# AllenNeuralDynamics/aind-exaspim-neuron-segmentation

Hardware: AMD Instinct MI355X
Metric: affinity voxels/sec on 96^3 patches over a 1024x1024x1024 volume, 1 MI355X (higher is better)
Workload: dtype fp16; 1 GPU; 1024x1024x1024 uint16 volume, 96^3 patches, overlap 32, trim 8, batch 16, fp16 (IEEE half) storage of activations and weights / fp32 accumulate (BASELINE.json configs[2]); streams=1

## Files before the change

### aind_exaspim_neuron_segmentation_amd/_native.py

```python

import ctypes
import os

_HERE = os.path.dirname(os.path.abspath(__file__))
LIB_PATH = os.path.join(_HERE, "csrc", "libexaspim_affinity.so")

DT_F32, DT_BF16, DT_F16 = 0, 1, 2
DT_BF16X3 = 3
VOX_U8, VOX_U16, VOX_I16, VOX_F32, VOX_F64 = 0, 1, 2, 3, 4
IN_F32, IN_PADDED_F32, IN_PADDED_SPLIT_F16, IN_PADDED_SPLIT_BF16 = 0, 1, 2, 3
UP_CONVT = 0x100
OPT_SEPARATE_POOL, OPT_SEPARATE_DEEP_POOLS, OPT_PLAIN_UPSAMPLE, OPT_FIRST_PER_GROUP = 1, 2, 4, 8
OPT_UPSAMPLE_PER_THREAD = 16
OPT_PER_PATCH_ENCODER = 32
OPT_SEPARATE_HEAD = 64
OPT_ROW_SEPARATE_BORDERS = 256
AFF_F32, AFF_F16 = 0, 1

DTYPE_CODES = {
    "fp32": DT_F32, "float32": DT_F32, "f32": DT_F32,
    "bf16": DT_BF16, "bfloat16": DT_BF16,
    "fp16": DT_F16, "float16": DT_F16, "f16": DT_F16,
    "bf16x3": DT_BF16X3,
}


class Block(ctypes.Structure):

    _fields_ = [
        ("dims", ctypes.c_int32 * 3),
        ("origin", ctypes.c_int32 * 3),
        ("global_", ctypes.c_int32 * 3),
    ]

    @classmethod
    def make(cls, dims, origin=None, global_shape=None):
        origin = (0, 0, 0) if origin is None else origin
        global_shape = dims if global_shape is None else global_shape
        b = cls()
        b.dims[:] = [int(v) for v in dims]
        b.origin[:] = [int(v) for v in origin]
        b.global_[:] = [int(v) for v in global_shape]
        return b


class Window(ctypes.Structure):

    _fields_ = [
        ("patch", ctypes.c_int32 * 3),
        ("overlap", ctypes.c_int32 * 3),
        ("trim", ctypes.c_int32),
    ]

    @classmethod
    def make(cls, patch, overlap, trim):
        w = cls()
        w.patch[:] = [int(v) for v in patch]
        w.overlap[:] = [int(v) for v in overlap]
        w.trim = int(trim)
        return w


class ComponentsStreamDesc(ctypes.Structure):

    _fields_ = [
        ("dims", ctypes.c_int32 * 3),
        ("channels", ctypes.c_int32),
        ("threshold", ctypes.c_float),
        ("capacity", ctypes.c_int32),
        ("min_size", ctypes.c_int64),
        ("next_z", ctypes.c_int32),
        ("reserved", ctypes.c_int32),
        ("id_parent_dev", ctypes.c_void_p),
        ("id_count_dev", ctypes.c_void_p),
        ("table_dev", ctypes.c_void_p),
        ("state_dev", ctypes.c_void_p),
        ("seam_ids_dev", ctypes.c_void_p),
        ("seam_bits_dev", ctypes.c_void_p),
    ]


_lib = None

_I32x5 = ctypes.c_int32 * 5
_I32x3 = ctypes.c_int32 * 3
_vp = ctypes.c_void_p
_sz = ctypes.c_size_t
_i32 = ctypes.c_int32

SIGNATURES = {
    "exaspim_abi_version": (_i32, []),
    "exaspim_last_error": (ctypes.c_char_p, []),
    "exaspim_unet_param_count": (_sz, [_I32x5, _i32, _i32]),
    "exaspim_unet_packed_bytes": (_sz, [_I32x5, _i32, _i32]),
    "exaspim_unet_pack_weights": (_i32, [_I32x5, _i32, _i32, _vp, _sz, _vp, _sz]),
    "exaspim_unet_create": (_i32, [_I32x5, _i32, _i32, _i32, _vp, _sz, ctypes.POINTER(_vp)]),
    "exaspim_unet_destroy": (None, [_vp]),
    "exaspim_unet_workspace_bytes": (_sz, [_vp, _i32, _i32, _i32, _i32]),
    "exaspim_unet_forward": (_i32, [_vp, _vp, _vp, _i32, _i32, _i32, _i32, _i32, _vp, _sz, _vp]),
    "exaspim_unet_forward_trimmed": (
        _i32, [_vp, _vp, _vp, _i32, _i32, _i32, _i32, _i32, _i32, _vp, _sz, _vp]
    ),
    "exaspim_unet_input_layout": (_i32, [_vp]),
    "exaspim_unet_forward_prepared": (
        _i32, [_vp, _vp, _vp, _i32, _i32, _i32, _i32, _i32, _i32, _vp, _sz, _vp]),
    "exaspim_unet_forward_prepared_row": (
        _i32, [_vp, _vp, _vp, _i32, _i32, _i32, _i32, _i32, _i32, _i32, _vp, _sz, _vp]),
    "exaspim_unet_forward_prepared_clipped": (
        _i32, [_vp, _vp, _vp, _i32, _i32, _i32, _i32, _i32, _i32, _i32, _I32x3, _vp, _sz, _vp]),
    "exaspim_unet_forward_absmax": (
        _i32, [_vp, _vp, _vp, _i32, _i32, _i32, _i32, _i32, _vp, _vp, _sz, _vp]),
    "exaspim_unet_set_options": (_i32, [_vp, ctypes.c_uint32]),
    "exaspim_unet_timing_begin": (_i32, [_vp, ctypes.c_uint32]),
    "exaspim_unet_timing_read": (_i32, [_vp, ctypes.POINTER(ctypes.c_double * 17),
                                        ctypes.POINTER(ctypes.c_int32 * 17)]),
    "exaspim_histogram": (_i32, [_vp, _i32, _sz, ctypes.c_double, _i32, _i32, ctypes.c_uint32, _vp, _vp]),
    "exaspim_histogram_wide": (_i32, [_vp, _i32, _sz, ctypes.c_double, _i32, _i32, ctypes.c_uint64, _vp, _vp]),
    "exaspim_gather_patches": (_i32, [_vp, _i32, ctypes.POINTER(Block), _vp, _i32, _I32x3,
                                      ctypes.c_double, _i32, ctypes.c_double, ctypes.c_double, _vp, _vp]),
    "exaspim_gather_patches_as": (_i32, [_vp, _i32, ctypes.POINTER(Block), _vp, _i32, _I32x3,
                                         ctypes.c_double, _i32, ctypes.c_double, ctypes.c_double, _i32,
                                         _vp, _vp]),
    "exaspim_stitch_accumulate": (_i32, [_vp, _vp, _i32, _i32, ctypes.POINTER(Window), _vp,
                                         ctypes.POINTER(Block), _vp]),
    "exaspim_stitch_finalize": (_i32, [_vp, _i32, ctypes.POINTER(Window), ctypes.POINTER(Block), _vp]),
    "exaspim_export_f16": (_i32, [_vp, _vp, ctypes.c_size_t, _vp]),
    "exaspim_components_workspace_bytes": (_sz, [_I32x3]),
    "exaspim_components": (_i32, [_vp, _i32, _i32, _I32x3, ctypes.c_float, ctypes.c_int64, _vp, _vp, _vp,
                                  _sz, _vp]),
    "exaspim_components_stream_slab_workspace_bytes": (_sz, [_I32x3]),
    "exaspim_components_stream_finish_workspace_bytes": (_sz, [_i32]),
    "exaspim_components_stream_slab": (_i32, [ctypes.POINTER(ComponentsStreamDesc), _vp, _i32, _I32x3, _i32, _vp,
                                              _vp, _sz, _vp]),
    "exaspim_components_stream_finish": (_i32, [ctypes.POINTER(ComponentsStreamDesc), _vp, _sz, _vp]),
    "exaspim_components_stream_apply": (_i32, [ctypes.POINTER(ComponentsStreamDesc), _vp, _sz, _vp]),
    "exaspim_region_graph_workspace_bytes": (_sz, [_I32x3, _i32, ctypes.c_int64]),
    "exaspim_region_graph": (_i32, [_vp, _vp, _i32, _I32x3, _i32, ctypes.c_int64, _vp, _vp, _vp, _vp, _vp, _vp,
                                    _sz, _vp]),
    "exaspim_agglomerate": (_i32, [_vp, _vp, _vp, ctypes.c_int64, _vp, _i32, ctypes.c_float, ctypes.c_int64,
                                   _vp, _vp]),
    "exaspim_apply_label_table": (_i32, [_vp, _sz, _vp, _i32, _vp]),
    "exaspim_synth_volume_u16": (_i32, [_vp, ctypes.POINTER(Block), ctypes.c_uint64, _vp]),
    "exaspim_synth_volume_neurite_u16": (_i32, [_vp, ctypes.POINTER(Block), ctypes.c_uint64, _vp]),
}


def lib():
    global _lib
    if _lib is None:
        path = LIB_PATH
        override = os.environ.get("EXASPIM_LIB")
        if override:
            import sys

            path = os.path.abspath(override)
            print(f"exaspim: EXASPIM_LIB is set, loading {path} instead of the in-tree library",
                  file=sys.stderr)
        if not os.path.exists(path):
            raise RuntimeError(
                f"HIP extension not built: {path} is missing. Build it with "
                "`make -C aind_exaspim_neuron_segmentation_amd/csrc` (or "
                "`python -c 'import __graft_entry__ as g; g.build()'`). "
                "There is no CPU fallback."
            )
        handle = ctypes.CDLL(path)
        for name, (restype, argtypes) in SIGNATURES.items():
            fn = getattr(handle, name)
            fn.restype = restype
            fn.argtypes = argtypes
        _lib = handle
    return _lib


def last_error():
    msg = lib().exaspim_last_error()
    return msg.decode("utf-8", "replace") if msg else ""


def check(rc, what):
    if rc == 0:
        return
    msg = f"{what}: {last_error()} (code {rc})"
    if rc == -1:
        raise ValueError(msg)
    raise RuntimeError(msg)


def channels_array(channels):
    if len(channels) != 5:
        raise ValueError("expected five channel widths")
    return _I32x5(*[int(c) for c in channels])


def int3(values):
    return _I32x3(*[int(v) for v in values])
```

### aind_exaspim_neuron_segmentation_amd/csrc/common.h

```cpp
#pragma once

#include <hip/hip_runtime.h>

#include <cstdarg>
#include <cstddef>
#include <cstdint>
#include <cstdio>

#include "../../include/exaspim_affinity.h"

namespace exaspim {

void set_error(const char* fmt, ...);
const char* get_error();

#define EXA_CHECK_ARG(cond, ...)                 \
    do {                                         \
        if (!(cond)) {                           \
            ::exaspim::set_error(__VA_ARGS__);   \
            return EXASPIM_E_INVALID;            \
        }                                        \
    } while (0)

#define EXA_CHECK_HIP(expr)                                                  \
    do {                                                                     \
        hipError_t _e = (expr);                                              \
        if (_e != hipSuccess) {                                              \
            ::exaspim::set_error("%s failed: %s (%s:%d)", #expr,             \
                                 hipGetErrorString(_e), __FILE__, __LINE__); \
            return EXASPIM_E_HIP;                                            \
        }                                                                    \
    } while (0)

__device__ __forceinline__ uint4 record_half(uint2 lo_group, uint2 hi_group) {
    const auto r0 = __builtin_amdgcn_permlane32_swap(lo_group.x, hi_group.x, false, false);
    const auto r1 = __builtin_amdgcn_permlane32_swap(lo_group.y, hi_group.y, false, false);
    return make_uint4(r0[0], r1[0], r0[1], r1[1]);
}


typedef unsigned int exa_u32x4 __attribute__((ext_vector_type(4)));
__device__ __forceinline__ void buf_store16(const uint4& v, __amdgpu_buffer_rsrc_t rsrc, unsigned voff,
                                            unsigned soff) {
    const exa_u32x4 d = {v.x, v.y, v.z, v.w};
    const unsigned ssoff = __builtin_amdgcn_readfirstlane(soff);
    asm volatile("s_nop 4\n\tbuffer_store_dwordx4 %0, %1, %2, %3 offen\n\ts_nop 1"
                 :: "v"(d), "v"(voff), "s"(rsrc), "s"(ssoff) : "memory");
}

__device__ __forceinline__ void buf_store16_counted(const uint4& v, __amdgpu_buffer_rsrc_t rsrc, unsigned voff,
                                                    unsigned soff) {
    const exa_u32x4 d = {v.x, v.y, v.z, v.w};
    __builtin_amdgcn_sched_barrier(0);
    __builtin_amdgcn_raw_buffer_store_b128(d, rsrc, (int)voff, (int)__builtin_amdgcn_readfirstlane(soff), 0);
    asm volatile("s_nop 1");
    __builtin_amdgcn_sched_barrier(0);
}

__device__ __forceinline__ float sat_f16(float v) {
    return v != v ? v : __builtin_amdgcn_fmed3f(v, -65504.f, 65504.f);
}

__device__ __forceinline__ float max_nan(float a, float b) {
    return (a != a || b != b) ? __uint_as_float(0x7fc00000u) : fmaxf(a, b);
}
__device__ __forceinline__ uint4 max_nan4(const uint4& a, const uint4& b) {
    return make_uint4(__float_as_uint(max_nan(__uint_as_float(a.x), __uint_as_float(b.x))),
                      __float_as_uint(max_nan(__uint_as_float(a.y), __uint_as_float(b.y))),
                      __float_as_uint(max_nan(__uint_as_float(a.z), __uint_as_float(b.z))),
                      __float_as_uint(max_nan(__uint_as_float(a.w), __uint_as_float(b.w))));
}
typedef short s16x2 __attribute__((ext_vector_type(2)));
typedef unsigned short u16x2 __attribute__((ext_vector_type(2)));
__device__ __forceinline__ unsigned key16x2(unsigned x) {
    const s16x2 m = __builtin_bit_cast(s16x2, x) >> (short)15;
    return x ^ (__builtin_bit_cast(unsigned, m) & 0x7fff7fffu);
}
template <unsigned INF16>
__device__ __forceinline__ unsigned okey16x2(unsigned x) {
    const u16x2 mag = __builtin_bit_cast(u16x2, x & 0x7fff7fffu);
    const auto nan = mag > (u16x2){(unsigned short)INF16, (unsigned short)INF16};
    return key16x2(x & ~(__builtin_bit_cast(unsigned, nan) & 0x80008000u));
}
__device__ __forceinline__ unsigned maxkey16x2(unsigned ka, unsigned kb) {
    return __builtin_bit_cast(
        unsigned, __builtin_elementwise_max(__builtin_bit_cast(s16x2, ka), __builtin_bit_cast(s16x2, kb)));
}
__device__ __forceinline__ uint4 key16(const uint4& v) {
    return make_uint4(key16x2(v.x), key16x2(v.y), key16x2(v.z), key16x2(v.w));
}
template <unsigned INF16>
__device__ __forceinline__ uint4 okey16(const uint4& v) {
    return make_uint4(okey16x2<INF16>(v.x), okey16x2<INF16>(v.y), okey16x2<INF16>(v.z), okey16x2<INF16>(v.w));
}
__device__ __forceinline__ uint4 maxkey16(const uint4& a, const uint4& b) {
    return make_uint4(maxkey16x2(a.x, b.x), maxkey16x2(a.y, b.y), maxkey16x2(a.z, b.z), maxkey16x2(a.w, b.w));
}

template <int N>
__device__ __forceinline__ float head_dot(float acc, const float (&f)[N], const float* w) {
#pragma clang fp contract(off)
#pragma unroll
    for (int j = 0; j < N; ++j) acc = fmaf(f[j], w[j], acc);
    return acc;
}
__device__ __forceinline__ float head_activation(float r, int apply_sigmoid) {
#pragma clang fp contract(off)
    if (apply_sigmoid) r = 1.f / (1.f + expf(-r));
    return r;
}

constexpr int kChannelPad = 32;
constexpr int kNumMfmaConvs = 17;

inline int pad_channels(int c) { return (c + kChannelPad - 1) / kChannelPad * kChannelPad; }
inline size_t align_up(size_t v, size_t a) { return (v + a - 1) / a * a; }
inline int storage_dtype(int dtype) { return dtype == EXASPIM_DT_BF16X3 ? EXASPIM_DT_F32 : dtype; }
inline int dtype_size(int dtype) { return storage_dtype(dtype) == EXASPIM_DT_F32 ? 4 : 2; }

struct ConvLayer {
    int ca_real = 0, cb_real = 0;
    int ca = 0, cb = 0;
    int cout_real = 0, cout = 0;
    size_t w_off = 0;
    size_t b_off = 0;
    size_t p_off = 0;
};

struct ConvTLayer {
    int cin_real = 0, cin = 0;
    int cout_real = 0, cout = 0;
    size_t w_off = 0;
    size_t b_off = 0;
    size_t p_off = 0;
};

struct UNetPlan {
    int channels[5] = {0, 0, 0, 0, 0};
    int out_channels = 0;
    int dtype = 0;
    bool convt = false;
    ConvTLayer up[4];
    int c0 = 0, c0p = 0;
    size_t first_p_off = 0;
    size_t first_w_off = 0;
    size_t first_b_off = 0;
    ConvLayer conv[kNumMfmaConvs];
    size_t head_p_off = 0;
    size_t head_w_off = 0;
    size_t head_b_off = 0;
    size_t packed_bytes = 0;
    size_t n_params = 0;
};

bool make_plan(const int32_t channels[5], int32_t out_channels, int32_t dtype,
               UNetPlan* plan);

int pack_weights(const UNetPlan& plan, const float* params, void* packed_host);

struct ConvArgs {
    const void* src_a;
    const void* src_b;
    int ca, cb;
    const void* weights;
    const void* weights_paired = nullptr;
    const void* weights_k32 = nullptr;
    const float* bias;
    void* dst;
    int cout;
    int n, d, h, w;
    float slope;
    const float* head_w = nullptr;
    const float* head_b = nullptr;
    float* head_out = nullptr;
    int head_oc = 0;
    int head_sigmoid = 0;
    int org[3] = {0, 0, 0};
    int ext[3] = {0, 0, 0};
    void* pool_dst = nullptr;
    int row_stride = 0;
    float* partial = nullptr;
    size_t partial_patch_bytes = 0;
    int ksplit = 1;
#ifdef EXASPIM_TRACE
    unsigned long long* trace = nullptr;
#endif
};

struct ConvLaunchRecord {
    const char* config = "";
    int ksplit = 0;
    bool row = false;
};
ConvLaunchRecord& last_conv_launch();
const char*& last_layer_kernel();

int launch_conv3x3x3(int dtype, const ConvArgs& a, hipStream_t stream);
int launch_conv3x3x3_thin(int dtype, const ConvArgs& a, hipStream_t stream);
int conv_zcol_main_extent(int ext, int axis);
bool conv_can_fuse_head(int cout, int w, int head_oc, int dtype = EXASPIM_DT_F32);
int launch_conv3x3x3_x3_head(const ConvArgs& a, hipStream_t stream);
bool conv_x3_can_fuse_head(int cout, int w, int head_oc);
bool conv_can_fuse_pool(int dtype, int cout, int d, int h, int w);
bool conv_row_mode_ok(int dtype, int cout, int n, int w, int row_stride, bool fused_pool_whole_patch);
constexpr int kRowStageMain = 1, kRowStageThin = 2, kRowStagePool = 4;
constexpr int kRowStagesAll = kRowStageMain | kRowStageThin | kRowStagePool;
constexpr int kRowStageBorders = 8;
constexpr int kRowStagesFused = kRowStageMain | kRowStageBorders;
int launch_conv3x3x3_row(int dtype, const ConvArgs& a, int stages, hipStream_t stream);

int launch_conv_first(int dtype, const float* x, float* xpad, const float* w, const float* bias,
                      void* dst, int n, int d, int h, int wd, int c0p, float slope,
                      hipStream_t stream, bool first_no_strips = false);
int launch_convt2(int dtype, const void* src, const void* weights, const float* bias, void* dst,
                  int n, int d, int h, int w, int cin, int cout, hipStream_t stream);
int launch_maxpool2(int dtype, const void* src, void* dst, int n, int d, int h, int w,
                    int c, hipStream_t stream);
int launch_maxpool2_xcols(int dtype, const void* src, void* dst, int n, int d, int h, int w,
                          int c, int ox0, int ox1, hipStream_t stream);
int launch_upsample2(int dtype, const void* src, void* dst, int n, int d, int h, int w,
                     int c, int margin, hipStream_t stream, bool plain_kernel = false, bool per_thread = false,
                     const int* margin_hi = nullptr);
int launch_absmax(int dtype, const void* src, size_t bytes, float* out, hipStream_t stream);
int launch_head(int dtype, const void* src, const float* w, const float* bias,
                float* out, int n, int d, int h, int wd, int c0p, int out_channels,
                int apply_sigmoid, hipStream_t stream);

}
```

### aind_exaspim_neuron_segmentation_amd/csrc/conv3d.hip

```cpp

#include <cstdlib>

#include "common.h"
#include "conv_device.h"
#include "conv_t14.h"
#include "conv_x3.h"
#include "conv_zcol.h"

namespace exaspim {

#ifdef EXASPIM_TRACE
int g_variant = 0;
#endif

ConvLaunchRecord& last_conv_launch() {
    static thread_local ConvLaunchRecord rec;
    return rec;
}

static int resident_workgroups(int per_cu) {
    static int cus = 0;
    if (cus == 0) {
        int dev = 0, n = 0;
        if (hipGetDevice(&dev) != hipSuccess ||
            hipDeviceGetAttribute(&n, hipDeviceAttributeMultiprocessorCount, dev) != hipSuccess || n <= 0)
            n = 256;
        cus = n;
    }
    return cus * per_cu;
}

static inline int cdiv(int a, int b) { return (a + b - 1) / b; }

struct TileGrid {
    int tz, ty, tx;
    long long blocks;
};
static int tile_grid(const ConvArgs& a, int TZ, int TY, int TX, int ex, int n, TileGrid& g) {
    g.tz = cdiv(a.ext[0], TZ), g.ty = cdiv(a.ext[1], TY), g.tx = cdiv(ex, TX);
    g.blocks = (long long)g.tz * g.ty * g.tx * n;
    if (g.blocks <= 0 || g.blocks > 0x7fffffffLL) {
        set_error("conv: grid of %lld blocks out of range", g.blocks);
        return EXASPIM_E_INVALID;
    }
    return EXASPIM_OK;
}

static int choose_ksplit(const ConvArgs& a, const TileGrid& g, int slices, int units) {
    const bool whole = a.ext[0] == a.d && a.ext[1] == a.h && a.ext[2] == a.w;
    constexpr int kNominalBatch = 16;
    const long long wgs = (long long)g.tz * g.ty * g.tx * kNominalBatch * slices;
    if (!a.partial || !whole || wgs * 2 > resident_workgroups(2)) return 1;
    int ks = (int)(resident_workgroups(2) / wgs);
    if (ks > 4) ks = 4;
    if (ks > units) ks = units;
    const size_t patch_vox = (size_t)a.d * a.h * a.w;
    while (ks > 1 && (size_t)ks * patch_vox * a.cout * sizeof(float) > a.partial_patch_bytes) --ks;
    return ks;
}

template <typename Tag, int TZ, int TY, int TX, int MINW, int D, int HEAD = 0, bool POOL = false>
static int launch_zpipe(const ConvArgs& a, hipStream_t stream) {
    const bool row = POOL && HEAD == 0 && Tag::kG == 8 && a.row_stride > 0;
    TileGrid g;
    if (int rc = row ? tile_grid(a, TZ, TY, TX, a.n * a.row_stride + a.w - a.row_stride, 1, g)
                     : tile_grid(a, TZ, TY, TX, a.ext[2], a.n, g))
        return rc;
    const int tz = g.tz, ty = g.ty, tx = g.tx;
    const long long blocks = g.blocks;
    const int slices = a.cout / 32;
    long long wgs = resident_workgroups(MINW) / slices / 8 * 8;
    if (wgs < 8) wgs = 8;
    if (wgs > blocks) wgs = blocks;
#ifdef EXASPIM_TRACE
    if (g_variant >= 10 && g_variant < 20) wgs = blocks;
    if (const char* e = getenv("EXASPIM_TRACE_WGS_PER_CU")) wgs = resident_workgroups(1) * (long long)atoi(e) / slices / 8 * 8;
#endif
    dim3 grid((unsigned)wgs, slices);
    last_conv_launch() = {__PRETTY_FUNCTION__, 1};
    if constexpr (POOL && HEAD == 0 && Tag::kG == 8) {
        if (row) {
            last_conv_launch().row = true;
            conv3x3x3_zpipe_row<Tag, TZ, TY, TX, MINW, D><<<grid, TY * TX * 2, 0, stream>>>(a, tz, ty, tx);
            EXA_CHECK_HIP(hipGetLastError());
            return EXASPIM_OK;
        }
    }
    conv3x3x3_zpipe<Tag, TZ, TY, TX, MINW, D, HEAD, POOL><<<grid, TY * TX * 2, 0, stream>>>(a, tz, ty, tx);
    EXA_CHECK_HIP(hipGetLastError());
    return EXASPIM_OK;
}


template <typename Tag, int TZ, int TY, int TX, int WAVES_M, int WAVES_N, int MT, int NT, int MINW, int PD = 3,
          bool ZORD = false, bool POOL = false>
static int launch_cfg(const ConvArgs& a, hipStream_t stream) {
    constexpr int NWG = WAVES_N * NT * 32;
    if (a.cout % NWG != 0) {
        set_error("conv: cout %d not a multiple of the %d-channel tile", a.cout, NWG);
        return EXASPIM_E_INVALID;
    }
    TileGrid g;
    if (int rc = tile_grid(a, TZ, TY, TX, a.ext[2], a.n, g)) return rc;
    const int tz = g.tz, ty = g.ty, tx = g.tx;
    ConvArgs b = a;
    b.ksplit = a.head_out ? 1 : choose_ksplit(a, g, a.cout / NWG, (a.ca + a.cb) / (2 * Tag::kG));
    const size_t nvox_all = (size_t)a.n * a.d * a.h * a.w;
    dim3 grid((unsigned)g.blocks, a.cout / NWG, b.ksplit);
    last_conv_launch() = {__PRETTY_FUNCTION__, b.ksplit};
    if (POOL && b.ksplit > 1) {
        b.pool_dst = nullptr;
        conv3x3x3_t14<Tag, TZ, TY, TX, WAVES_M, WAVES_N, MT, NT, MINW, PD, ZORD, false>
            <<<grid, WAVES_M * WAVES_N * 64, 0, stream>>>(b, tz, ty, tx);
    } else {
        conv3x3x3_t14<Tag, TZ, TY, TX, WAVES_M, WAVES_N, MT, NT, MINW, PD, ZORD, POOL>
            <<<grid, WAVES_M * WAVES_N * 64, 0, stream>>>(b, tz, ty, tx);
    }
    EXA_CHECK_HIP(hipGetLastError());
    if (b.ksplit > 1) {
        const size_t items = nvox_all * (a.cout / 4);
        splitk_reduce_kernel<Tag><<<(unsigned)((items + 255) / 256), 256, 0, stream>>>(
            a.partial, a.bias, a.dst, nvox_all, (size_t)a.d * a.h * a.w, a.cout, b.ksplit, a.slope);
        EXA_CHECK_HIP(hipGetLastError());
        if (POOL)
            return launch_maxpool2(Tag::kCode, a.dst, a.pool_dst, a.n, a.d, a.h, a.w, a.cout, stream);
    }
    return EXASPIM_OK;
}

template <typename Tag> struct ES_of { static constexpr int value = 16 / Tag::kG; };

template <typename Tag, int TZ, int TY, int TX, int WAVES_M, int WAVES_N, int MT, int NT, int MINW>
static int launch_cfg_pool(const ConvArgs& a, hipStream_t stream) {
    if constexpr (ES_of<Tag>::value == 2) {
        if (a.pool_dst)
            return launch_cfg<Tag, TZ, TY, TX, WAVES_M, WAVES_N, MT, NT, MINW, 3, false, true>(a, stream);
    }
    return launch_cfg<Tag, TZ, TY, TX, WAVES_M, WAVES_N, MT, NT, MINW>(a, stream);
}

template <typename Tag, int TZ, int D>
static int launch_zpipe_head(const ConvArgs& a, hipStream_t stream) {
    if (a.head_out && a.cout == 32) {
        switch (a.head_oc) {
            case 1: return launch_zpipe<Tag, TZ, 8, 16, 2, D, 1>(a, stream);
            case 2: return launch_zpipe<Tag, TZ, 8, 16, 2, D, 2>(a, stream);
            case 3: return launch_zpipe<Tag, TZ, 8, 16, 2, D, 3>(a, stream);
            case 4: return launch_zpipe<Tag, TZ, 8, 16, 2, D, 4>(a, stream);
        }
    }
    if (a.pool_dst) return launch_zpipe<Tag, TZ, 8, 16, 2, D, 0, true>(a, stream);
    return launch_zpipe<Tag, TZ, 8, 16, 2, D>(a, stream);
}

template <typename Tag, int TZ>
static int launch_zpipe_d(const ConvArgs& a, hipStream_t stream) {
#ifdef EXASPIM_TRACE
    if (g_variant % 10 == 3) return launch_zpipe_head<Tag, TZ, 3>(a, stream);
    if (g_variant % 10 == 5) return launch_zpipe_head<Tag, TZ, 5>(a, stream);
#endif
    return launch_zpipe_head<Tag, TZ, 4>(a, stream);
}

template <typename Tag>
static int launch_typed(const ConvArgs& a, hipStream_t stream) {
    if (a.w >= 16 && a.w % 16 == 0) {
#ifdef EXASPIM_TRACE
        if (g_variant >= 20) return launch_zpipe_d<Tag, 6>(a, stream);
#endif
        if (a.cout % 64 != 0) {
            if (a.head_out && a.cout == 32 && a.ext[0] % 6 != 0 && a.ext[0] % kHeadTZ == 0) {
                switch (a.head_oc) {
                    case 1: return launch_zpipe<Tag, kHeadTZ, 8, 16, 2, 4, 1>(a, stream);
                    case 2: return launch_zpipe<Tag, kHeadTZ, 8, 16, 2, 4, 2>(a, stream);
                    case 3: return launch_zpipe<Tag, kHeadTZ, 8, 16, 2, 4, 3>(a, stream);
                    case 4: return launch_zpipe<Tag, kHeadTZ, 8, 16, 2, 4, 4>(a, stream);
                }
            }
            if (a.d % 6 == 0) return launch_zpipe_d<Tag, 6>(a, stream);
            return launch_zpipe_d<Tag, 4>(a, stream);
        }
        if (a.pool_dst) return launch_cfg_pool<Tag, 4, 8, 16, 4, 1, 4, 2, 2>(a, stream);
        return launch_cfg<Tag, 4, 8, 16, 4, 1, 4, 2, 2>(a, stream);
    }
    if (a.w > 12) {
        if (a.cout % 64 == 0) return launch_cfg_pool<Tag, 4, 4, 24, 4, 1, 3, 2, 2>(a, stream);
        return launch_cfg_pool<Tag, 4, 4, 24, 4, 1, 3, 1, 2>(a, stream);
    }
    if (a.w > 6) {
        if (a.cout % 256 == 0) return launch_cfg_pool<Tag, 4, 4, 12, 2, 1, 3, 1, 2>(a, stream);
        if (a.cout % 128 == 0) return launch_cfg_pool<Tag, 4, 4, 12, 2, 2, 3, 2, 2>(a, stream);
        if (a.cout % 64 == 0) return launch_cfg_pool<Tag, 4, 4, 12, 2, 2, 3, 1, 2>(a, stream);
        return launch_cfg_pool<Tag, 4, 4, 12, 2, 1, 3, 1, 2>(a, stream);
    }
    return launch_cfg<Tag, 6, 6, 6, 4, 1, 2, 1, 2>(a, stream);
}

template <int TZ, int TY, int TX, int WAVES_M, int WAVES_N, int MT, int NT, int MINW, int PD>
static int launch_x3(const ConvArgs& a, hipStream_t stream) {
    constexpr int NWG = WAVES_N * NT * 32;
    if (a.cout % NWG != 0) {
        set_error("conv: cout %d not a multiple of the %d-channel tile", a.cout, NWG);
        return EXASPIM_E_INVALID;
    }
    TileGrid g;
    if (int rc = tile_grid(a, TZ, TY, TX, a.ext[2], a.n, g)) return rc;
    const int tz = g.tz, ty = g.ty, tx = g.tx;
    ConvArgs b = a;
    b.ksplit = choose_ksplit(a, g, a.cout / NWG, (a.ca + a.cb) / 16);
    const size_t patch_vox_all = (size_t)a.d * a.h * a.w;
    const size_t nvox_all = (size_t)a.n * patch_vox_all;
    dim3 grid((unsigned)g.blocks, a.cout / NWG, b.ksplit);
    last_conv_launch() = {__PRETTY_FUNCTION__, b.ksplit};
    conv3x3x3_x3<TZ, TY, TX, WAVES_M, WAVES_N, MT, NT, MINW, PD>
        <<<grid, WAVES_M * WAVES_N * 64, 0, stream>>>(b, tz, ty, tx);
    EXA_CHECK_HIP(hipGetLastError());
    if (b.ksplit > 1) {
        const size_t items = nvox_all * (a.cout / 4);
        splitk_reduce_kernel<F32Tag><<<(unsigned)((items + 255) / 256), 256, 0, stream>>>(
            a.partial, a.bias, a.dst, nvox_all, patch_vox_all, a.cout, b.ksplit, a.slope);
        EXA_CHECK_HIP(hipGetLastError());
    }
    return EXASPIM_OK;
}

static int launch_typed_x3(const ConvArgs& a, hipStream_t stream) {
    if (a.w >= 16 && a.w % 16 == 0) {
        if (a.cout % 64 == 0) return launch_x3<2, 8, 16, 4, 1, 2, 2, 2, 3>(a, stream);
        return launch_x3<4, 8, 16, 4, 1, 4, 1, 2, 3>(a, stream);
    }
    if (a.w > 12) {
        if (a.cout % 64 == 0) return launch_x3<4, 4, 24, 4, 1, 3, 2, 2, 1>(a, stream);
        return launch_x3<4, 4, 24, 4, 1, 3, 1, 2, 3>(a, stream);
    }
    if (a.w > 6) {
        if (a.cout % 256 == 0) return launch_x3<4, 4, 12, 2, 1, 3, 1, 2, 3>(a, stream);
        if (a.cout % 128 == 0) return launch_x3<4, 4, 12, 2, 2, 3, 2, 2, 2>(a, stream);
        if (a.cout % 64 == 0) return launch_x3<4, 4, 12, 2, 2, 3, 1, 2, 3>(a, stream);
        return launch_x3<4, 4, 12, 2, 1, 3, 1, 2, 3>(a, stream);
    }
    return launch_x3<6, 6, 6, 4, 1, 2, 1, 2, 3>(a, stream);
}

static int launch_thin_typed_x3(const ConvArgs& a, hipStream_t stream) {
    if (a.ext[1] <= a.ext[2]) return launch_x3<8, 2, 16, 4, 1, 2, 1, 2, 3>(a, stream);
    return launch_x3<8, 16, 2, 4, 1, 2, 1, 2, 3>(a, stream);
}

template <int HEAD>
static int launch_x3_head(const ConvArgs& a, hipStream_t stream) {
    TileGrid g;
    if (int rc = tile_grid(a, kX3HeadTZ, kX3HeadTY, kX3HeadTX, a.ext[2], a.n, g)) return rc;
    last_conv_launch() = {__PRETTY_FUNCTION__, 1};
    conv3x3x3_x3_head<HEAD><<<dim3((unsigned)g.blocks, 1, 1), 256, 0, stream>>>(a, g.tz, g.ty, g.tx);
    EXA_CHECK_HIP(hipGetLastError());
    return EXASPIM_OK;
}

bool conv_can_fuse_pool(int dtype, int cout, int d, int h, int w) {
    if (d % 2 != 0 || h % 2 != 0 || w % 2 != 0) return false;
    if (dtype == EXASPIM_DT_BF16X3) return false;
    if (cout % 64 != 0 && w >= 16 && w % 16 == 0) return true;
    return dtype != EXASPIM_DT_F32 && w > 6;
}

static bool head_shape_ok(int cout, int w, int head_oc) {
    return cout == 32 && w >= 16 && w % 16 == 0 && head_oc >= 1 && head_oc <= 4;
}
bool conv_can_fuse_head(int cout, int w, int head_oc, int dtype) {
    return dtype != EXASPIM_DT_BF16X3 && head_shape_ok(cout, w, head_oc);
}
bool conv_x3_can_fuse_head(int cout, int w, int head_oc) { return head_shape_ok(cout, w, head_oc); }

static int resolve_region(ConvArgs& a) {
    const int dims[3] = {a.d, a.h, a.w};
    for (int i = 0; i < 3; ++i) {
        if (a.ext[i] == 0 && a.org[i] == 0) a.ext[i] = dims[i];
        EXA_CHECK_ARG(a.org[i] >= 0 && a.ext[i] > 0 && a.org[i] + a.ext[i] <= dims[i],
                      "conv: region [%d, %d) outside axis %d of a %dx%dx%d patch", a.org[i],
                      a.org[i] + a.ext[i], i, a.d, a.h, a.w);
    }
    return EXASPIM_OK;
}

int conv_zcol_main_extent(int ext, int axis) {
    const int tile = axis == 1 ? 8 : 16;
    const int rem = ext % tile;
    return (axis != 0 && ext > tile && rem >= 1 && rem <= 4) ? ext - rem : ext;
}

bool conv_row_mode_ok(int dtype, int cout, int n, int w, int row_stride, bool fused_pool_whole_patch) {
    const int o = w - row_stride;
    return dtype_size(dtype) == 2 && fused_pool_whole_patch && cout % 64 != 0 &&
           w % 16 == 0 && n >= 2 && row_stride > 0 && o > 0 && o % 32 == 0 && row_stride >= o;
}

static int check_row_args(int dtype, const ConvArgs& a) {
    const bool whole = a.ext[0] == a.d && a.ext[1] == a.h && a.ext[2] == a.w;
    EXA_CHECK_ARG(conv_row_mode_ok(dtype, a.cout, a.n, a.w, a.row_stride,
                                   a.pool_dst && !a.head_out && whole &&
                                       conv_can_fuse_pool(dtype, a.cout, a.d, a.h, a.w)),
                  "conv: row mode needs a 16-bit fused-pool z-column layer, whole patches, n >= 2 and "
                  "an overlap that is a multiple of 32 and at most the stride (w %d, stride %d, n %d)",
                  a.w, a.row_stride, a.n);
    return EXASPIM_OK;
}

enum : unsigned { kCheckPadded = 1, kCheckEmpty = 2, kCheckSlope = 4, kCheckPatchBytes = 8, kCheckAll = 15 };
static int check_conv_args(int dtype, const ConvArgs& a, unsigned checks) {
    const int kc = dtype == EXASPIM_DT_F32 ? 8 : 16;
    EXA_CHECK_ARG(!(checks & kCheckPadded) || (a.ca % kc == 0 && a.cb % kc == 0 && a.cout % 32 == 0 && a.ca > 0),
                  "conv: channels (%d,%d)->%d not padded", a.ca, a.cb, a.cout);
    EXA_CHECK_ARG(!(checks & kCheckEmpty) || (a.n > 0 && a.d > 0 && a.h > 0 && a.w > 0), "conv: empty input");
    EXA_CHECK_ARG(!(checks & kCheckSlope) || (a.slope >= 0.f && a.slope <= 1.f),
                  "conv: LeakyReLU slope %g outside [0, 1]", a.slope);
    const unsigned long long rec = (unsigned long long)a.d * a.h * a.w * (a.ca > a.cb ? a.ca : a.cb) * dtype_size(dtype);
    EXA_CHECK_ARG(!(checks & kCheckPatchBytes) || rec < 0x80000000ULL,
                  "conv: one patch of one source is %llu bytes (>= 2 GiB)", rec);
    return EXASPIM_OK;
}

int launch_conv3x3x3(int dtype, const ConvArgs& a_in, hipStream_t stream) {
    ConvArgs a = a_in;
    if (int rc = check_conv_args(dtype, a, kCheckAll)) return rc;
    if (int rc = resolve_region(a)) return rc;
    const bool whole = a.ext[0] == a.d && a.ext[1] == a.h && a.ext[2] == a.w;
    EXA_CHECK_ARG(!a.pool_dst || (conv_can_fuse_pool(dtype, a.cout, a.d, a.h, a.w) && !a.head_out && whole),
                  "conv: fused max-pool needs an even, untrimmed patch (16-bit modes: wider than 6 voxels; "
                  "float32: a 32-cout-slice layer)");
    EXA_CHECK_ARG(!a.head_out || conv_can_fuse_head(a.cout, a.w, a.head_oc, dtype),
                  "conv: fused head needs cout 32, w %% 16 == 0, 1..4 outputs (and not bf16x3)");
    if (a.row_stride > 0)
        if (int rc = check_row_args(dtype, a)) return rc;
    switch (dtype) {
        case EXASPIM_DT_F32: return launch_typed<F32Tag>(a, stream);
        case EXASPIM_DT_BF16: return launch_typed<BF16Tag>(a, stream);
        case EXASPIM_DT_F16: return launch_typed<F16Tag>(a, stream);
        case EXASPIM_DT_BF16X3: return launch_typed_x3(a, stream);
    }
    set_error("conv: unknown dtype %d", dtype);
    return EXASPIM_E_INVALID;
}

int launch_conv3x3x3_x3_head(const ConvArgs& a_in, hipStream_t stream) {
    ConvArgs a = a_in;
    if (int rc = check_conv_args(EXASPIM_DT_BF16X3, a, kCheckAll)) return rc;
    EXA_CHECK_ARG(conv_x3_can_fuse_head(a.cout, a.w, a.head_oc),
                  "conv: bf16x3 fused head needs cout 32, w %% 16 == 0 and 1..4 outputs (cout %d, w %d, %d outputs)",
                  a.cout, a.w, a.head_oc);
    EXA_CHECK_ARG(a.head_out && a.head_w && a.head_b, "conv: bf16x3 fused head: NULL head pointer");
    EXA_CHECK_ARG(!a.pool_dst && a.row_stride == 0, "conv: bf16x3 fused head has no fused max-pool or row mode");
    if (int rc = resolve_region(a)) return rc;
    a.partial = nullptr;
    a.ksplit = 1;
    switch (a.head_oc) {
        case 1: return launch_x3_head<1>(a, stream);
        case 2: return launch_x3_head<2>(a, stream);
        case 3: return launch_x3_head<3>(a, stream);
        default: return launch_x3_head<4>(a, stream);
    }
}

template <typename Tag>
static int launch_thin_typed(const ConvArgs& a, hipStream_t stream) {
    const int ez = a.ext[0];
    auto planes = [&](int tz) { return (ez + tz - 1) / tz * tz; };
    if (a.ext[1] <= a.ext[2]) {
        const float c4 = planes(4) * 1.00f, c8 = planes(8) * 0.76f, c12 = planes(12) * 0.66f;
        if (c12 <= c8 && c12 <= c4) return launch_cfg<Tag, 12, 2, 16, 4, 1, 3, 1, 3, 3, true>(a, stream);
        if (c8 <= c4) return launch_cfg<Tag, 8, 2, 16, 4, 1, 2, 1, 4, 3, true>(a, stream);
        return launch_cfg<Tag, 4, 2, 16, 4, 1, 1, 1, 4, 3, true>(a, stream);
    }
    if (planes(8) * 0.78f <= planes(4) * 1.00f) return launch_cfg<Tag, 8, 16, 2, 4, 1, 2, 1, 4, 3, true>(a, stream);
    return launch_cfg<Tag, 4, 16, 2, 4, 1, 1, 1, 4, 3, true>(a, stream);
}

int launch_conv3x3x3_thin(int dtype, const ConvArgs& a_in, hipStream_t stream) {
    ConvArgs a = a_in;
    if (int rc = check_conv_args(dtype, a, kCheckPadded | kCheckEmpty)) return rc;
    EXA_CHECK_ARG(!a.pool_dst && !a.head_out && a.row_stride == 0, "conv: thin tiles have no fused pool, head or row mode");
    if (int rc = resolve_region(a)) return rc;
    a.partial = nullptr;
    switch (dtype) {
        case EXASPIM_DT_F32: return launch_thin_typed<F32Tag>(a, stream);
        case EXASPIM_DT_BF16: return launch_thin_typed<BF16Tag>(a, stream);
        case EXASPIM_DT_F16: return launch_thin_typed<F16Tag>(a, stream);
        case EXASPIM_DT_BF16X3: return launch_thin_typed_x3(a, stream);
    }
    set_error("conv: unknown dtype %d", dtype);
    return EXASPIM_E_INVALID;
}

template <typename Tag, int TZ, int MT>
static int launch_row_borders_cfg(const ConvArgs& a, hipStream_t stream) {
    const int tz = cdiv(a.d, TZ), ty = cdiv(a.h, 16);
    const long long blocks = (long long)tz * ty * 2 * (a.n - 1);
    if (blocks <= 0 || blocks > 0x7fffffffLL) {
        set_error("conv: grid of %lld blocks out of range", blocks);
        return EXASPIM_E_INVALID;
    }
    last_conv_launch() = {__PRETTY_FUNCTION__, 1};
    conv3x3x3_t14<Tag, TZ, 16, 2, 4, 1, MT, 1, 4, 3, true, true>
        <<<dim3((unsigned)blocks, a.cout / 32, 1), 256, 0, stream>>>(a, tz, ty, 2);
    EXA_CHECK_HIP(hipGetLastError());
    return EXASPIM_OK;
}

template <typename Tag>
static int launch_row_borders(const ConvArgs& a_in, hipStream_t stream) {
    ConvArgs a = a_in;
    a.partial = nullptr;
    a.ksplit = 1;
    a.row_stride = 0;
    auto planes = [&](int tz) { return (a.d + tz - 1) / tz * tz; };
    if (planes(8) * 0.78f <= planes(4) * 1.00f) return launch_row_borders_cfg<Tag, 8, 2>(a, stream);
    return launch_row_borders_cfg<Tag, 4, 1>(a, stream);
}

int launch_conv3x3x3_row(int dtype, const ConvArgs& a, int stages, hipStream_t stream) {
    ConvArgs b = a;
    if (int rc = check_conv_args(dtype, a, kCheckEmpty)) return rc;
    if (int rc = resolve_region(b)) return rc;
    if (int rc = check_row_args(dtype, b)) return rc;
    int r = EXASPIM_OK;
    if (stages & kRowStageMain) r = launch_conv3x3x3(dtype, a, stream);
    b.pool_dst = nullptr;
    b.row_stride = 0;
    b.n = a.n - 1;
    b.ext[2] = 2;
    if (r == EXASPIM_OK && (stages & kRowStageThin)) {
        const size_t vox = (size_t)a.d * a.h * a.w;
        b.src_a = static_cast<const char*>(a.src_a) + vox * a.ca * dtype_size(dtype);
        b.dst = static_cast<char*>(a.dst) + vox * a.cout * dtype_size(dtype);
        r = launch_conv3x3x3_thin(dtype, b, stream);
        if (r == EXASPIM_OK) {
            b.org[2] = a.w - 2;
            b.src_a = a.src_a;
            b.dst = a.dst;
            r = launch_conv3x3x3_thin(dtype, b, stream);
        }
    }
    if (r == EXASPIM_OK && (stages & kRowStagePool))
        r = launch_maxpool2_xcols(dtype, a.dst, a.pool_dst, a.n, a.d, a.h, a.w, a.cout, 0, a.w / 2 - 1, stream);
    if (r == EXASPIM_OK && (stages & kRowStageBorders)) {
        r = check_conv_args(dtype, a, kCheckPadded);
        ConvArgs c = a;
        for (int i = 0; i < 3; ++i) { c.org[i] = b.org[i]; c.ext[i] = b.ext[i]; }
        c.org[2] = 0;
        if (r == EXASPIM_OK)
            r = dtype == EXASPIM_DT_F16 ? launch_row_borders<F16Tag>(c, stream) : launch_row_borders<BF16Tag>(c, stream);
    }
    return r;
}

}
```

### aind_exaspim_neuron_segmentation_amd/csrc/conv_zcol.h

```cpp
#pragma once

#include "conv_device.h"

namespace exaspim {

template <typename Tag, int TZ, int TY, int TX, int MINW, int D, int HEAD, bool POOL, bool ROW>
__device__ __forceinline__ void zpipe_body(const ConvArgs& a, int tiles_z, int tiles_y, int tiles_x) {
    constexpr int G = Tag::kG;
    constexpr int KC = 2 * G;
    constexpr int ES = 16 / G;
    constexpr int HZ = TZ + 2, HY = TY + 2, HX = TX + 2;
    constexpr int HXP = HX;
    constexpr int PLANE = HY * HXP;
    constexpr int HVP = HZ * PLANE;
    constexpr int GS = HVP + (24 - HVP % 16) % 16;
    constexpr int NWAVES = TY * TX / 32;
    constexpr int NTHREADS = NWAVES * 64;
    constexpr int NPAIR = 2 * HY * HX;
    constexpr int REM = NPAIR > NTHREADS ? NPAIR - NTHREADS : 0;
    constexpr int SEC = (REM * HZ + NTHREADS - 1) / NTHREADS;
    constexpr int NITEMS = HZ + SEC;
    constexpr int RECB = 32 * ES;
    constexpr int RECP = RECB + 16;
    constexpr int EPI_UNITS = NWAVES * 32 * RECP / 16;
    constexpr int WUNITS = 27 * 64;
    constexpr int WITEMS = (WUNITS + NTHREADS - 1) / NTHREADS;
    constexpr int XUNITS = 2 * GS > EPI_UNITS ? 2 * GS : EPI_UNITS;
    constexpr int LDS_UNITS = XUNITS + WUNITS;
    constexpr int NS = 9 * HZ;
    constexpr int R = D + 1;
    constexpr int kLoadStride = 2;
    constexpr int LOAD_STRIDE = kLoadStride * (NITEMS + WITEMS) <= NS ? kLoadStride : 1;
    static_assert(TY * TX % 32 == 0 && NPAIR <= 2 * NTHREADS, "tile shape");
    static_assert(LOAD_STRIDE * (NITEMS + WITEMS) <= NS, "the staged pieces fit into the steps");

    __shared__ __attribute__((aligned(16))) uint4 lds[LDS_UNITS];

    const int tid = threadIdx.x;
    const int lane = tid & 63;
    const int wave = __builtin_amdgcn_readfirstlane(tid >> 6);
    const int half = lane >> 5;
    const int r = (TX == 16 && (lane & 16)) ? 16 + (((lane & 15) - HXP) & 15) : (lane & 31);

    constexpr bool row = ROW;
    static_assert(!ROW || (POOL && ES == 2 && HEAD == 0), "row mode: 16-bit fused-pool epilogue");
    const int total = tiles_z * tiles_y * tiles_x * (row ? 1 : a.n);
    int t_first, t_count, t_step;
    {
        const int q = total >> 3, rem = total & 7;
        const int xcd = blockIdx.x & 7, slot = blockIdx.x >> 3;
        t_first = (xcd < rem ? xcd * (q + 1) : rem * (q + 1) + (xcd - rem) * q) + slot;
        t_count = q + (xcd < rem ? 1 : 0) - slot;
        t_step = (gridDim.x + 7 - xcd) >> 3;
    }
    if (t_count <= 0) return;
    const int ntiles = a.cout >> 5;
    const int ntile0 = blockIdx.y;

    struct Tile {
        int z0, y0, x0, nb;
    };
    auto row_tile_at = [&](int id) {
        Tile t;
        const int s = a.row_stride, ho = (a.w - s) >> 1;
        const int rx = (id % tiles_x) * TX; id /= tiles_x;
        const int nb = min(max(rx - ho, 0) / s, a.n - 1);
        t.x0 = __builtin_amdgcn_readfirstlane(rx - nb * s);
        t.y0 = __builtin_amdgcn_readfirstlane((id % tiles_y) * TY); id /= tiles_y;
        t.z0 = __builtin_amdgcn_readfirstlane((id % tiles_z) * TZ);
        t.nb = __builtin_amdgcn_readfirstlane(nb);
        return t;
    };
    auto tile_at = [&](int id) {
        if (row) return row_tile_at(id);
        Tile t;
        t.x0 = __builtin_amdgcn_readfirstlane(a.org[2] + (id % tiles_x) * TX); id /= tiles_x;
        t.y0 = __builtin_amdgcn_readfirstlane(a.org[1] + (id % tiles_y) * TY); id /= tiles_y;
        t.z0 = __builtin_amdgcn_readfirstlane(a.org[0] + (id % tiles_z) * TZ); id /= tiles_z;
        id = __builtin_amdgcn_readfirstlane(id);
        t.nb = id;
        return t;
    };

    const int pos = wave * 32 + r;
    const int col = (pos / TX) * HXP + (pos % TX) + half * GS;

    const int plane_vox = a.h * a.w;
    const size_t patch_vox = (size_t)a.d * plane_vox;
    const bool p_ok = tid < NPAIR;
    const int p_hy = (tid >> 1) / HX, p_hx = (tid >> 1) % HX, p_kg = tid & 1;
    const int p_slot = p_kg * GS + p_hy * HXP + p_hx;
    unsigned p_voff;
    unsigned s_voff[SEC > 0 ? SEC : 1];
    int s_slot[SEC > 0 ? SEC : 1];
#pragma unroll
    for (int k = 0; k < SEC; ++k) {
        const int q = tid + k * NTHREADS;
        const int pr = NTHREADS + q % REM, hz = q / REM;
        const int c = pr >> 1, kg = pr & 1;
        s_slot[k] = q < REM * HZ ? kg * GS + hz * PLANE + (c / HX) * HXP + c % HX : -1;
    }
    auto set_offsets = [&](const Tile& t) {
        {
            const int gy = t.y0 + p_hy - 1, gx = t.x0 + p_hx - 1;
            const bool in = p_ok && (unsigned)gy < (unsigned)a.h && (unsigned)gx < (unsigned)a.w;
            p_voff = in ? (unsigned)(gy * a.w + gx) * 32u + p_kg * 16u : kOutOfRange;
        }
#pragma unroll
        for (int k = 0; k < SEC; ++k) {
            const int q = tid + k * NTHREADS;
            const int pr = NTHREADS + q % REM, hz = q / REM;
            const int c = pr >> 1, kg = pr & 1;
            const int gz = t.z0 + hz - 1, gy = t.y0 + c / HX - 1, gx = t.x0 + c % HX - 1;
            const bool in = q < REM * HZ && (unsigned)gz < (unsigned)a.d &&
                            (unsigned)gy < (unsigned)a.h && (unsigned)gx < (unsigned)a.w;
            s_voff[k] = in ? (unsigned)((gz * a.h + gy) * a.w + gx) * 32u + kg * 16u : kOutOfRange;
        }
    };
    const unsigned wvoff = (((tid >> 6) * ntiles) * 64 + (tid & 63)) * 16u;

    __shared__ __attribute__((aligned(16))) float bias_s[32];
    if (tid < 32) bias_s[tid] = a.bias[ntile0 * 32 + tid];
    __shared__ __attribute__((aligned(16))) float head_s[HEAD > 0 ? HEAD * 32 + 4 : 4];
    if (HEAD > 0) {
        if (tid < HEAD * 32) head_s[tid] = a.head_w[tid];
        if (tid < HEAD) head_s[HEAD * 32 + tid] = a.head_b[tid];
    }

    const int nchunks = (a.ca + a.cb) / KC;
    uint4 stg[NITEMS + WITEMS];
    uint4* const wlds = lds + XUNITS;
    const __amdgpu_buffer_rsrc_t wrsrc = make_rsrc(a.weights, (size_t)nchunks * 27 * ntiles * 1024);

    struct ChunkSrc {
        __amdgpu_buffer_rsrc_t rsrc;
        __amdgpu_buffer_rsrc_t none;
        unsigned cbase;
    };
    auto chunk_src = [&](int c, int nb) {
        const char* src;
        int cs, ch0;
        if (c * KC < a.ca) {
            src = static_cast<const char*>(a.src_a); cs = a.ca; ch0 = c * KC;
        } else {
            src = static_cast<const char*>(a.src_b); cs = a.cb; ch0 = c * KC - a.ca;
        }
        const size_t patchb = patch_vox * cs * ES;
        return ChunkSrc{make_rsrc(src + (size_t)nb * patchb, patchb), make_rsrc(src + (size_t)nb * patchb, 0),
                        (unsigned)(ch0 / KC) * (unsigned)patch_vox * 32u};
    };
    auto load_piece = [&](const ChunkSrc& cs, int c, int z0, int i) {
        if (i < NITEMS) {
            if (i < HZ) {
                const int gz = z0 + i - 1;
                stg[i] = (unsigned)gz < (unsigned)a.d
                             ? buf_load16(cs.rsrc, p_voff, cs.cbase + (unsigned)gz * plane_vox * 32u)
                             : buf_load16(cs.none, p_voff, 0);
            } else {
                stg[i] = buf_load16(cs.rsrc, s_voff[i - HZ], cs.cbase);
            }
        } else {
            const int it = i - NITEMS;
            stg[i] = it * NWAVES + wave < 27
                         ? buf_load16(wrsrc, wvoff, ((c * 27 + it * NWAVES) * ntiles + ntile0) * 1024)
                         : make_uint4(0, 0, 0, 0);
        }
    };
    auto stage_store = [&]() {
        if ((EXASPIM_ABLATE & 4) && stg[0].x != 0x12345u) return;
        if (p_ok) {
#pragma unroll
            for (int hz = 0; hz < HZ; ++hz) lds[p_slot + hz * PLANE] = stg[hz];
        }
#pragma unroll
        for (int k = 0; k < SEC; ++k)
            if (s_slot[k] >= 0) lds[s_slot[k]] = stg[HZ + k];
#pragma unroll
        for (int it = 0; it < WITEMS; ++it) {
            const int i = tid + it * NTHREADS;
            if (i < WUNITS) wlds[i] = stg[NITEMS + it];
        }
    };

    int tile_id = t_first;
    Tile cur = tile_at(tile_id);
    set_offsets(cur);
    {
        const ChunkSrc cs0 = chunk_src(0, cur.nb);
#pragma unroll
        for (int i = 0; i < NITEMS + WITEMS; ++i) load_piece(cs0, 0, cur.z0, i);
    }
    stage_store();

    for (;;) {
#ifdef EXASPIM_TRACE
        const size_t trace_rec = ((size_t)tile_id * NWAVES + wave) * 16;
        if (a.trace && lane == 0)
            a.trace[trace_rec + 15] =
                ((unsigned long long)__builtin_amdgcn_s_getreg((31 << 11) | 20) << 32) |
                (unsigned)__builtin_amdgcn_s_getreg((31 << 11) | 4);
#endif
        EXA_TRACE(0);
        EXA_TRACE(1);
        __syncthreads();
        f32x16 acc[TZ];
        const int half_t = fresh_lane() >> 5;
#pragma unroll
        for (int q = 0; q < 4; ++q) {
            const float4 b = *reinterpret_cast<const float4*>(bias_s + 8 * q + 4 * half_t);
#pragma unroll
            for (int mt = 0; mt < TZ; ++mt) {
                acc[mt][4 * q + 0] = b.x; acc[mt][4 * q + 1] = b.y;
                acc[mt][4 * q + 2] = b.z; acc[mt][4 * q + 3] = b.w;
            }
        }
        EXA_TRACE(2);

        t_count -= t_step;
        const bool has_next = t_count > 0;
        Tile nxt = cur;
        for (int c = 0; c < nchunks; ++c) {
            const bool more = c + 1 < nchunks;
            const bool pre = more || has_next;
            if (!more && has_next) {
                nxt = tile_at(tile_id + t_step);
                set_offsets(nxt);
            }
            const ChunkSrc csn = chunk_src(more ? c + 1 : 0, more ? cur.nb : nxt.nb);
            const int cn = more ? c + 1 : 0, zn = more ? cur.z0 : nxt.z0;
            uint4 xr[R];
            uint4 wb[3];
#pragma unroll
            for (int dz = 0; dz < 3; ++dz) wb[dz] = wlds[(dz * 9) * 64 + lane];
#pragma unroll
            for (int s = 0; s < D; ++s)
                xr[s % R] = lds[col + (s % HZ) * PLANE + ((s / HZ) / 3) * HXP + (s / HZ) % 3];
            __builtin_amdgcn_sched_barrier(0);
            if (ES == 2) __builtin_amdgcn_s_setprio(kSetprio);
#pragma unroll
            for (int s = 0; s < NS; ++s) {
                const int g = s / HZ, zin = s % HZ;
                if (s + D < NS) {
                    const int g2 = (s + D) / HZ, z2 = (s + D) % HZ;
                    xr[(s + D) % R] = lds[col + z2 * PLANE + (g2 / 3) * HXP + g2 % 3];
                }
#ifdef EXASPIM_TRACE
                if (nchunks == 2 && c == 0 && s > 0 && s % (NS / 4) == 0 && s / (NS / 4) <= 3) EXA_TRACE(8 + s / (NS / 4));
#endif
                if (g + 1 < 9 && zin >= TZ) wb[zin - TZ] = wlds[((zin - TZ) * 9 + g + 1) * 64 + lane];
                if (g > 0 && zin == 0) wb[2] = wlds[(2 * 9 + g) * 64 + lane];
                if (!(EXASPIM_ABLATE & 1) && pre && s % LOAD_STRIDE == 0 && s / LOAD_STRIDE < NITEMS + WITEMS)
                    load_piece(csn, cn, zn, s / LOAD_STRIDE);
#pragma unroll
                for (int dz = 0; dz < 3; ++dz) {
                    const int z = zin - dz;
                    if (z >= 0 && z < TZ) mma_inplace<Tag>(acc[z], wb[dz], xr[s % R]);
                }
                __builtin_amdgcn_sched_barrier(0);
            }
            if (ES == 2) __builtin_amdgcn_s_setprio(0);
            if (ES == 2) asm volatile("s_nop 7\n\ts_nop 7\n\ts_nop 1");
            if (c < 4) EXA_TRACE(3 + 3 * c);
            __syncthreads();
            if (c < 4) EXA_TRACE(4 + 3 * c);
            if (more) {
                stage_store();
                __syncthreads();
                if (c < 3) EXA_TRACE(5 + 3 * c);
            }
        }
        if (has_next) {
#pragma unroll
            for (int i = 0; i < NITEMS + WITEMS; ++i)
                asm volatile("" : "+v"(stg[i].x), "+v"(stg[i].y), "+v"(stg[i].z), "+v"(stg[i].w));
        }

        const int lane_e = fresh_lane();
        const int half_e = lane_e >> 5;
        const int r_e = (TX == 16 && (lane_e & 16)) ? 16 + (((lane_e & 15) - HXP) & 15) : (lane_e & 31);
        const int pos_e = wave * 32 + r_e;
        if (HEAD > 0) {
            float part[TZ][HEAD > 0 ? HEAD : 1];
#pragma unroll
            for (int z = 0; z < TZ; ++z)
#pragma unroll
                for (int o = 0; o < HEAD; ++o) part[z][o] = 0.f;
#pragma unroll
            for (int q = 0; q < 4; ++q) {
                float4 hw[HEAD > 0 ? HEAD : 1];
#pragma unroll
                for (int o = 0; o < HEAD; ++o)
                    hw[o] = *reinterpret_cast<const float4*>(head_s + o * 32 + 8 * q + 4 * half_e);
#pragma unroll
                for (int z = 0; z < TZ; ++z) {
                    float v0 = acc[z][4 * q + 0], v1 = acc[z][4 * q + 1];
                    float v2 = acc[z][4 * q + 2], v3 = acc[z][4 * q + 3];
                    v0 = leaky(v0, a.slope);
                    v1 = leaky(v1, a.slope);
                    v2 = leaky(v2, a.slope);
                    v3 = leaky(v3, a.slope);
#pragma unroll
                    for (int o = 0; o < HEAD; ++o)
                        part[z][o] = fmaf(v3, hw[o].w, fmaf(v2, hw[o].z, fmaf(v1, hw[o].y, fmaf(v0, hw[o].x, part[z][o]))));
                }
            }
            const size_t plane = (size_t)a.h * a.w;
            const int gy = cur.y0 + pos_e / TX, gx = cur.x0 + pos_e % TX;
            const bool okyx = gy < a.org[1] + a.ext[1] && gx < a.org[2] + a.ext[2];
            float* const hpatch = a.head_out + (size_t)cur.nb * HEAD * a.d * plane;
            const size_t hbytes = (size_t)HEAD * a.d * plane * sizeof(float);
            const unsigned hvoff[2] = {okyx && half_e == 0 ? (unsigned)(gy * a.w + gx) * 4u : kOutOfRange,
                                       okyx && half_e == 1 ? (unsigned)(gy * a.w + gx) * 4u : kOutOfRange};
#pragma unroll
            for (int z = 0; z < TZ; ++z) {
                const int gz = cur.z0 + z;
                const __amdgpu_buffer_rsrc_t hrsrc = make_rsrc(hpatch, gz < a.org[0] + a.ext[0] ? hbytes : (size_t)0);
#pragma unroll
                for (int o = 0; o < HEAD; ++o) {
                    float t = part[z][o] + __shfl_xor(part[z][o], 32) + head_s[HEAD * 32 + o];
                    if (a.head_sigmoid) t = 1.f / (1.f + expf(-t));
                    __builtin_amdgcn_raw_buffer_store_b32(__float_as_uint(t), hrsrc, (int)hvoff[o & 1],
                                                          (int)((unsigned)(o * a.d + gz) * (unsigned)plane * 4u), 0);
                }
            }
        } else if (ES == 2 && !POOL) {
            char* const dplane = static_cast<char*>(a.dst) +
                                 ((size_t)cur.nb * (a.cout / KC) + ntile0 * 2) * patch_vox * 32;
            const int gy = cur.y0 + pos_e / TX, gx = cur.x0 + pos_e % TX;
            const bool okyx = gy < a.org[1] + a.ext[1] && gx < a.org[2] + a.ext[2];
            const unsigned ovoff = okyx ? (unsigned)(gy * a.w + gx) * 32u + half_e * 16u : kOutOfRange;
#pragma unroll
            for (int z = 0; z < TZ; ++z) {
                uint2 grp[4];
#pragma unroll
                for (int q = 0; q < 4; ++q)
                    grp[q] = pack4<Tag>(leaky(acc[z][4 * q + 0], a.slope), leaky(acc[z][4 * q + 1], a.slope),
                                        leaky(acc[z][4 * q + 2], a.slope), leaky(acc[z][4 * q + 3], a.slope));
                const int gz = cur.z0 + z;
#pragma unroll
                for (int ck = 0; ck < 2; ++ck) {
                    const uint4 rec = record_half(grp[2 * ck], grp[2 * ck + 1]);
                    const unsigned soff = ((unsigned)ck * (unsigned)patch_vox + (unsigned)gz * (unsigned)plane_vox) * 32u;
                    const __amdgpu_buffer_rsrc_t orsrc =
                        make_rsrc(dplane, gz < a.org[0] + a.ext[0] ? (size_t)2 * patch_vox * 32 : (size_t)0);
                    buf_store16(rec, orsrc, ovoff, soff);
                }
            }
        } else if (ES == 2 && POOL) {
            static_assert(!(ES == 2 && POOL) || (TZ % 2 == 0 && TY % 2 == 0 && TX == 16), "pooled tile shape");
            constexpr int CPT = 2;
            char* wl = reinterpret_cast<char*>(lds) + wave * ((TZ / 2) * 32 * RECP);
            char* const dplane = static_cast<char*>(a.dst) +
                                 ((size_t)cur.nb * (a.cout / KC) + ntile0 * 2) * patch_vox * 32;
            const int gy = cur.y0 + pos_e / TX, gx = cur.x0 + pos_e % TX;
            const bool okyx = gy < a.org[1] + a.ext[1] && gx < a.org[2] + a.ext[2];
            const unsigned ovoff = okyx ? (unsigned)(gy * a.w + gx) * 32u + half_e * 16u : kOutOfRange;
            const int rs = a.row_stride, rho = (a.w - rs) >> 1;
            const bool nnext = row && cur.x0 >= rs && cur.x0 < rs + rho && cur.nb + 1 < a.n;
            const bool nprev = row && cur.x0 >= rho && cur.x0 < 2 * rho && cur.nb >= 1;
            const bool shared = nnext || nprev;
            const int nshift = nnext ? -rs : nprev ? rs : 0;
            const int nnb = cur.nb + (nnext ? 1 : nprev ? -1 : 0);
            const int ngx = gx + nshift;
            const bool nlane = ngx >= 2 && ngx < a.w - 2;
            const int nbase = nshift * 32;
            char* const nplane = static_cast<char*>(a.dst) + nbase +
                                 ((size_t)nnb * (a.cout / KC) + ntile0 * 2) * patch_vox * 32;
            const size_t nbytes = (size_t)((long long)2 * patch_vox * 32 - nbase);
#pragma unroll
            for (int zp = 0; zp < TZ / 2; ++zp) {
                uint2 grp[2][4];
#pragma unroll
                for (int zz = 0; zz < 2; ++zz)
#pragma unroll
                    for (int q = 0; q < 4; ++q)
                        grp[zz][q] = pack4<Tag>(leaky(acc[2 * zp + zz][4 * q + 0], a.slope), leaky(acc[2 * zp + zz][4 * q + 1], a.slope),
                                                leaky(acc[2 * zp + zz][4 * q + 2], a.slope), leaky(acc[2 * zp + zz][4 * q + 3], a.slope));
#pragma unroll
                for (int q = 0; q < 4; ++q) {
                    const uint2 km = make_uint2(maxkey16x2(okey16x2<Tag::kInf16>(grp[0][q].x), okey16x2<Tag::kInf16>(grp[1][q].x)),
                                                maxkey16x2(okey16x2<Tag::kInf16>(grp[0][q].y), okey16x2<Tag::kInf16>(grp[1][q].y)));
                    *reinterpret_cast<uint2*>(wl + zp * (32 * RECP) + r_e * RECP + (8 * q + 4 * half_e) * ES) = km;
                }
#pragma unroll
                for (int zz = 0; zz < 2; ++zz) {
                    const int gz = cur.z0 + 2 * zp + zz;
                    const __amdgpu_buffer_rsrc_t orsrc =
                        make_rsrc(dplane, gz < a.org[0] + a.ext[0] ? (size_t)2 * patch_vox * 32 : (size_t)0);
                    const __amdgpu_buffer_rsrc_t nrsrc = make_rsrc(nplane, gz < a.org[0] + a.ext[0] ? nbytes : (size_t)0);
#pragma unroll
                    for (int ck = 0; ck < 2; ++ck) {
                        const uint4 rec = record_half(grp[zz][2 * ck], grp[zz][2 * ck + 1]);
                        buf_store16(rec, orsrc, ovoff, ((unsigned)ck * (unsigned)patch_vox + (unsigned)gz * (unsigned)plane_vox) * 32u);
                        if (shared)
                            buf_store16(rec, nrsrc, nlane ? ovoff : kOutOfRange, ((unsigned)ck * (unsigned)patch_vox + (unsigned)gz * (unsigned)plane_vox) * 32u);
                    }
                }
            }
            __builtin_amdgcn_fence(__ATOMIC_RELEASE, "wavefront");
            __builtin_amdgcn_wave_barrier();
            {
                constexpr int NP = (TZ / 2) * 8 * CPT * 2;
                const int pd = a.d >> 1, ph = a.h >> 1, pw2 = a.w >> 1;
                const size_t pvox = (size_t)pd * ph * pw2;
                char* const pplane = static_cast<char*>(a.pool_dst) +
                                     ((size_t)cur.nb * (a.cout / KC) + ntile0 * CPT) * pvox * 32;
                const __amdgpu_buffer_rsrc_t prsrc = make_rsrc(pplane, (size_t)CPT * pvox * 32);
                char* const npplane = static_cast<char*>(a.pool_dst) + nbase / 2 +
                                      ((size_t)nnb * (a.cout / KC) + ntile0 * CPT) * pvox * 32;
                const __amdgpu_buffer_rsrc_t nprsrc = make_rsrc(npplane, (size_t)((long long)CPT * pvox * 32 - nbase / 2));
#pragma unroll
                for (int p0 = 0; p0 < NP; p0 += 64) {
                    const int p = p0 + lane_e;
                    const bool live = p < NP;
                    const int pc = live ? p : 0;
                    const int zp = pc / (8 * CPT * 2), rem = pc % (8 * CPT * 2);
                    const int ck = rem / 16, xp = (rem % 16) >> 1, sb = rem & 1;
                    const char* rec = wl + zp * (32 * RECP) + (2 * xp) * RECP + (ck * 2 + sb) * 16;
                    uint4 m = *reinterpret_cast<const uint4*>(rec);
#pragma unroll
                    for (int k = 1; k < 4; ++k)
                        m = maxkey16(m, *reinterpret_cast<const uint4*>(rec + (k >> 1) * 16 * RECP + (k & 1) * RECP));
                    m = key16(m);
                    const int qz = cur.z0 / 2 + zp, qy = cur.y0 / 2 + wave, qx = cur.x0 / 2 + xp;
                    const unsigned pvoff = live && qz < pd && qy < ph && qx < pw2
                                               ? (unsigned)((ck * (int)pvox + (qz * ph + qy) * pw2 + qx) * 32 + sb * 16)
                                               : kOutOfRange;
                    buf_store16(m, prsrc, pvoff, 0u);
                    if (shared) {
                        const int nqx = qx + nshift / 2;
                        buf_store16(m, nprsrc, nqx >= 1 && nqx < pw2 - 1 ? pvoff : kOutOfRange, 0u);
                    }
                }
            }
            __builtin_amdgcn_fence(__ATOMIC_ACQUIRE, "wavefront");
            __builtin_amdgcn_wave_barrier();
        } else {
            constexpr int CPT = RECB / 32;
            constexpr int TB_MAX = LDS_UNITS * 16 / (NWAVES * 32 * RECP);
            constexpr int TB = POOL ? ((TB_MAX >= TZ ? TZ : TB_MAX) & ~1)
                                    : (TB_MAX >= TZ ? TZ : (TB_MAX >= (TZ + 1) / 2 ? (TZ + 1) / 2 : 1));
            static_assert(!POOL || (TB >= 2 && TZ % 2 == 0 && TY % 2 == 0 && TX == 16), "pooled tile shape");
            char* wl = reinterpret_cast<char*>(lds) + wave * (TB * 32 * RECP);
            char* const dplane = static_cast<char*>(a.dst) +
                                 ((size_t)cur.nb * (a.cout / KC) + ntile0 * CPT) * patch_vox * 32;
            const int vv = lane_e >> 1, sub = lane_e & 1;
            const int po = wave * 32 + vv;
            const int ogy = cur.y0 + po / TX, ogx = cur.x0 + po % TX;
#pragma unroll
            for (int zb = 0; zb < TZ; zb += TB) {
#pragma unroll
                for (int z = zb; z < zb + TB && z < TZ; ++z) {
#pragma unroll
                    for (int q = 0; q < 4; ++q) {
                        const int cl = 8 * q + 4 * half_e;
                        float v0 = acc[z][4 * q + 0], v1 = acc[z][4 * q + 1];
                        float v2 = acc[z][4 * q + 2], v3 = acc[z][4 * q + 3];
                        v0 = leaky(v0, a.slope);
                        v1 = leaky(v1, a.slope);
                        v2 = leaky(v2, a.slope);
                        v3 = leaky(v3, a.slope);
                        store4<Tag>(wl + (z - zb) * (32 * RECP), (size_t)(r_e * RECP) / ES + cl, v0, v1, v2, v3);
                    }
                }
                __builtin_amdgcn_fence(__ATOMIC_RELEASE, "wavefront");
                __builtin_amdgcn_wave_barrier();
#pragma unroll
                for (int z = zb; z < zb + TB && z < TZ; ++z) {
                    const int gz = cur.z0 + z;
                    const bool tokyx = ogy < a.org[1] + a.ext[1] && ogx < a.org[2] + a.ext[2];
                    const unsigned tvoff = tokyx ? (unsigned)(ogy * a.w + ogx) * 32u + sub * 16u : kOutOfRange;
                    const __amdgpu_buffer_rsrc_t trsrc =
                        make_rsrc(dplane, gz < a.org[0] + a.ext[0] ? (size_t)CPT * patch_vox * 32 : (size_t)0);
#pragma unroll
                    for (int ck = 0; ck < CPT; ++ck) {
                        const uint4 val = *reinterpret_cast<const uint4*>(
                            wl + (z - zb) * (32 * RECP) + vv * RECP + (ck * 2 + sub) * 16);
                        buf_store16(val, trsrc, tvoff,
                                    ((unsigned)ck * (unsigned)patch_vox + (unsigned)gz * (unsigned)plane_vox) * 32u);
                    }
                }
                if (POOL) {
                    constexpr int NP = (TB / 2) * 8 * CPT * 2;
                    const int pd = a.d >> 1, ph = a.h >> 1, pw2 = a.w >> 1;
                    const size_t pvox = (size_t)pd * ph * pw2;
                    char* const pplane = static_cast<char*>(a.pool_dst) +
                                         ((size_t)cur.nb * (a.cout / KC) + ntile0 * CPT) * pvox * 32;
                    const __amdgpu_buffer_rsrc_t prsrc = make_rsrc(pplane, (size_t)CPT * pvox * 32);
#pragma unroll
                    for (int p0 = 0; p0 < NP; p0 += 64) {
                        const int p = p0 + lane_e;
                        const bool live0 = p < NP;
                        const int pc = live0 ? p : 0;
                        const int zp = pc / (8 * CPT * 2), rem = pc % (8 * CPT * 2);
                        const int ck = rem / 16, xp = (rem % 16) >> 1, sb = rem & 1;
                        const bool live = live0 && zb + 2 * zp + 1 < TZ;
                        const int zr = zb + 2 * zp + 1 < TZ ? zp : 0;
                        const char* rec = wl + (2 * zr) * (32 * RECP) + (2 * xp) * RECP + (ck * 2 + sb) * 16;
                        uint4 m = *reinterpret_cast<const uint4*>(rec);
                        if (ES == 2) m = okey16<Tag::kInf16>(m);
#pragma unroll
                        for (int k = 1; k < 8; ++k) {
                            const uint4 v = *reinterpret_cast<const uint4*>(
                                rec + (k >> 2) * (32 * RECP) + ((k >> 1) & 1) * 16 * RECP + (k & 1) * RECP);
                            m = ES == 2 ? maxkey16(m, okey16<Tag::kInf16>(v)) : max16<Tag>(m, v);
                        }
                        if (ES == 2) m = key16(m);
                        const int qz = (cur.z0 + zb) / 2 + zp, qy = cur.y0 / 2 + wave, qx = cur.x0 / 2 + xp;
                        const unsigned pvoff =
                            live && qz < pd && qy < ph && qx < pw2
                                ? (unsigned)((ck * (int)pvox + (qz * ph + qy) * pw2 + qx) * 32 + sb * 16)
                                : kOutOfRange;
                        buf_store16(m, prsrc, pvoff, 0u);
                    }
                }
                __builtin_amdgcn_fence(__ATOMIC_ACQUIRE, "wavefront");
                __builtin_amdgcn_wave_barrier();
            }
        }
        EXA_TRACE(14);
        if (!has_next) break;
        if (!(HEAD > 0 || (ES == 2 && !POOL))) __syncthreads();
        stage_store();
        tile_id += t_step;
        cur = nxt;
    }
}

template <typename Tag, int TZ, int TY, int TX, int MINW, int D, int HEAD = 0, bool POOL = false>
__global__ __launch_bounds__(TY* TX * 2, MINW) void conv3x3x3_zpipe(
    ConvArgs a, int tiles_z, int tiles_y, int tiles_x) {
    zpipe_body<Tag, TZ, TY, TX, MINW, D, HEAD, POOL, false>(a, tiles_z, tiles_y, tiles_x);
}

template <typename Tag, int TZ, int TY, int TX, int MINW, int D>
__global__ __launch_bounds__(TY* TX * 2, MINW) void conv3x3x3_zpipe_row(
    ConvArgs a, int tiles_z, int tiles_y, int tiles_x) {
    zpipe_body<Tag, TZ, TY, TX, MINW, D, 0, true, true>(a, tiles_z, tiles_y, tiles_x);
}

}
```

### aind_exaspim_neuron_segmentation_amd/csrc/engine.hip

```cpp

#include <algorithm>
#include <cstdlib>
#include <new>
#include <string_view>

#include "common.h"

namespace exaspim {

constexpr float kLeakySlope = 0.01f;

struct Workspace {
    size_t skip[5], a[5], b[5];
    size_t xpad;
    size_t bytes;
};

}

struct LayerTimer {
    static constexpr int kRing = 16384;
    uint32_t mask = 0;
    int next = 0, used = 0;
    hipEvent_t start[kRing], stop[kRing];
    int layer[kRing];
    bool created = false;
};

struct exaspim_unet {
    exaspim::UNetPlan plan;
    int device;
    const char* packed;
    LayerTimer* timer = nullptr;
    uint32_t options = 0;
};

namespace exaspim {

static bool level_dims_ok(int d, int h, int w) {
    return d > 0 && h > 0 && w > 0 && d % 16 == 0 && h % 16 == 0 && w % 16 == 0;
}

static int conv_level(int i) {
    if (i == 0) return 0;
    if (i <= 8) return (i + 1) / 2;
    return 3 - (i - 9) / 2;
}

static Workspace make_workspace(const UNetPlan& p, int n, int d, int h, int w) {
    int maxc[5] = {p.c0p, 0, 0, 0, 0};
    for (int i = 0; i < kNumMfmaConvs; ++i) {
        const ConvLayer& L = p.conv[i];
        int& m = maxc[conv_level(i)];
        m = std::max(m, std::max(std::max(L.ca, L.cb), L.cout));
    }
    const size_t es = dtype_size(p.dtype);
    Workspace ws;
    size_t off = 0;
    for (int l = 0; l < 5; ++l) {
        const size_t vox = (size_t)n * (d >> l) * (h >> l) * (w >> l);
        const size_t sz = align_up(vox * maxc[l] * es, 256);
        ws.skip[l] = off; off += (l < 4 ? sz : 0);
        ws.a[l] = off; off += sz;
        ws.b[l] = off; off += sz;
    }
    ws.xpad = off;
    off += align_up((size_t)n * (d + 2) * (h + 2) * (w + 2) * sizeof(float), 256);
    ws.bytes = off;
    return ws;
}

static int forward(exaspim_unet* e, const float* x, float* out, int n, int d, int h, int w,
                   int apply_sigmoid, int trim, void* workspace, size_t workspace_bytes,
                   hipStream_t stream, const void* x_prepared = nullptr, float* absmax = nullptr,
                   int row_stride = 0, const int32_t* keep_hi = nullptr) {
    const UNetPlan& p = e->plan;
    const Workspace ws = make_workspace(p, n, d, h, w);
    if (workspace_bytes < ws.bytes) {
        set_error("forward: workspace %zu bytes < required %zu", workspace_bytes, ws.bytes);
        return EXASPIM_E_WORKSPACE;
    }
    char* base = static_cast<char*>(workspace);
    auto skip = [&](int l) { return (void*)(base + ws.skip[l]); };
    auto A = [&](int l) { return (void*)(base + ws.a[l]); };
    auto B = [&](int l) { return (void*)(base + ws.b[l]); };
    const int dt = p.dtype;
    int rc;

    const bool x3 = dt == EXASPIM_DT_BF16X3;
    const int last_cout = p.conv[kNumMfmaConvs - 1].cout;
    const bool fuse_head = !absmax && !(e->options & EXASPIM_OPT_SEPARATE_HEAD) &&
                           (x3 ? conv_x3_can_fuse_head(last_cout, w, p.out_channels)
                               : conv_can_fuse_head(last_cout, w, p.out_channels, dt));
    const bool trimmed = fuse_head && trim > 0 && 2 * trim < d && 2 * trim < h && 2 * trim < w;
    int khi[3] = {d - trim, h - trim, w - trim};
    if (trimmed && keep_hi)
        for (int i = 0; i < 3; ++i) khi[i] = keep_hi[i];
    const bool separate_pool = (e->options & EXASPIM_OPT_SEPARATE_POOL) != 0;
    const bool separate_deep = (e->options & EXASPIM_OPT_SEPARATE_DEEP_POOLS) != 0;
    bool fuse_pool[4];
    for (int l = 0; l < 4; ++l)
        fuse_pool[l] = !separate_pool && !(separate_deep && l > 0) && conv_can_fuse_pool(p.dtype, p.conv[2 * l].cout, d >> l, h >> l, w >> l);
    const bool row = !absmax && !(e->options & EXASPIM_OPT_PER_PATCH_ENCODER) &&
                     conv_row_mode_ok(dt, p.conv[0].cout, n, w, row_stride, fuse_pool[0]);
    auto conv = [&](int idx, const void* sa, const void* sb, void* dst, int l) -> int {
        const ConvLayer& L = p.conv[idx];
        ConvArgs a;
        a.partial = reinterpret_cast<float*>(base + ws.xpad);
        a.partial_patch_bytes = (size_t)(d + 2) * (h + 2) * (w + 2) * sizeof(float);
        if (idx <= 6 && idx % 2 == 0 && fuse_pool[idx / 2]) a.pool_dst = A(idx / 2 + 1);
        const bool last = idx == kNumMfmaConvs - 1, last_but_one = idx == kNumMfmaConvs - 2;
        const int margin = !trimmed ? 0 : last ? trim : last_but_one ? trim - 1 : 0;
        const int full[3] = {d >> l, h >> l, w >> l};
        for (int i = 0; i < 3; ++i) {
            a.org[i] = margin;
            a.ext[i] = trimmed && (last || last_but_one) ? khi[i] + (last ? 0 : 1) - margin : full[i];
        }
        int rem_y = 0, rem_x = 0;
        const bool has_head = idx == kNumMfmaConvs - 1 && fuse_head;
        if (margin > 0 && !has_head && L.cout % 64 != 0 && full[2] % 16 == 0) {
            rem_y = a.ext[1] - conv_zcol_main_extent(a.ext[1], 1);
            rem_x = a.ext[2] - conv_zcol_main_extent(a.ext[2], 2);
            a.ext[1] -= rem_y;
            a.ext[2] -= rem_x;
        }
        if (idx == kNumMfmaConvs - 1 && fuse_head) {
            a.head_w = reinterpret_cast<const float*>(e->packed + p.head_w_off);
            a.head_b = reinterpret_cast<const float*>(e->packed + p.head_b_off);
            a.head_out = out;
            a.head_oc = p.out_channels;
            a.head_sigmoid = apply_sigmoid;
        }
        a.src_a = sa; a.src_b = sb; a.ca = L.ca; a.cb = L.cb;
        a.weights = e->packed + L.w_off;
        a.bias = reinterpret_cast<const float*>(e->packed + L.b_off);
        a.dst = dst; a.cout = L.cout;
        a.n = n; a.d = d >> l; a.h = h >> l; a.w = w >> l;
        a.slope = kLeakySlope;
        if (idx == 0 && row) a.row_stride = row_stride;
        LayerTimer* t = e->timer;
        const bool timed = t && (t->mask >> idx & 1u) && t->used < LayerTimer::kRing;
        int slot = 0;
        if (timed) {
            slot = t->next;
            EXA_CHECK_HIP(hipEventRecord(t->start[slot], stream));
        }
        int r = x3 && has_head      ? launch_conv3x3x3_x3_head(a, stream)
                : a.row_stride > 0 ? launch_conv3x3x3_row(dt, a, (e->options & EXASPIM_OPT_ROW_SEPARATE_BORDERS) ? kRowStagesAll : kRowStagesFused, stream)
                                   : launch_conv3x3x3(dt, a, stream);
        if (timed && r == EXASPIM_OK) {
            EXA_CHECK_HIP(hipEventRecord(t->stop[slot], stream));
            t->layer[slot] = idx;
            t->next = (slot + 1) % LayerTimer::kRing;
            t->used++;
        }
        if (r == EXASPIM_OK && rem_y > 0) {
            ConvArgs b = a;
            b.org[1] = a.org[1] + a.ext[1]; b.ext[1] = rem_y;
            b.ext[2] = a.ext[2] + rem_x;
            r = launch_conv3x3x3_thin(dt, b, stream);
        }
        if (r == EXASPIM_OK && rem_x > 0) {
            ConvArgs b = a;
            b.org[2] = a.org[2] + a.ext[2]; b.ext[2] = rem_x;
            r = launch_conv3x3x3_thin(dt, b, stream);
        }
        if (r == EXASPIM_OK && absmax)
            r = launch_absmax(dt, dst, (size_t)n * (d >> l) * (h >> l) * (w >> l) * L.cout * dtype_size(dt),
                              absmax + 1 + idx, stream);
        return r;
    };
#define RUN(expr) do { rc = (expr); if (rc) return rc; } while (0)

    RUN(launch_conv_first(dt, x, x ? reinterpret_cast<float*>(base + ws.xpad)
                                   : const_cast<float*>(static_cast<const float*>(x_prepared)),
                          reinterpret_cast<const float*>(e->packed + p.first_w_off),
                          reinterpret_cast<const float*>(e->packed + p.first_b_off), A(0), n, d,
                          h, w, p.c0p, kLeakySlope, stream, (e->options & EXASPIM_OPT_FIRST_PER_GROUP) != 0));
    if (absmax) RUN(launch_absmax(dt, A(0), (size_t)n * d * h * w * p.c0p * dtype_size(dt), absmax, stream));
    RUN(conv(0, A(0), nullptr, skip(0), 0));
    for (int l = 1; l <= 4; ++l) {
        const ConvLayer& L0 = p.conv[2 * l - 1];
        const void* prev = skip(l - 1);
        if (!fuse_pool[l - 1])
            RUN(launch_maxpool2(dt, prev, A(l), n, d >> (l - 1), h >> (l - 1), w >> (l - 1), L0.ca,
                                stream));
        RUN(conv(2 * l - 1, A(l), nullptr, B(l), l));
        RUN(conv(2 * l, B(l), nullptr, l < 4 ? skip(l) : A(l), l));
    }
    const void* prev = A(4);
    for (int l = 3; l >= 0; --l) {
        const int i0 = 9 + 2 * (3 - l);
        const ConvLayer& L0 = p.conv[i0];
        if (p.convt) {
            const ConvTLayer& U = p.up[3 - l];
            RUN(launch_convt2(dt, prev, e->packed + U.w_off,
                              reinterpret_cast<const float*>(e->packed + U.b_off), A(l), n,
                              d >> (l + 1), h >> (l + 1), w >> (l + 1), U.cin, U.cout, stream));
            if (absmax)
                RUN(launch_absmax(dt, A(l), (size_t)n * (d >> l) * (h >> l) * (w >> l) * U.cout * dtype_size(dt),
                                  absmax + 1 + kNumMfmaConvs + (3 - l), stream));
        } else {
            const bool ups_trimmed = trimmed && l == 0 && trim > 2;
            const int ups_hi[3] = {std::max(d - khi[0] - 2, 0), std::max(h - khi[1] - 2, 0), std::max(w - khi[2] - 2, 0)};
            RUN(launch_upsample2(dt, prev, A(l), n, d >> (l + 1), h >> (l + 1), w >> (l + 1), L0.cb,
                                 ups_trimmed ? trim - 2 : 0, stream,
                                 (e->options & EXASPIM_OPT_PLAIN_UPSAMPLE) != 0,
                                 (e->options & EXASPIM_OPT_UPSAMPLE_PER_THREAD) != 0, ups_trimmed ? ups_hi : nullptr));
        }
        RUN(conv(i0, skip(l), A(l), B(l), l));
        RUN(conv(i0 + 1, B(l), nullptr, A(l), l));
        prev = A(l);
    }
    if (!fuse_head)
    RUN(launch_head(dt, prev, reinterpret_cast<const float*>(e->packed + p.head_w_off),
                    reinterpret_cast<const float*>(e->packed + p.head_b_off), out, n, d, h, w,
                    p.c0p, p.out_channels, apply_sigmoid, stream));
#undef RUN
    return EXASPIM_OK;
}

}

using namespace exaspim;

extern "C" int exaspim_abi_version(void) { return EXASPIM_ABI_VERSION; }
extern "C" const char* exaspim_last_error(void) { return get_error(); }

extern "C" size_t exaspim_unet_param_count(const int32_t channels[5], int32_t out_channels,
                                           int32_t dtype) {
    UNetPlan p;
    if (!make_plan(channels, out_channels, dtype, &p)) return 0;
    return p.n_params;
}

extern "C" size_t exaspim_unet_packed_bytes(const int32_t channels[5], int32_t out_channels,
                                            int32_t dtype) {
    UNetPlan p;
    if (!make_plan(channels, out_channels, dtype, &p)) return 0;
    return p.packed_bytes;
}

extern "C" int exaspim_unet_pack_weights(const int32_t channels[5], int32_t out_channels,
                                         int32_t dtype, const float* params, size_t n_params,
                                         void* packed_host, size_t packed_bytes) {
    UNetPlan p;
    if (!make_plan(channels, out_channels, dtype, &p)) return EXASPIM_E_INVALID;
    EXA_CHECK_ARG(params && packed_host, "pack_weights: NULL pointer");
    EXA_CHECK_ARG(n_params == p.n_params, "pack_weights: got %zu parameters, expected %zu",
                  n_params, p.n_params);
    EXA_CHECK_ARG(packed_bytes == p.packed_bytes, "pack_weights: buffer %zu bytes, expected %zu",
                  packed_bytes, p.packed_bytes);
    return pack_weights(p, params, packed_host);
}

extern "C" int exaspim_unet_create(const int32_t channels[5], int32_t out_channels,
                                   int32_t dtype, int32_t device, const void* packed_dev,
                                   size_t packed_bytes, exaspim_unet** out) {
    EXA_CHECK_ARG(out != nullptr && packed_dev != nullptr, "create: NULL pointer");
    UNetPlan p;
    if (!make_plan(channels, out_channels, dtype, &p)) return EXASPIM_E_INVALID;
    EXA_CHECK_ARG(packed_bytes == p.packed_bytes, "create: packed image %zu bytes, expected %zu",
                  packed_bytes, p.packed_bytes);
    int ndev = 0;
    if (hipGetDeviceCount(&ndev) != hipSuccess || ndev <= 0 || device < 0 || device >= ndev) {
        set_error("create: device %d not available (%d HIP devices visible)", device, ndev);
        return EXASPIM_E_NODEVICE;
    }
    hipDeviceProp_t prop;
    EXA_CHECK_HIP(hipGetDeviceProperties(&prop, device));
    if (std::string_view(prop.gcnArchName).substr(0, 6) != "gfx950") {
        set_error("create: device %d is %s; this library is built for gfx950 only", device,
                  prop.gcnArchName);
        return EXASPIM_E_NODEVICE;
    }
    exaspim_unet* e = new (std::nothrow) exaspim_unet;
    EXA_CHECK_ARG(e != nullptr, "create: out of host memory");
    e->plan = p;
    e->device = device;
    e->packed = static_cast<const char*>(packed_dev);
    *out = e;
    return EXASPIM_OK;
}

extern "C" void exaspim_unet_destroy(exaspim_unet* h) {
    if (!h) return;
    if (h->timer) {
        if (h->timer->created)
            for (int i = 0; i < LayerTimer::kRing; ++i) {
                (void)hipEventDestroy(h->timer->start[i]);
                (void)hipEventDestroy(h->timer->stop[i]);
            }
        delete h->timer;
    }
    delete h;
}

extern "C" int exaspim_unet_timing_begin(exaspim_unet* h, uint32_t conv_mask) {
    EXA_CHECK_ARG(h != nullptr, "timing_begin: NULL handle");
    if (!h->timer) h->timer = new (std::nothrow) LayerTimer;
    EXA_CHECK_ARG(h->timer != nullptr, "timing_begin: out of host memory");
    LayerTimer* t = h->timer;
    if (!t->created) {
        for (int i = 0; i < LayerTimer::kRing; ++i) {
            EXA_CHECK_HIP(hipEventCreate(&t->start[i]));
            EXA_CHECK_HIP(hipEventCreate(&t->stop[i]));
        }
        t->created = true;
    }
    t->mask = conv_mask;
    t->next = 0;
    t->used = 0;
    return EXASPIM_OK;
}

extern "C" int exaspim_unet_timing_read(exaspim_unet* h, double ms_sum[17], int32_t count[17]) {
    EXA_CHECK_ARG(h && h->timer && ms_sum && count, "timing_read: timing was not started");
    LayerTimer* t = h->timer;
    for (int i = 0; i < kNumMfmaConvs; ++i) { ms_sum[i] = 0.0; count[i] = 0; }
    for (int s = 0; s < t->used; ++s) {
        EXA_CHECK_HIP(hipEventSynchronize(t->stop[s]));
        float ms = 0.f;
        EXA_CHECK_HIP(hipEventElapsedTime(&ms, t->start[s], t->stop[s]));
        ms_sum[t->layer[s]] += ms;
        count[t->layer[s]]++;
    }
    t->mask = 0;
    t->used = 0;
    t->next = 0;
    return EXASPIM_OK;
}

extern "C" size_t exaspim_unet_workspace_bytes(const exaspim_unet* h, int32_t n, int32_t d,
                                               int32_t hgt, int32_t w) {
    if (!h || n <= 0 || !level_dims_ok(d, hgt, w)) {
        set_error("workspace_bytes: bad arguments (n %d, patch %dx%dx%d must be multiples of 16)",
                  n, d, hgt, w);
        return 0;
    }
    return make_workspace(h->plan, n, d, hgt, w).bytes;
}

extern "C" int exaspim_unet_forward(exaspim_unet* h, const float* x_dev, float* out_dev,
                                    int32_t n, int32_t d, int32_t hgt, int32_t w,
                                    int32_t apply_sigmoid, void* workspace_dev,
                                    size_t workspace_bytes, void* stream) {
    EXA_CHECK_ARG(h && x_dev && out_dev && workspace_dev, "forward: NULL pointer");
    EXA_CHECK_ARG(n > 0, "forward: empty batch");
    EXA_CHECK_ARG(level_dims_ok(d, hgt, w),
                  "forward: patch %dx%dx%d: every dimension must be a positive multiple of 16",
                  d, hgt, w);
    return forward(h, x_dev, out_dev, n, d, hgt, w, apply_sigmoid, 0, workspace_dev, workspace_bytes,
                   (hipStream_t)stream);
}

extern "C" int exaspim_unet_input_layout(const exaspim_unet* h) {
    if (!h) return EXASPIM_E_INVALID;
    switch (h->plan.dtype) {
        case EXASPIM_DT_F32:
        case EXASPIM_DT_BF16X3: return EXASPIM_IN_PADDED_F32;
        case EXASPIM_DT_F16: return EXASPIM_IN_PADDED_SPLIT_F16;
        case EXASPIM_DT_BF16: return EXASPIM_IN_PADDED_SPLIT_BF16;
    }
    return EXASPIM_E_INVALID;
}

extern "C" int exaspim_unet_forward_prepared(exaspim_unet* h, const void* x_prepared_dev, float* out_dev,
                                             int32_t n, int32_t d, int32_t hgt, int32_t w,
                                             int32_t apply_sigmoid, int32_t trim,
                                             void* workspace_dev, size_t workspace_bytes,
                                             void* stream) {
    EXA_CHECK_ARG(h && x_prepared_dev && out_dev && workspace_dev, "forward: NULL pointer");
    EXA_CHECK_ARG(n > 0, "forward: empty batch");
    EXA_CHECK_ARG(trim >= 0, "forward: negative trim %d", trim);
    EXA_CHECK_ARG(level_dims_ok(d, hgt, w),
                  "forward: patch %dx%dx%d: every dimension must be a positive multiple of 16",
                  d, hgt, w);
    return forward(h, nullptr, out_dev, n, d, hgt, w, apply_sigmoid, trim, workspace_dev,
                   workspace_bytes, (hipStream_t)stream, x_prepared_dev);
}

extern "C" int exaspim_unet_forward_prepared_row(exaspim_unet* h, const void* x_prepared_dev, float* out_dev,
                                                 int32_t n, int32_t d, int32_t hgt, int32_t w,
                                                 int32_t apply_sigmoid, int32_t trim, int32_t row_stride,
                                                 void* workspace_dev, size_t workspace_bytes,
                                                 void* stream) {
    EXA_CHECK_ARG(h && x_prepared_dev && out_dev && workspace_dev, "forward: NULL pointer");
    EXA_CHECK_ARG(n > 0, "forward: empty batch");
    EXA_CHECK_ARG(trim >= 0, "forward: negative trim %d", trim);
    EXA_CHECK_ARG(row_stride >= 0, "forward: negative row stride %d", row_stride);
    EXA_CHECK_ARG(level_dims_ok(d, hgt, w),
                  "forward: patch %dx%dx%d: every dimension must be a positive multiple of 16",
                  d, hgt, w);
    return forward(h, nullptr, out_dev, n, d, hgt, w, apply_sigmoid, trim, workspace_dev,
                   workspace_bytes, (hipStream_t)stream, x_prepared_dev, nullptr, row_stride);
}

extern "C" int exaspim_unet_forward_prepared_clipped(exaspim_unet* h, const void* x_prepared_dev, float* out_dev,
                                                     int32_t n, int32_t d, int32_t hgt, int32_t w,
                                                     int32_t apply_sigmoid, int32_t trim, int32_t row_stride,
                                                     const int32_t keep_hi[3], void* workspace_dev,
                                                     size_t workspace_bytes, void* stream) {
    EXA_CHECK_ARG(h && x_prepared_dev && out_dev && workspace_dev && keep_hi, "forward: NULL pointer");
    EXA_CHECK_ARG(n > 0, "forward: empty batch");
    EXA_CHECK_ARG(trim >= 0, "forward: negative trim %d", trim);
    EXA_CHECK_ARG(row_stride >= 0, "forward: negative row stride %d", row_stride);
    EXA_CHECK_ARG(level_dims_ok(d, hgt, w),
                  "forward: patch %dx%dx%d: every dimension must be a positive multiple of 16",
                  d, hgt, w);
    const int size[3] = {d, hgt, w};
    for (int i = 0; i < 3; ++i)
        EXA_CHECK_ARG(keep_hi[i] > trim && keep_hi[i] <= size[i] - trim,
                      "forward: keep_hi[%d] = %d outside (%d, %d] (trim %d of %d voxels)", i, keep_hi[i], trim,
                      size[i] - trim, trim, size[i]);
    return forward(h, nullptr, out_dev, n, d, hgt, w, apply_sigmoid, trim, workspace_dev,
                   workspace_bytes, (hipStream_t)stream, x_prepared_dev, nullptr, row_stride, keep_hi);
}

extern "C" int exaspim_unet_forward_trimmed(exaspim_unet* h, const float* x_dev, float* out_dev,
                                            int32_t n, int32_t d, int32_t hgt, int32_t w,
                                            int32_t apply_sigmoid, int32_t trim,
                                            void* workspace_dev, size_t workspace_bytes,
                                            void* stream) {
    EXA_CHECK_ARG(h && x_dev && out_dev && workspace_dev, "forward: NULL pointer");
    EXA_CHECK_ARG(n > 0, "forward: empty batch");
    EXA_CHECK_ARG(trim >= 0, "forward: negative trim %d", trim);
    EXA_CHECK_ARG(level_dims_ok(d, hgt, w),
                  "forward: patch %dx%dx%d: every dimension must be a positive multiple of 16",
                  d, hgt, w);
    return forward(h, x_dev, out_dev, n, d, hgt, w, apply_sigmoid, trim, workspace_dev,
                   workspace_bytes, (hipStream_t)stream);
}

extern "C" int exaspim_unet_forward_absmax(exaspim_unet* h, const float* x_dev, float* out_dev,
                                           int32_t n, int32_t d, int32_t hgt, int32_t w,
                                           int32_t apply_sigmoid, float* absmax_dev,
                                           void* workspace_dev, size_t workspace_bytes, void* stream) {
    EXA_CHECK_ARG(h && x_dev && out_dev && workspace_dev && absmax_dev, "forward_absmax: NULL pointer");
    EXA_CHECK_ARG(n > 0, "forward: empty batch");
    EXA_CHECK_ARG(level_dims_ok(d, hgt, w),
                  "forward: patch %dx%dx%d: every dimension must be a positive multiple of 16",
                  d, hgt, w);
    return forward(h, x_dev, out_dev, n, d, hgt, w, apply_sigmoid, 0, workspace_dev, workspace_bytes,
                   (hipStream_t)stream, nullptr, absmax_dev);
}

extern "C" int exaspim_unet_set_options(exaspim_unet* h, uint32_t options) {
    EXA_CHECK_ARG(h != nullptr, "set_options: NULL handle");
    EXA_CHECK_ARG((options & ~(uint32_t)(EXASPIM_OPT_SEPARATE_POOL | EXASPIM_OPT_SEPARATE_DEEP_POOLS | EXASPIM_OPT_PLAIN_UPSAMPLE | EXASPIM_OPT_FIRST_PER_GROUP |
                                          EXASPIM_OPT_UPSAMPLE_PER_THREAD | EXASPIM_OPT_PER_PATCH_ENCODER |
                                          EXASPIM_OPT_SEPARATE_HEAD | EXASPIM_OPT_ROW_SEPARATE_BORDERS)) == 0,
                  "set_options: unknown option bits 0x%x", options);
    h->options = options;
    return EXASPIM_OK;
}
```

### aind_exaspim_neuron_segmentation_amd/csrc/layer_probe.hip

```cpp

#include "common.h"

using namespace exaspim;

extern "C" {

const char* probe_last_error(void) { return get_error(); }

const char* probe_last_config(void) { return last_conv_launch().config; }
int probe_last_ksplit(void) { return last_conv_launch().ksplit; }
void probe_reset_config(void) {
    last_conv_launch() = ConvLaunchRecord{};
    last_layer_kernel() = "";
}
int probe_last_row(void) { return last_conv_launch().row ? 1 : 0; }
const char* probe_last_layer_kernel(void) { return last_layer_kernel(); }

int probe_conv3x3x3(int thin, int dtype, const void* src_a, const void* src_b, int ca, int cb,
                    const void* weights, const float* bias, void* dst, int cout, int n, int d, int h,
                    int w, float slope, const int32_t* region, void* pool_dst, float* partial,
                    size_t partial_patch_bytes, const float* head_w, const float* head_b,
                    float* head_out, int head_oc, int head_sigmoid, hipStream_t stream) {
    ConvArgs a{};
    a.src_a = src_a;
    a.src_b = src_b;
    a.ca = ca;
    a.cb = cb;
    a.weights = weights;
    a.bias = bias;
    a.dst = dst;
    a.cout = cout;
    a.n = n;
    a.d = d;
    a.h = h;
    a.w = w;
    a.slope = slope;
    for (int i = 0; i < 3; ++i) {
        a.org[i] = region ? region[i] : 0;
        a.ext[i] = region ? region[3 + i] : 0;
    }
    a.pool_dst = pool_dst;
    a.partial = partial;
    a.partial_patch_bytes = partial_patch_bytes;
    a.head_w = head_w;
    a.head_b = head_b;
    a.head_out = head_out;
    a.head_oc = head_oc;
    a.head_sigmoid = head_sigmoid;
    return thin ? launch_conv3x3x3_thin(dtype, a, stream) : launch_conv3x3x3(dtype, a, stream);
}

int probe_conv3x3x3_x3_head(int thin, int dtype, const void* src_a, const void* src_b, int ca, int cb,
                            const void* weights, const float* bias, void* dst, int cout, int n, int d, int h,
                            int w, float slope, const int32_t* region, void* pool_dst, float* partial,
                            size_t partial_patch_bytes, const float* head_w, const float* head_b,
                            float* head_out, int head_oc, int head_sigmoid, hipStream_t stream) {
    EXA_CHECK_ARG(!thin && dtype == EXASPIM_DT_BF16X3 && !partial,
                  "probe: the bf16x3 head launcher has no thin tiles, no other dtype and no split-K");
    ConvArgs a{};
    a.src_a = src_a;
    a.src_b = src_b;
    a.ca = ca;
    a.cb = cb;
    a.weights = weights;
    a.bias = bias;
    a.dst = dst;
    a.cout = cout;
    a.n = n;
    a.d = d;
    a.h = h;
    a.w = w;
    a.slope = slope;
    for (int i = 0; i < 3; ++i) {
        a.org[i] = region ? region[i] : 0;
        a.ext[i] = region ? region[3 + i] : 0;
    }
    a.pool_dst = pool_dst;
    a.head_w = head_w;
    a.head_b = head_b;
    a.head_out = head_out;
    a.head_oc = head_oc;
    a.head_sigmoid = head_sigmoid;
    return launch_conv3x3x3_x3_head(a, stream);
}

int probe_conv3x3x3_row(int dtype, const void* src, int ca, const void* weights, const float* bias, void* dst,
                        int cout, int n, int d, int h, int w, float slope, int row_stride, void* pool_dst,
                        int stages, hipStream_t stream) {
    ConvArgs a{};
    a.src_a = src;
    a.ca = ca;
    a.weights = weights;
    a.bias = bias;
    a.dst = dst;
    a.cout = cout;
    a.n = n;
    a.d = d;
    a.h = h;
    a.w = w;
    a.slope = slope;
    a.row_stride = row_stride;
    a.pool_dst = pool_dst;
    return launch_conv3x3x3_row(dtype, a, stages, stream);
}

int probe_conv_row_mode_ok(int dtype, int cout, int n, int w, int row_stride, int fused_pool_whole_patch) {
    return conv_row_mode_ok(dtype, cout, n, w, row_stride, fused_pool_whole_patch != 0) ? 1 : 0;
}

int probe_conv_first(int dtype, const float* x, float* xpad, const float* w, const float* bias,
                     void* dst, int n, int d, int h, int wd, int c0p, float slope, int per_group,
                     hipStream_t stream) {
    return launch_conv_first(dtype, x, xpad, w, bias, dst, n, d, h, wd, c0p, slope, stream, per_group != 0);
}

int probe_maxpool2(int dtype, const void* src, void* dst, int n, int d, int h, int w, int c,
                   hipStream_t stream) {
    return launch_maxpool2(dtype, src, dst, n, d, h, w, c, stream);
}

int probe_maxpool2_xcols(int dtype, const void* src, void* dst, int n, int d, int h, int w, int c, int ox0,
                         int ox1, hipStream_t stream) {
    return launch_maxpool2_xcols(dtype, src, dst, n, d, h, w, c, ox0, ox1, stream);
}

int probe_upsample2(int dtype, const void* src, void* dst, int n, int d, int h, int w, int c,
                    int margin, int plain_kernel, int per_thread, hipStream_t stream) {
    return launch_upsample2(dtype, src, dst, n, d, h, w, c, margin, stream, plain_kernel != 0,
                            per_thread != 0);
}

int probe_convt2(int dtype, const void* src, const void* weights, const float* bias, void* dst, int n,
                 int d, int h, int w, int cin, int cout, hipStream_t stream) {
    return launch_convt2(dtype, src, weights, bias, dst, n, d, h, w, cin, cout, stream);
}

int probe_head(int dtype, const void* src, const float* w, const float* bias, float* out, int n,
               int d, int h, int wd, int c0p, int out_channels, int apply_sigmoid, hipStream_t stream) {
    return launch_head(dtype, src, w, bias, out, n, d, h, wd, c0p, out_channels, apply_sigmoid, stream);
}

int probe_plan_conv(const int32_t channels[5], int32_t out_channels, int32_t dtype, int layer,
                    int64_t out[8]) {
    UNetPlan p;
    if (!make_plan(channels, out_channels, dtype, &p)) return EXASPIM_E_INVALID;
    EXA_CHECK_ARG(layer >= 0 && layer < kNumMfmaConvs, "probe: layer %d out of range", layer);
    const ConvLayer& L = p.conv[layer];
    const int64_t v[8] = {L.ca_real, L.cb_real, L.ca, L.cb, L.cout_real, L.cout, (int64_t)L.w_off,
                          (int64_t)L.b_off};
    for (int i = 0; i < 8; ++i) out[i] = v[i];
    return EXASPIM_OK;
}

}
```

### aind_exaspim_neuron_segmentation_amd/inference.py

```python

import ctypes
import itertools
import threading
import time
from concurrent.futures import ThreadPoolExecutor

import numpy as np
import torch

from aind_exaspim_neuron_segmentation_amd import _native
from aind_exaspim_neuron_segmentation_amd.machine_learning.unet3d import UNet3D
from aind_exaspim_neuron_segmentation_amd.utils import img_util

try:
    from tqdm import tqdm
except ImportError:
    tqdm = None

DEFAULT_STREAMS = 3
PLAIN_GATHER = False
FULL_PATCHES = False
CLIP_TO_VOLUME = True

_VOX_CODES = {
    np.dtype(np.uint8): _native.VOX_U8,
    np.dtype(np.uint16): _native.VOX_U16,
    np.dtype(np.int16): _native.VOX_I16,
    np.dtype(np.float32): _native.VOX_F32,
    np.dtype(np.float64): _native.VOX_F64,
}
_TORCH_VOXELS = {np.dtype(np.uint8): torch.uint8, np.dtype(np.uint16): torch.int16,
                 np.dtype(np.int16): torch.int16, np.dtype(np.float32): torch.float32,
                 np.dtype(np.float64): torch.float64}


def predict(
    img,
    model,
    affinity_mode=True,
    batch_size=16,
    brightness_clip=1000,
    normalization_percentiles=(1, 99.9),
    patch_shape=(96, 96, 96),
    overlap=(32, 32, 32),
    trim=8,
    verbose=True,
    *,
    return_device_tensor=False,
    n_streams=DEFAULT_STREAMS,
    out_dtype=np.float32,
):
    out_dtype = _checked_out_dtype(out_dtype)
    device = _hip_device(model)
    if not return_device_tensor and not isinstance(img, (DeviceVolume, torch.Tensor)):
        return predict_streaming(
            img, model, affinity_mode=affinity_mode, batch_size=batch_size,
            brightness_clip=brightness_clip, normalization_percentiles=normalization_percentiles,
            patch_shape=patch_shape, overlap=overlap, trim=trim, verbose=verbose,
            n_streams=n_streams, out_dtype=out_dtype,
        )
    volume = DeviceVolume.from_array(img, device, clip=brightness_clip)
    plan = SlidingWindow(volume.shape, patch_shape, overlap, trim)
    n_channels = 3 if affinity_mode else 1
    with torch.cuda.device(device):
        mn, mx = volume_percentiles(volume, brightness_clip, normalization_percentiles)
        accum = run_sliding_window(
            volume, model, plan, n_channels, batch_size, brightness_clip, mn, mx,
            verbose=verbose, n_streams=n_streams,
        )
        stitch_finalize(accum, plan, volume.block)
        if out_dtype == np.float16:
            accum = export_half(accum)
    pred = accum if affinity_mode else accum[0]
    if return_device_tensor:
        return pred
    return pred.cpu().numpy()


def _checked_out_dtype(out_dtype):
    out_dtype = np.dtype(out_dtype)
    if out_dtype not in (np.dtype(np.float32), np.dtype(np.float16)):
        raise TypeError(f"out_dtype must be numpy.float32 or numpy.float16, got {out_dtype}")
    return out_dtype


def export_half(tensor, out=None):
    if tensor.dtype != torch.float32 or not tensor.is_contiguous():
        raise ValueError("export_half needs a contiguous float32 tensor")
    if out is None:
        out = torch.empty(tensor.shape, dtype=torch.float16, device=tensor.device)
    elif out.dtype != torch.float16 or not out.is_contiguous() or out.numel() != tensor.numel():
        raise ValueError("export_half: out must be a contiguous float16 tensor of the same size")
    _native.check(
        _native.lib().exaspim_export_f16(tensor.data_ptr(), out.data_ptr(), tensor.numel(),
                                         _stream(tensor.device)),
        "exaspim_export_f16",
    )
    return out.view(tensor.shape)


_AFF_CODES = {torch.float32: _native.AFF_F32, torch.float16: _native.AFF_F16}


def _components_on_device(affinities, threshold=0.5, min_segment_size=100):
    if not isinstance(affinities, torch.Tensor):
        raise TypeError(f"_components_on_device needs a torch tensor, got {type(affinities).__name__}")
    if affinities.dtype not in _AFF_CODES:
        raise TypeError(f"affinities must be float32 or float16, got {affinities.dtype}")
    if affinities.dim() == 4:
        if affinities.shape[0] != 3:
            raise ValueError(f"4-D affinities must be (3, D, H, W), got {tuple(affinities.shape)}")
        channels = 3
    elif affinities.dim() == 3:
        channels = 1
    else:
        raise ValueError("affinities must be (3, D, H, W) or a (D, H, W) foreground map, "
                         f"got {affinities.dim()} dimensions")
    if affinities.device.type != "cuda":
        raise RuntimeError(
            "affinities_to_components (MI355X) has no CPU path: the tensor must be on a HIP device, "
            f"got {affinities.device}"
        )
    dims = tuple(int(v) for v in affinities.shape[-3:])
    if min(dims) < 1:
        raise ValueError(f"empty volume {dims}")
    affinities = affinities.contiguous()
    device = affinities.device
    lib = _native.lib()
    need = lib.exaspim_components_workspace_bytes(_native.int3(dims))
    if need == 0:
        raise ValueError(_native.last_error())
    with torch.cuda.device(device):
        labels = torch.empty(dims, dtype=torch.int32, device=device)
        count = torch.empty(1, dtype=torch.int32, device=device)
        workspace = torch.empty(need, dtype=torch.uint8, device=device)
        _native.check(
            lib.exaspim_components(affinities.data_ptr(), _AFF_CODES[affinities.dtype], channels,
                                   _native.int3(dims), float(np.float32(threshold)), int(min_segment_size),
                                   labels.data_ptr(), count.data_ptr(), workspace.data_ptr(), need,
                                   _stream(device)),
            "exaspim_components",
        )
    return labels, count


def affinities_to_components(affinities, threshold=0.5, min_segment_size=100, *,
                             return_device_tensor=False):
    if isinstance(affinities, np.ndarray):
        if affinities.dtype not in (np.dtype(np.float32), np.dtype(np.float16)):
            raise TypeError(f"affinities must be float32 or float16, got {affinities.dtype}")
        if affinities.ndim not in (3, 4):
            raise ValueError("affinities must be (3, D, H, W) or a (D, H, W) foreground map, "
                             f"got {affinities.ndim} dimensions")
        if not torch.cuda.is_available():
            raise RuntimeError("affinities_to_components (MI355X) has no CPU path and no HIP device is present")
        affinities = torch.from_numpy(np.ascontiguousarray(affinities)).to("cuda:0")
    labels, _ = _components_on_device(affinities, threshold, min_segment_size)
    if return_device_tensor:
        return labels
    return labels.cpu().numpy()


DEFAULT_EDGE_CAPACITY = 1 << 22


def _default_edge_capacity(voxels):
    want = 6 * int(voxels)
    return min(DEFAULT_EDGE_CAPACITY, 1 << max(want - 1, 0).bit_length())


def _region_graph_on_device(labels, affinities, n_labels, edge_capacity=None):
    if labels.dtype != torch.int32 or labels.dim() != 3:
        raise TypeError(f"labels must be a 3-D int32 tensor, got {labels.dtype} with {labels.dim()} dimensions")
    if affinities.dtype not in _AFF_CODES:
        raise TypeError(f"affinities must be float32 or float16, got {affinities.dtype}")
    dims = tuple(int(v) for v in labels.shape)
    if affinities.dim() != 4 or tuple(affinities.shape) != (3,) + dims:
        raise ValueError(f"affinities must be (3, D, H, W) = {(3,) + dims}, got {tuple(affinities.shape)}; "
                         "a foreground map has no affinities to score")
    if min(dims) < 1:
        raise ValueError(f"empty volume {dims}")
    if labels.device.type != "cuda" or affinities.device != labels.device:
        raise RuntimeError("region_graph (MI355X) has no CPU path: labels and affinities must be on one HIP "
                           f"device, got {labels.device} and {affinities.device}")
    n_labels = int(n_labels)
    if n_labels < 0:
        raise ValueError(f"n_labels must not be negative, got {n_labels}")
    capacity = _default_edge_capacity(np.prod(dims, dtype=np.int64)) if edge_capacity is None else int(edge_capacity)
    labels, affinities = labels.contiguous(), affinities.contiguous()
    device = labels.device
    lib = _native.lib()
    need = lib.exaspim_region_graph_workspace_bytes(_native.int3(dims), n_labels, capacity)
    if need == 0:
        raise ValueError(_native.last_error())
    with torch.cuda.device(device):
        edges = torch.empty((capacity, 2), dtype=torch.int32, device=device)
        counts = torch.empty(capacity, dtype=torch.int64, device=device)
        sums = torch.empty(capacity, dtype=torch.int64, device=device)
        sizes = torch.empty(n_labels + 1, dtype=torch.int64, device=device)
        state = torch.empty(2, dtype=torch.int32, device=device)
        workspace = torch.empty(need, dtype=torch.uint8, device=device)
        _native.check(
            lib.exaspim_region_graph(labels.data_ptr(), affinities.data_ptr(), _AFF_CODES[affinities.dtype],
                                     _native.int3(dims), n_labels, capacity, edges.data_ptr(), counts.data_ptr(),
                                     sums.data_ptr(), sizes.data_ptr(), state.data_ptr(), workspace.data_ptr(),
                                     need, _stream(device)),
            "exaspim_region_graph",
        )
        n_edges, overflow = (int(v) for v in state.cpu())
        if overflow:
            raise RuntimeError(
                f"region_graph: the volume has more pairs of adjacent labels than edge_capacity={capacity}; "
                "run it again with a larger edge_capacity (a power of two)")
        edges_h = edges[:n_edges].cpu().numpy()
        counts_h = counts[:n_edges].cpu().numpy()
        sums_h = sums[:n_edges].cpu().numpy().view(np.uint64)
        sizes_h = sizes.cpu().numpy()
    order = np.lexsort((edges_h[:, 1], edges_h[:, 0]))
    return (np.ascontiguousarray(edges_h[order]), np.ascontiguousarray(counts_h[order]),
            np.ascontiguousarray(sums_h[order]), sizes_h)


def region_graph(labels, affinities, *, edge_capacity=None):
    def on_device(a, what, dtypes):
        if isinstance(a, np.ndarray):
            if a.dtype not in dtypes:
                raise TypeError(f"{what} must be {' or '.join(str(np.dtype(d)) for d in dtypes)}, got {a.dtype}")
            if not torch.cuda.is_available():
                raise RuntimeError("region_graph (MI355X) has no CPU path and no HIP device is present")
            return torch.from_numpy(np.ascontiguousarray(a)).to("cuda:0")
        if not isinstance(a, torch.Tensor):
            raise TypeError(f"{what} must be a torch tensor or a numpy array, got {type(a).__name__}")
        return a

    labels = on_device(labels, "labels", (np.int32,))
    affinities = on_device(affinities, "affinities", (np.float32, np.float16))
    if labels.dtype != torch.int32 or labels.dim() != 3:
        raise TypeError(f"labels must be a 3-D int32 tensor, got {labels.dtype} with {labels.dim()} dimensions")
    n_labels = max(int(labels.max()), 0) if labels.numel() else 0
    return _region_graph_on_device(labels, affinities, n_labels, edge_capacity)


def _last_threshold(agglomeration_thresholds):
    thresholds = [float(t) for t in agglomeration_thresholds]
    if not thresholds:
        raise ValueError("agglomeration_thresholds is empty")
    if any(t != t for t in thresholds):
        raise ValueError(f"agglomeration_thresholds holds a NaN: {thresholds}")
    if any(b < a for a, b in zip(thresholds, thresholds[1:])):
        raise ValueError(f"agglomeration_thresholds must be non-decreasing, got {thresholds}")
    return thresholds[-1]


def agglomerate(edges, counts, sums, sizes, agglomeration_thresholds=(0.6, 0.8, 0.9), min_segment_size=100):
    threshold = _last_threshold(agglomeration_thresholds)
    edges = np.ascontiguousarray(edges, dtype=np.int32).reshape(-1, 2)
    counts = np.ascontiguousarray(counts, dtype=np.int64)
    sums = np.ascontiguousarray(sums, dtype=np.uint64)
    sizes = np.ascontiguousarray(sizes, dtype=np.int64)
    if sizes.ndim != 1 or sizes.size < 1 or counts.shape != (edges.shape[0],) or sums.shape != counts.shape:
        raise ValueError("agglomerate needs edges (E, 2), counts (E,), sums (E,) and sizes (K + 1,)")
    table = np.zeros(sizes.size, np.int32)
    n_segments = ctypes.c_int32(0)
    _native.check(
        _native.lib().exaspim_agglomerate(edges.ctypes.data, counts.ctypes.data, sums.ctypes.data, edges.shape[0],
                                          sizes.ctypes.data, sizes.size - 1, float(np.float32(threshold)),
                                          int(min_segment_size), table.ctypes.data, ctypes.addressof(n_segments)),
        "exaspim_agglomerate",
    )
    return table, int(n_segments.value)


def agglomerate_affinities(affinities, agglomeration_thresholds=[0.6, 0.8, 0.9], min_segment_size=100, *,
                           fragment_threshold=0.5, edge_capacity=None, return_device_tensor=False):
    thresholds = list(agglomeration_thresholds)
    _last_threshold(thresholds)
    if isinstance(affinities, np.ndarray):
        if affinities.dtype not in (np.dtype(np.float32), np.dtype(np.float16)):
            raise TypeError(f"affinities must be float32 or float16, got {affinities.dtype}")
        ndim = affinities.ndim
    elif isinstance(affinities, torch.Tensor):
        ndim = affinities.dim()
    else:
        raise TypeError(f"affinities must be a torch tensor or a numpy array, got {type(affinities).__name__}")
    if ndim != 4 or affinities.shape[0] != 3:
        raise ValueError(f"agglomerate_affinities needs (3, D, H, W) affinities, got {tuple(affinities.shape)}; "
                         "a foreground map has no affinities to score")
    if isinstance(affinities, np.ndarray):
        if not torch.cuda.is_available():
            raise RuntimeError("agglomerate_affinities (MI355X) has no CPU path and no HIP device is present")
        affinities = torch.from_numpy(np.ascontiguousarray(affinities)).to("cuda:0")
    affinities = affinities.contiguous()
    labels, count = _components_on_device(affinities, fragment_threshold, 0)
    n_fragments = int(count.cpu()[0])
    edges, counts, sums, sizes = _region_graph_on_device(labels, affinities, n_fragments, edge_capacity)
    table, _ = agglomerate(edges, counts, sums, sizes, thresholds, min_segment_size)
    device = labels.device
    with torch.cuda.device(device):
        table_dev = torch.from_numpy(table).to(device)
        _native.check(
            _native.lib().exaspim_apply_label_table(labels.data_ptr(), labels.numel(), table_dev.data_ptr(),
                                                    table.size, _stream(device)),
            "exaspim_apply_label_table",
        )
    if return_device_tensor:
        return labels
    return labels.cpu().numpy()


DEFAULT_ID_CAPACITY = 1 << 24


class ComponentsStream:

    def __init__(self, shape, threshold=0.5, min_segment_size=100, *, foreground=False, device=None,
                 id_capacity=None):
        shape = tuple(int(v) for v in shape)
        if len(shape) != 3 or min(shape) < 1:
            raise ValueError(f"shape must be a non-empty (D, H, W), got {shape}")
        if shape[1] * shape[2] > 2**31 - 1:
            raise ValueError(f"a plane of {shape[1]} x {shape[2]} voxels exceeds 2^31 - 1")
        device = torch.device("cuda:0" if device is None else device)
        if device.type != "cuda":
            raise RuntimeError(f"ComponentsStream (MI355X) has no CPU path: it needs a HIP device, got {device}")
# ... 29 lines not shown
        return int(self.desc.next_z)

    def _scratch(self, need):
        if self.workspace is None or self.workspace.numel() < need:
            self.workspace = torch.empty(need, dtype=torch.uint8, device=self.device)
        return self.workspace

    def push(self, slab, z0=None, out=None):
        if self.finished:
            raise RuntimeError("ComponentsStream: push() after finish()")
        if not isinstance(slab, torch.Tensor):
            raise TypeError(f"push needs a torch tensor, got {type(slab).__name__}")
        if slab.dtype not in _AFF_CODES:
            raise TypeError(f"slab must be float32 or float16, got {slab.dtype}")
        if slab.device != self.device:
            raise RuntimeError(f"slab is on {slab.device}, the stream on {self.device}")
        want_dims = 3 if self.foreground else 4
        if slab.dim() != want_dims or (not self.foreground and slab.shape[0] != 3):
            raise ValueError("slab must be " + ("(d, H, W)" if self.foreground else "(3, d, H, W)") +
                             f", got {tuple(slab.shape)}")
        dims = tuple(int(v) for v in slab.shape[-3:])
        if min(dims) < 1:
            raise ValueError(f"empty slab {dims}")
        slab = slab.contiguous()
        lib = _native.lib()
        need = lib.exaspim_components_stream_slab_workspace_bytes(_native.int3(dims))
        if need == 0:
            raise ValueError(_native.last_error())
        with torch.cuda.device(self.device):
            if out is None:
                out = torch.empty(dims, dtype=torch.int32, device=self.device)
            elif (out.dtype != torch.int32 or tuple(out.shape) != dims or not out.is_contiguous()
                  or out.device != self.device):
                raise ValueError(f"out must be a contiguous int32 {dims} tensor on {self.device}")
            ws = self._scratch(need)
            _native.check(
                lib.exaspim_components_stream_slab(
                    ctypes.byref(self.desc), slab.data_ptr(), _AFF_CODES[slab.dtype], _native.int3(dims),
                    self.next_z if z0 is None else int(z0), out.data_ptr(), ws.data_ptr(), need,
                    _stream(self.device)),
                "exaspim_components_stream_slab",
            )
        return out

    def finish(self):
        if self.finished:
            raise RuntimeError("ComponentsStream: finish() called twice")
        lib = _native.lib()
        need = lib.exaspim_components_stream_finish_workspace_bytes(self.id_capacity)
        with torch.cuda.device(self.device):
            ws = self._scratch(need)
            _native.check(
                lib.exaspim_components_stream_finish(ctypes.byref(self.desc), ws.data_ptr(), need,
                                                     _stream(self.device)),
                "exaspim_components_stream_finish",
            )
            self.finished = True
            used, overflow, count, _ = (int(v) for v in self.state.cpu())
        if overflow:
            raise RuntimeError(
                f"ComponentsStream: the volume needs more than id_capacity={self.id_capacity} provisional ids; "
                "the labels handed out are unusable. Label it again with a larger id_capacity (or deeper slabs)")
        self.ids_used = used
        return self.table, count

    def apply(self, labels):
        if not self.finished:
            raise RuntimeError("ComponentsStream: apply() before finish()")
        if (not isinstance(labels, torch.Tensor) or labels.dtype != torch.int32 or labels.device != self.device
                or not labels.is_contiguous()):
            raise ValueError(f"apply needs a contiguous int32 tensor on {self.device}")
        with torch.cuda.device(self.device):
            _native.check(
                _native.lib().exaspim_components_stream_apply(ctypes.byref(self.desc), labels.data_ptr(),
                                                              labels.numel(), _stream(self.device)),
                "exaspim_components_stream_apply",
            )
        return labels


def _labels_fit_on_device(device, shape):
    free, _ = torch.cuda.mem_get_info(device)
    return int(np.prod(shape, dtype=np.int64)) * 4 <= free // 4


def _relabel_host_array(cs, result, planes):
    for z0 in range(0, result.shape[0], planes):
        part = torch.from_numpy(result[z0:z0 + planes]).to(cs.device)
        result[z0:z0 + planes] = cs.apply(part).cpu().numpy()


def affinities_to_components_streaming(source, threshold=0.5, min_segment_size=100, *, slab_depth,
                                       write_block=None, id_capacity=None, device=None,
                                       keep_labels_resident=None):
    if not hasattr(source, "shape") or not hasattr(source, "dtype"):
        source = np.asarray(source)
    if np.dtype(source.dtype) not in (np.dtype(np.float32), np.dtype(np.float16)):
        raise TypeError(f"affinities must be float32 or float16, got {source.dtype}")
    shape = tuple(int(v) for v in source.shape)
    if len(shape) == 4 and shape[0] == 3:
        foreground = False
    elif len(shape) == 3:
        foreground = True
    else:
        raise ValueError(f"affinities must be (3, D, H, W) or a (D, H, W) foreground map, got shape {shape}")
    vshape = shape[-3:]
    slab_depth = int(slab_depth)
    if slab_depth < 1:
        raise ValueError(f"slab_depth must be positive, got {slab_depth}")
    if not torch.cuda.is_available():
        raise RuntimeError("affinities_to_components_streaming (MI355X) has no CPU path and no HIP device is present")
    cs = ComponentsStream(vshape, threshold, min_segment_size, foreground=foreground, device=device,
                          id_capacity=id_capacity)
    device = cs.device
    with torch.cuda.device(device):
        if keep_labels_resident is None:
            keep_labels_resident = _labels_fit_on_device(device, vshape)
        resident = result = None
        if write_block is None:
            if keep_labels_resident:
                resident = torch.empty(vshape, dtype=torch.int32, device=device)
            else:
                result = np.empty(vshape, dtype=np.int32)
        for z0 in range(0, vshape[0], slab_depth):
            z1 = min(z0 + slab_depth, vshape[0])
            block = np.asarray(source[..., z0:z1, :, :])
            labels = cs.push(_carrier(block).to(device), z0, None if resident is None else resident[z0:z1])
            if write_block is not None:
                write_block(z0, z1, labels.cpu().numpy())
            elif result is not None:
                result[z0:z1] = labels.cpu().numpy()
        table, count = cs.finish()
        if write_block is not None:
            return table[: cs.ids_used + 1].cpu().numpy(), count
        if resident is not None:
            return cs.apply(resident).cpu().numpy()
        _relabel_host_array(cs, result, slab_depth)
    return result


def _predict_batch(img, model, starts, patch_shape, trim=8, *, clip=None, mn=0.0, mx=1.0):
    device = next(model.parameters()).device
    starts_dev = torch.tensor(list(starts), dtype=torch.int32, device=device).reshape(-1, 3)
    inputs = _get_batch_inputs(img, starts_dev, patch_shape, device, clip=clip, mn=mn, mx=mx)
    outputs = _model_probabilities(model, inputs, trim)
    if trim > 0:
        outputs = outputs[..., trim:-trim, trim:-trim, trim:-trim]
    return outputs


def _get_batch_inputs(img, starts, patch_shape, device, *, clip=None, mn=0.0, mx=1.0, out=None,
                      layout=_native.IN_F32):
    n = int(starts.shape[0])
    border = 0 if layout == _native.IN_F32 else 2
    if out is None:
        shape = (n, 1) + tuple(patch_shape) if border == 0 else (n,) + tuple(int(p) + 2 for p in patch_shape)
        out = torch.empty(shape, dtype=torch.float32, device=device)
    has_clip = clip is not None
    denom = float(np.float64(mx) - np.float64(mn) + 1e-8)
    piece = max(1, 65535 // (int(patch_shape[0]) + border))
    for i in range(0, n, piece):
        m = min(piece, n - i)
        _native.check(
            _native.lib().exaspim_gather_patches_as(
                img.tensor.data_ptr(), img.vox_code, img.block, starts[i:i + m].data_ptr(), m,
                _native.int3(patch_shape), float(clip) if has_clip else 0.0,
                1 if has_clip else 0, float(mn), denom, int(layout), out[i:i + m].data_ptr(),
                _stream(device),
            ),
            "exaspim_gather_patches_as",
        )
    return out


def count_patches(img_shape, patch_shape, overlap):
    assert len(img_shape) == 5, "Image must have shape (1, 1, D, H, W)"
    total = 1
    for axis_range in _start_ranges(img_shape[2:], patch_shape, overlap):
        total *= len(axis_range)
    return total


def generate_patch_starts(img_shape, patch_shape, overlap):
    assert len(img_shape) == 5, "Image must have shape (1, 1, D, H, W)"
    yield from itertools.product(*_start_ranges(img_shape[2:], patch_shape, overlap))


def load_model(path, affinity_mode=True, device="cuda", *, compute_dtype="fp32"):
    output_channels = 3 if affinity_mode else 1
    model = UNet3D(output_channels=output_channels, compute_dtype=compute_dtype)
    state = torch.load(path, map_location=device, weights_only=True)
    model.load_state_dict(state)
    model.to(device)
    model.eval()
    return model


def to_tensor(arr, device="cuda"):
    while arr.ndim < 5:
        arr = arr[:, np.newaxis, ...]
    return torch.tensor(arr).to(device, dtype=torch.float32)


class DeviceVolume:

    def __init__(self, tensor, np_dtype, origin=None, global_shape=None, storage_dtype=None):
        np_dtype = np.dtype(np_dtype)
        storage = np.dtype(storage_dtype) if storage_dtype is not None else _device_voxel_dtype(np_dtype)[0]
        if storage not in _VOX_CODES:
            raise TypeError(_unsupported(np_dtype))
        if tensor.dim() != 3 or not tensor.is_cuda:
            raise ValueError("DeviceVolume expects a 3-D tensor on a HIP device")
        if tensor.element_size() != storage.itemsize:
            raise ValueError("tensor element size does not match the voxel dtype")
        self.tensor = tensor.contiguous()
        self.np_dtype = np_dtype
        self.storage_dtype = storage
        self.vox_code = _VOX_CODES[storage]
        self.shape = tuple(int(v) for v in (global_shape or tensor.shape))
        self.block = _native.Block.make(tuple(tensor.shape), origin, self.shape)

    @classmethod
    def from_array(cls, img, device, clip=None):
        if isinstance(img, DeviceVolume):
            return img
        if isinstance(img, torch.Tensor):
            t = img
            while t.dim() > 3:
                if t.shape[0] != 1:
                    raise ValueError("leading image axes must have length 1")
                t = t[0]
            np_dtype = {
                torch.uint8: np.uint8, torch.int16: np.int16, torch.float32: np.float32,
                torch.float64: np.float64, getattr(torch, "uint16", None): np.uint16,
            }.get(t.dtype)
            if np_dtype is None:
                raise TypeError(f"tensor dtype {t.dtype} not supported")
            return cls(t.to(device), np_dtype)
        arr = np.asarray(img)
        while arr.ndim > 3:
            if arr.shape[0] != 1:
                raise ValueError("leading image axes must have length 1")
            arr = arr[0]
        if arr.ndim != 3:
            raise ValueError(f"expected a 3-D image, got shape {np.shape(img)}")
        storage, convert = _device_voxel_dtype(arr.dtype, whole=arr, clip=clip)
        if storage not in _VOX_CODES:
            raise TypeError(_unsupported(arr.dtype))
        return cls(_carrier(convert(arr)).to(device), arr.dtype, storage_dtype=storage)


def _unsupported(np_dtype):
    return (f"voxel dtype {np_dtype} not supported (8-, 16-, 32- and 64-bit integers, float32 and "
            "float64 are; 64-bit integers must be exactly representable in float64)")


class SlidingWindow:

    def __init__(self, shape, patch_shape, overlap, trim):
        self.shape = tuple(int(v) for v in shape)
        self.patch_shape = tuple(int(v) for v in patch_shape)
        self.overlap = tuple(int(v) for v in overlap)
        self.trim = int(trim)
        if len(self.patch_shape) != 3 or len(self.overlap) != 3:
            raise ValueError("patch_shape and overlap must have three entries")
        if any(o >= p or o < 0 for o, p in zip(self.overlap, self.patch_shape)):
            raise ValueError("overlap must be in [0, patch_shape)")
        if self.trim < 0 or any(2 * self.trim >= p for p in self.patch_shape):
            raise ValueError("trim must satisfy 0 <= 2 * trim < patch_shape")
        self.window = _native.Window.make(self.patch_shape, self.overlap, self.trim)
        self.shape5 = (1, 1) + self.shape
        n_starts = [len(range(0, d - ov, ps - ov))
                    for d, ps, ov in zip(self.shape, self.patch_shape, self.overlap)]
        if self.trim > 0 and len(self.shape) == 3 and all(n_starts):
            for axis, (d, ps, ov) in enumerate(zip(self.shape, self.patch_shape, self.overlap)):
                out = ps - 2 * self.trim
                for s0 in reversed(range(0, d - ov, ps - ov)):
                    if s0 + self.trim <= d:
                        break
                    if s0 + self.trim < d + out:
                        raise ValueError(
                            "operands could not be broadcast together: the patch starting at "
                            f"{s0} on axis {axis} begins {s0 + self.trim - d} voxel(s) past the "
                            f"image (size {d}) after trimming {self.trim}; the reference's stitch "
                            "loop fails on this geometry (trim > overlap + 1)"
                        )

    def starts(self):
        return list(generate_patch_starts(self.shape5, self.patch_shape, self.overlap))


def batch_row_stride(starts, patch_shape, overlap):
    stride = int(patch_shape[2]) - int(overlap[2])
    if len(starts) < 2 or stride <= 0:
        return 0
    z0, y0, x0 = (int(v) for v in starts[0])
    for i, s in enumerate(starts):
        z, y, x = (int(v) for v in s)
        if z != z0 or y != y0 or x != x0 + i * stride:
            return 0
    return stride


def batch_keep_hi(starts, patch_shape, trim, global_shape):
    trim = int(trim)
    keep = []
    for axis in range(3):
        full = int(patch_shape[axis]) - trim
        hi = min(full, max(int(global_shape[axis]) - int(s[axis]) for s in starts))
        if hi <= trim:
            hi = full
        keep.append(hi)
    if trim <= 0 or all(k == int(p) - trim for k, p in zip(keep, patch_shape)):
        return None
    return tuple(keep)


def _start_ranges(dims, patch_shape, overlap):
    return [
        range(0, d - ps + (ps - ov), ps - ov)
        for d, ps, ov in zip(dims, patch_shape, overlap)
    ]


def _stream(device):
    return torch.cuda.current_stream(device).cuda_stream


_WORKER_STREAMS = {}


def _worker_streams(device, n):
    pool = _WORKER_STREAMS.setdefault(str(device), [])
    while len(pool) < n:
        pool.append(torch.cuda.Stream(device))
    return pool[:n]


def _effective_clip(np_dtype, brightness_clip, storage_dtype=None):
    np_dtype = np.dtype(np_dtype)
    if brightness_clip is None:
        return None, np_dtype
    probe = np.minimum(np.zeros(1, dtype=np_dtype), brightness_clip)
    if probe.dtype == np_dtype:
        return np_dtype.type(brightness_clip), np_dtype
    if probe.dtype.kind in "iu" and np_dtype.kind in "iu":
        info, c = np.iinfo(np_dtype), int(brightness_clip)
        if c < info.min:
            raise NotImplementedError(f"brightness_clip {brightness_clip!r} lies below every {np_dtype} voxel")
        return (None if c >= info.max else np_dtype.type(c)), probe.dtype
    if probe.dtype != np.float64:
        raise NotImplementedError(
            f"brightness_clip {brightness_clip!r} promotes {np_dtype} voxels to {probe.dtype}"
        )
    clip = np.float64(brightness_clip)
    if np_dtype.kind in "iu" and clip < np.iinfo(np_dtype).min:
        raise NotImplementedError(f"brightness_clip {brightness_clip!r} lies below every {np_dtype} voxel")
    storage = np.dtype(storage_dtype) if storage_dtype is not None else _device_voxel_dtype(np_dtype)[0]
    if storage == np.float32 and np_dtype != np.float32 and np.float64(np.float32(clip)) != clip:
        raise NotImplementedError(
            f"brightness_clip {brightness_clip!r} is not a float32 number (the volume travels as float32)"
        )
    return clip, np.dtype(np.float64)


def _histogram_into(hist, tensor, vox_code, clip, pass_index=0, prefix=0):
    if vox_code == _native.VOX_F64:
        _native.check(
            _native.lib().exaspim_histogram_wide(
                tensor.data_ptr(), vox_code, tensor.numel(),
                float(clip) if clip is not None else 0.0, 1 if clip is not None else 0,
                pass_index, int(prefix), hist.data_ptr(), _stream(tensor.device),
            ),
            "exaspim_histogram_wide",
        )
        return
    _native.check(
        _native.lib().exaspim_histogram(
            tensor.data_ptr(), vox_code, tensor.numel(),
            float(clip) if clip is not None else 0.0, 1 if clip is not None else 0,
            pass_index, prefix, hist.data_ptr(), _stream(tensor.device),
        ),
        "exaspim_histogram",
    )


def volume_histogram(volume, clip, pass_index=0, prefix=0):
    hist = torch.zeros(65536, dtype=torch.int64, device=volume.tensor.device)
    _histogram_into(hist, volume.tensor, volume.vox_code, clip, pass_index, prefix)
    return hist


def _key_to_f32(key):
    key = np.uint32(key)
    bits = (key & np.uint32(0x7FFFFFFF)) if key & np.uint32(0x80000000) else ~key
    return np.array([bits], dtype=np.uint32).view(np.float32)[0]


def _key_to_f64(key):
    key = int(key)
    bits = (key & 0x7FFFFFFFFFFFFFFF) if key >> 63 else (~key & 0xFFFFFFFFFFFFFFFF)
    return np.array([bits], dtype=np.uint64).view(np.float64)[0]


def _percentiles_from_histograms(histogram, storage_dtype, percentiles, value_dtype=None, clip=None):
    storage_dtype = np.dtype(storage_dtype)
    value_dtype = np.dtype(value_dtype) if value_dtype is not None else storage_dtype

    def as_value(v):
        if clip is not None and np.float64(v) > np.float64(clip):
            return value_dtype.type(clip)
        return value_dtype.type(v)

    if storage_dtype.kind in "ui":
        offset = 32768 if storage_dtype == np.int16 else 0
        stats = img_util.OrderStatistics(histogram(), lambda b: as_value(b - offset))
    elif storage_dtype == np.float64:
        levels = {}

        def level(p, prefix):
            if (p, prefix) not in levels:
                levels[(p, prefix)] = img_util.OrderStatistics(histogram(p, prefix), lambda b: b)
            return levels[(p, prefix)]

        class _F64Stats:
            n = level(0, 0).n

            @staticmethod
            def kth(k):
                prefix, rank = 0, k
                for p in range(4):
                    b, rank = level(p, prefix).bin_of_rank(rank)
                    prefix = (prefix << 16) | b
                return as_value(_key_to_f64(prefix))

        stats = _F64Stats()
    else:
        coarse = img_util.OrderStatistics(histogram(0), lambda b: b)
        fine = {}

        class _F32Stats:
            n = coarse.n

            @staticmethod
            def kth(k):
                hi, within = coarse.bin_of_rank(k)
                if hi not in fine:
                    fine[hi] = img_util.OrderStatistics(histogram(1, hi), lambda b: b)
                lo, _ = fine[hi].bin_of_rank(within)
                return as_value(_key_to_f32((hi << 16) | lo))

        stats = _F32Stats()
    mn, mx = img_util.percentiles_from_statistics(stats, percentiles, value_dtype)
    return mn, mx


def volume_percentiles(volume, brightness_clip, percentiles, reduce_fn=None):
    clip, value_dtype = _effective_clip(volume.np_dtype, brightness_clip, volume.storage_dtype)

    def histogram(pass_index=0, prefix=0):
        hist = volume_histogram(volume, clip, pass_index, prefix)
        if reduce_fn is not None:
            reduce_fn(hist)
        return hist.cpu().numpy()

    return _percentiles_from_histograms(histogram, volume.storage_dtype, percentiles, value_dtype, clip)


def _model_probabilities(model, inputs, trim=0, out=None):
    if isinstance(model, UNet3D):
        if FULL_PATCHES:
            trim = 0
        return model.run(inputs, apply_sigmoid=True, trim=trim, out=out)
    with torch.no_grad():
        return torch.sigmoid(model(inputs)).to(torch.float32).contiguous()


def stitch_accumulate(pred, starts_dev, plan, accum, block):
    n = int(starts_dev.shape[0])
    piece = max(1, 65535 // max(1, plan.patch_shape[0] - 2 * plan.trim))
    for i in range(0, n, piece):
        m = min(piece, n - i)
        _native.check(
            _native.lib().exaspim_stitch_accumulate(
                pred[i:i + m].data_ptr(), starts_dev[i:i + m].data_ptr(), m,
                int(accum.shape[0]), plan.window, accum.data_ptr(), block,
                _stream(accum.device),
            ),
            "exaspim_stitch_accumulate",
        )


def stitch_finalize(accum, plan, block):
    _native.check(
        _native.lib().exaspim_stitch_finalize(
            accum.data_ptr(), int(accum.shape[0]), plan.window, block, _stream(accum.device)
        ),
        "exaspim_stitch_finalize",
    )


def run_sliding_window(volume, model, plan, n_channels, batch_size, brightness_clip,
                       mn, mx, starts=None, accum=None, accum_block=None, verbose=False,
                       n_streams=1, pbar=None):
    device = volume.tensor.device
    clip, _ = _effective_clip(volume.np_dtype, brightness_clip, volume.storage_dtype)
    if starts is None:
        starts = plan.starts()
    if accum_block is None:
        accum_block = volume.block
    if accum is None:
        accum = torch.zeros((n_channels,) + tuple(accum_block.dims), dtype=torch.float32,
                            device=device)
    if len(starts) == 0:
        return accum
    if any(p % 16 for p in plan.patch_shape):
        raise RuntimeError(
            "Sizes of tensors must match: patch_shape entries must be multiples of 16, "
            f"got {plan.patch_shape}"
        )
    starts_dev = torch.tensor(starts, dtype=torch.int32, device=device).reshape(-1, 3)
    batch_size = max(1, min(int(batch_size), 65535 // (max(plan.patch_shape) + 2)))
    own_pbar = pbar is None and verbose and tqdm is not None
    if own_pbar:
        pbar = tqdm(total=len(starts), desc="Predict")
    main = torch.cuda.current_stream(device)
    n_streams = max(1, min(int(n_streams), -(-len(starts) // batch_size)))
    workers = _worker_streams(device, n_streams) if n_streams > 1 else [main]
    for s in workers:
        s.wait_stream(main)
    if isinstance(model, UNet3D) and model.needs_resolution():
        probe = _get_batch_inputs(volume, starts_dev[:batch_size], plan.patch_shape, device, clip=clip,
                                  mn=mn, mx=mx)
        model.resolve_compute_dtype(probe)
        del probe
    prepared_layout = None
    if isinstance(model, UNet3D) and not PLAIN_GATHER:
        prepared_layout = model.input_layout(device)
    for bi, i in enumerate(range(0, len(starts), batch_size)):
        batch = starts_dev[i:i + batch_size]
        row_stride = batch_row_stride(starts[i:i + batch_size], plan.patch_shape, plan.overlap)
        keep_hi = None
        if CLIP_TO_VOLUME and not FULL_PATCHES:
            keep_hi = batch_keep_hi(starts[i:i + batch_size], plan.patch_shape, plan.trim, plan.shape)
        worker = workers[bi % n_streams]
        with torch.cuda.stream(worker):
            if prepared_layout is not None:
                inputs = _get_batch_inputs(volume, batch, plan.patch_shape, device, clip=clip,
                                           mn=mn, mx=mx, layout=prepared_layout)
                pred = model.run_prepared(
                    inputs, (int(batch.shape[0]),) + tuple(plan.patch_shape), apply_sigmoid=True,
                    trim=0 if FULL_PATCHES else plan.trim, row_stride=row_stride, keep_hi=keep_hi)
            else:
                inputs = _get_batch_inputs(volume, batch, plan.patch_shape, device, clip=clip,
                                           mn=mn, mx=mx)
                pred = _model_probabilities(model, inputs, plan.trim)
        if pred.shape[1] != n_channels:
            raise RuntimeError(
                f"model produced {pred.shape[1]} channels, expected {n_channels}"
            )
        if worker is not main:
            main.wait_stream(worker)
            pred.record_stream(main)
        stitch_accumulate(pred, batch, plan, accum, accum_block)
        if pbar is not None:
            pbar.update(int(batch.shape[0]))
    if own_pbar:
        pbar.close()
    return accum


_COPY_STREAMS = {}
_PINNED_LOCK = threading.Lock()
_PINNED_FREE = {}
PINNED_SLOT_BYTES = 512 << 20


def _checkout_pinned(device, count, numel, dtype):
    key = (str(device), dtype)
    with _PINNED_LOCK:
        free = _PINNED_FREE.setdefault(key, [])
        free.sort(key=lambda t: t.numel())
        taken = []
        while free and len(taken) < count and free[-1].numel() >= numel:
            taken.append(free.pop())
    while len(taken) < count:
        try:
            taken.append(torch.empty(numel, dtype=dtype, pin_memory=True))
        except RuntimeError:
            taken.append(torch.empty(numel, dtype=dtype))
    return taken


def _return_pinned(device, dtype, buffers):
    with _PINNED_LOCK:
        _PINNED_FREE.setdefault((str(device), dtype), []).extend(b for b in buffers if b.is_pinned())


def release_pinned_buffers():
    with _PINNED_LOCK:
        _PINNED_FREE.clear()


def _copy_stream(device):
    key = str(device)
    with _PINNED_LOCK:
        if key not in _COPY_STREAMS:
            _COPY_STREAMS[key] = torch.cuda.Stream(device)
        return _COPY_STREAMS[key]


class _SlabDrain:

    N_SLOTS = 3

    def __init__(self, device, slot_elems, half_out, threads, label_elems=0):
        self.device = device
        self.half_out = half_out
        self.main = torch.cuda.current_stream(device)
        self.copy_stream = _copy_stream(device)
        self.host_dtype = torch.int32 if label_elems else torch.float16 if half_out else torch.float32
        n = self.N_SLOTS
        self.dev_labels = [torch.empty(label_elems, dtype=torch.int32, device=device) for _ in range(n)
                           if label_elems]
        self.dev_out = [torch.empty(slot_elems, dtype=torch.float32, device=device) for _ in range(n)]
        self.dev_half = ([torch.empty(slot_elems, dtype=torch.float16, device=device) for _ in range(n)]
                         if half_out else None)
        self.host = _checkout_pinned(device, n, label_elems or slot_elems, self.host_dtype)
        self.pool = ThreadPoolExecutor(max_workers=max(1, int(threads)))
        self.pending = [[] for _ in range(n)]
        self.n_emitted = 0

    def emit(self, shape, fill, consumers, label=None):
        slot = self.n_emitted % self.N_SLOTS
        self.n_emitted += 1
        for f in self.pending[slot]:
            f.result()
        count = int(np.prod(shape))
        out = self.dev_out[slot][:count].view(shape)
        out.zero_()
        fill(out)
        if label is not None:
            out = label(out, self.dev_labels[slot])
            if out is None:
                self.pending[slot] = []
                return
            shape, count = tuple(out.shape), out.numel()
        elif self.half_out:
            out = export_half(out, self.dev_half[slot][:count]).view(shape)
        ready, done = torch.cuda.Event(), torch.cuda.Event()
        ready.record(self.main)
        with torch.cuda.stream(self.copy_stream):
            self.copy_stream.wait_event(ready)
            self.host[slot][:count].view(shape).copy_(out, non_blocking=True)
            done.record(self.copy_stream)
        view = self.host[slot][:count].numpy().reshape(shape)

        def after_download(job):
            def run():
                done.synchronize()
                job()
            return run

        self.pending[slot] = [self.pool.submit(after_download(job)) for job in consumers(view)]

    def drain(self):
        for jobs in self.pending:
            for f in jobs:
                f.result()
        self.pending = [[] for _ in range(self.N_SLOTS)]

    def close(self):
        self.pool.shutdown(wait=True)
        _return_pinned(self.device, self.host_dtype, self.host)
        self.host = []


class _ArraySource:

    def __init__(self, arr):
        while len(arr.shape) > 3:
            if arr.shape[0] != 1:
                raise ValueError("leading image axes must have length 1")
            arr = arr[0]
        if len(arr.shape) != 3:
            raise ValueError(f"expected a 3-D image, got shape {tuple(arr.shape)}")
        self.arr = arr
        self.shape = tuple(int(v) for v in arr.shape)
        self.dtype = np.dtype(arr.dtype)

    def __call__(self, lo, hi):
        return np.asarray(self.arr[tuple(slice(a, b) for a, b in zip(lo, hi))])


def _plane_reader(read_block, shape):
    def read_box(lo, hi):
        block = read_block(lo[0], hi[0])
        if tuple(block.shape) != (hi[0] - lo[0],) + tuple(shape[1:]):
            raise ValueError(f"read_block({lo[0]}, {hi[0]}) returned shape {tuple(block.shape)}")
        return block[:, lo[1]:hi[1], lo[2]:hi[2]]
    return read_box


def _device_voxel_dtype(np_dtype, whole=None, clip=None):
    np_dtype = np.dtype(np_dtype)
    if np_dtype == np.int8:
        return np.dtype(np.int16), lambda block: block.astype(np.int16)
    if np_dtype.kind in "iuf" and np_dtype.itemsize in (4, 8) and np_dtype != np.float32:
        clip_ok = clip is None or np.float64(np.float32(clip)) == np.float64(clip)
        if whole is not None and clip_ok:
            as32 = np.asarray(whole).astype(np.float32)
            if np.array_equal(as32.astype(np_dtype), whole):
                def to_f32(block):
                    b32 = block.astype(np.float32)
                    if not np.array_equal(b32.astype(np_dtype), block):
                        raise TypeError(f"{np_dtype} volume is not exactly representable in float32")
                    return b32
                return np.dtype(np.float32), to_f32

        def to_f64(block):
            b64 = block.astype(np.float64)
            if np_dtype.kind in "iu" and np_dtype.itemsize == 8 and not np.array_equal(b64.astype(np_dtype), block):
                raise TypeError(f"{np_dtype} volume is not exactly representable in float64")
            return b64
        return np.dtype(np.float64), to_f64
    if np_dtype in _VOX_CODES:
        return np_dtype, lambda block: block
    return np_dtype, lambda block: block


def _carrier(block):
    block = np.ascontiguousarray(block)
    if not block.flags.writeable:
        block = block.copy()
    if block.dtype == np.uint16:
        block = block.view(np.int16)
    return torch.from_numpy(block)


class DeviceShardOps:

    def __init__(self, model, plan, n_channels, batch_size, brightness_clip, n_streams, half_out,
                 copy_threads):
        self.model, self.plan = model, plan
        self.n_channels, self.batch_size = n_channels, batch_size
        self.brightness_clip, self.n_streams = brightness_clip, n_streams
        self.half_out, self.copy_threads = half_out, copy_threads
        self.device = _hip_device(model)

    def storage(self, src_dtype, whole=None):
        vdtype, convert = _device_voxel_dtype(src_dtype, whole=whole, clip=self.brightness_clip)
        if vdtype not in _VOX_CODES:
            raise TypeError(_unsupported(src_dtype))
        return vdtype, convert

    def upload(self, block, convert):
        return _carrier(convert(block))

    def empty_voxels(self, dims, vdtype):
        return torch.empty(tuple(dims), dtype=_TORCH_VOXELS[np.dtype(vdtype)], device=self.device)

    def effective_clip(self, src_dtype, vdtype):
        return _effective_clip(src_dtype, self.brightness_clip, vdtype)

    def histogram_into(self, hist, voxels, vdtype, clip, pass_index, prefix):
        _histogram_into(hist, voxels.contiguous(), _VOX_CODES[np.dtype(vdtype)], clip, pass_index, prefix)

    def percentiles(self, histogram, vdtype, percentiles, value_dtype, clip):
        return _percentiles_from_histograms(histogram, vdtype, percentiles, value_dtype, clip)

    def run_layer(self, voxels, vox_origin, src_dtype, vdtype, starts, accum, accum_origin, mn, mx, pbar=None):
        gshape = self.plan.shape
        volume = DeviceVolume(voxels, src_dtype, vox_origin, gshape, storage_dtype=vdtype)
        blk = _native.Block.make(tuple(accum.shape[1:]), accum_origin, gshape)
        run_sliding_window(volume, self.model, self.plan, self.n_channels, self.batch_size,
                           self.brightness_clip, mn, mx, starts=starts, accum=accum,
                           accum_block=blk, n_streams=self.n_streams, pbar=pbar)

    def finalize(self, out, origin):
        stitch_finalize(out, self.plan, _native.Block.make(tuple(out.shape[1:]), origin, self.plan.shape))

    def zeros(self, shape):
        return torch.zeros(tuple(shape), dtype=torch.float32, device=self.device)

    def empty(self, shape):
        return torch.empty(tuple(shape), dtype=torch.float32, device=self.device)

    def slab_bytes_cap(self):
        return PINNED_SLOT_BYTES

    def make_drain(self, slot_elems, threads, label_elems=0):
        return _SlabDrain(self.device, slot_elems, self.half_out, threads, label_elems=label_elems)

    def synchronize(self):
        torch.cuda.synchronize(self.device)


class _WholeVolume:

    def __init__(self, plan):
        self.plan = plan
        ranges = _start_ranges(plan.shape, plan.patch_shape, plan.overlap)
        self.yx_starts = list(itertools.product(*ranges[1:]))
        self.z_starts = list(ranges[0]) if self.yx_starts else []
        self.input_origin = self.core_origin = self.accum_origin = self.own_lo = (0, 0, 0)
        self.input_dims = self.core_dims = self.accum_dims = self.own_hi = plan.shape


def run_slab_pipeline(ops, shard, read_box, src_dtype, storage, normalization_percentiles, *,
                      affinity_mode=True, write_block=None, result=None, label=None, copy_threads=4,
                      keep_input_resident=None, exchanges=None, progress=None, timings=None):
    plan = shard.plan
    vdtype, convert = storage
    n_channels = 3 if affinity_mode else 1
    D, H, W = plan.shape
    pz, trim = plan.patch_shape[0], plan.trim
    stride = pz - plan.overlap[0]
    z_starts, yx_starts = shard.z_starts, shard.yx_starts
    in_lo = shard.input_origin
    in_hi = tuple(o + d for o, d in zip(in_lo, shard.input_dims))
    core_lo = shard.core_origin
    core_hi = tuple(o + d for o, d in zip(core_lo, shard.core_dims))
    acc_lo = shard.accum_origin
    AH, AW = shard.accum_dims[1], shard.accum_dims[2]
    own_lo, own_hi = shard.own_lo, shard.own_hi
    own_dims = tuple(h - l for l, h in zip(own_lo, own_hi))
    res4 = None if result is None else result.reshape((-1,) + own_dims)

    def read(lo, hi):
        block = read_box(tuple(lo), tuple(hi))
        if tuple(block.shape) != tuple(h - l for l, h in zip(lo, hi)):
            raise ValueError(f"read_box({tuple(lo)}, {tuple(hi)}) returned shape {tuple(block.shape)}")
        return ops.upload(block, convert)

    in_plane_bytes = shard.input_dims[1] * shard.input_dims[2] * np.dtype(vdtype).itemsize
    if keep_input_resident is None:
        keep_input_resident = False
        if ops.device.type == "cuda":
            free, _ = torch.cuda.mem_get_info(ops.device)
            keep_input_resident = shard.input_dims[0] * in_plane_bytes <= free // 4
    chunk = max(1, min(shard.input_dims[0], max(stride, (256 << 20) // max(in_plane_bytes, 1))))
    resident = ops.empty_voxels(shard.input_dims, vdtype) if keep_input_resident else None
    clip, value_dtype = ops.effective_clip(src_dtype, vdtype)
    loaded = [False]

    def core_chunks():
        z_lo, z_hi = (in_lo[0], in_hi[0]) if resident is not None else (core_lo[0], core_hi[0])
        for z0 in range(z_lo, z_hi, chunk):
            z1 = min(z0 + chunk, z_hi)
            if resident is None:
                yield read((z0, core_lo[1], core_lo[2]), (z1, core_hi[1], core_hi[2])).to(ops.device, non_blocking=True)
                continue
            if not loaded[0]:
                resident[z0 - in_lo[0]:z1 - in_lo[0]].copy_(read((z0, in_lo[1], in_lo[2]), (z1, in_hi[1], in_hi[2])),
                                                            non_blocking=True)
# ... 263 lines not shown
```

### aind_exaspim_neuron_segmentation_amd/machine_learning/unet3d.py

```python

import ctypes
import math
import warnings

import numpy as np
import torch
from torch import nn

from aind_exaspim_neuron_segmentation_amd import _native
from aind_exaspim_neuron_segmentation_amd.machine_learning.spec import (
    unet_channels,
    unet_layer_specs,
)


class _Holder(nn.Module):
    """Anonymous node of the parameter tree (no computation of its own)."""


class _ConvParams(nn.Module):

    def __init__(self, cin, cout, k):
        super().__init__()
        self.weight = nn.Parameter(torch.empty(cout, cin, k, k, k))
        self.bias = nn.Parameter(torch.empty(cout))
        bound = 1.0 / math.sqrt(cin * k ** 3)
        nn.init.uniform_(self.weight, -bound, bound)
        nn.init.uniform_(self.bias, -bound, bound)


class _ConvTransposeParams(nn.Module):

    def __init__(self, cin, cout, k):
        super().__init__()
        self.weight = nn.Parameter(torch.empty(cin, cout, k, k, k))
        self.bias = nn.Parameter(torch.empty(cout))
        bound = 1.0 / math.sqrt(cout * k ** 3)
        nn.init.uniform_(self.weight, -bound, bound)
        nn.init.uniform_(self.bias, -bound, bound)


class _NormParams(nn.Module):

    def __init__(self, c):
        super().__init__()
        self.weight = nn.Parameter(torch.ones(c))
        self.bias = nn.Parameter(torch.zeros(c))
        self.register_buffer("running_mean", torch.zeros(c))
        self.register_buffer("running_var", torch.ones(c))
        self.register_buffer("num_batches_tracked", torch.tensor(0, dtype=torch.long))


def _attach(root, dotted, module):
    node = root
    parts = dotted.split(".")
    for name in parts[:-1]:
        if name not in node._modules:
            node.add_module(name, _Holder())
        node = node._modules[name]
    node.add_module(parts[-1], module)


class UNet3D(nn.Module):

    AUTO_TOLERANCE = 1e-3
    AUTO_HEADROOM = 2.0
    HALF_MAX = 65504.0

    def __init__(self, output_channels=1, trilinear=True, width_multiplier=1,
                 compute_dtype="fp32"):
        super().__init__()
        if compute_dtype != "auto" and compute_dtype not in _native.DTYPE_CODES:
            raise ValueError(f"unknown compute_dtype {compute_dtype!r}")
        self.channels = unet_channels(width_multiplier)
        self.trilinear = trilinear
        self.output_channels = output_channels
        self.compute_dtype = compute_dtype
        layers, (head_in, head_out) = unet_layer_specs(
            output_channels, trilinear, width_multiplier
        )
        for kind, prefix, *widths in layers:
            if kind == "conv_transpose":
                cin, cout = widths
                _attach(self, prefix, _ConvTransposeParams(cin, cout, 2))
                continue
            cin, cmid, cout = widths
            _attach(self, f"{prefix}.0", _ConvParams(cin, cmid, 3))
            _attach(self, f"{prefix}.1", _NormParams(cmid))
            _attach(self, f"{prefix}.3", _ConvParams(cmid, cout, 3))
            _attach(self, f"{prefix}.4", _NormParams(cout))
        _attach(self, "outc.conv", _ConvParams(head_in, head_out, 1))
        self._engines = {}
        self._resolved = None
        self._resolved_key = None
        self.auto_report = None
        self._workspace = None
        self.engine_options = 0

    def _canonical_params(self):
        chunks = []
        for key, value in self.state_dict().items():
            if key.endswith("num_batches_tracked"):
                continue
            chunks.append(value.detach().to("cpu", torch.float32).reshape(-1))
        return torch.cat(chunks).contiguous().numpy()

    def _state_key(self, device, dtype):
        tensors = list(self.parameters()) + list(self.buffers())
        return (
            str(device), dtype,
            tuple((t.data_ptr(), t._version) for t in tensors),
        )

    def active_dtype(self):
        if self.compute_dtype == "auto":
            return self._resolved or "fp32"
        return self.compute_dtype

    @property
    def _engine(self):
        entry = self._engines.get(self.active_dtype())
        return entry["handle"] if entry else None

    def _release_engine(self):
        for entry in self._engines.values():
            _native.lib().exaspim_unet_destroy(entry["handle"])
        self._engines = {}

    def __del__(self):
        try:
            self._release_engine()
        except Exception:
            pass

    def _ensure_engine(self, device, dtype=None):
        dtype = dtype or self.active_dtype()
        key = self._state_key(device, dtype)
        entry = self._engines.get(dtype)
        if entry is not None and key == entry["key"]:
            return self._apply_options(dtype)
        if entry is not None:
            _native.lib().exaspim_unet_destroy(entry["handle"])
            del self._engines[dtype]
        lib = _native.lib()
        ch = _native.channels_array(self.channels)
        code = _native.DTYPE_CODES[dtype]
        if not self.trilinear:
            code |= _native.UP_CONVT
        params = self._canonical_params()
        expected = lib.exaspim_unet_param_count(ch, self.output_channels, code)
        if expected == 0:
            raise ValueError(f"unsupported network: {_native.last_error()}")
        if params.size != expected:
            raise RuntimeError(
                f"parameter vector has {params.size} values, extension expects {expected}"
            )
        nbytes = lib.exaspim_unet_packed_bytes(ch, self.output_channels, code)
        packed = np.empty(nbytes, dtype=np.uint8)
        _native.check(
            lib.exaspim_unet_pack_weights(
                ch, self.output_channels, code, params.ctypes.data, params.size,
                packed.ctypes.data, nbytes,
            ),
            "exaspim_unet_pack_weights",
        )
        packed_dev = torch.from_numpy(packed).to(device)
        handle = ctypes.c_void_p()
        index = device.index if device.index is not None else torch.cuda.current_device()
        _native.check(
            lib.exaspim_unet_create(
                ch, self.output_channels, code, index, packed_dev.data_ptr(), nbytes,
                ctypes.byref(handle),
            ),
            "exaspim_unet_create",
        )
        self._engines[dtype] = {"handle": handle, "packed": packed_dev, "key": key, "options": 0}
        return self._apply_options(dtype)

    def _apply_options(self, dtype):
        entry = self._engines[dtype]
        if entry["options"] != self.engine_options:
            _native.check(_native.lib().exaspim_unet_set_options(entry["handle"], int(self.engine_options)),
                          "exaspim_unet_set_options")
            entry["options"] = self.engine_options
        return entry["handle"]

    def _get_workspace(self, n, d, h, w, device, stream):
        need = _native.lib().exaspim_unet_workspace_bytes(self._engine, n, d, h, w)
        if need == 0:
            raise RuntimeError(
                "Sizes of tensors must match: " + _native.last_error()
            )
        if self._workspace is None:
            self._workspace = {}
        key = (str(device), stream)
        ws = self._workspace.get(key)
        if ws is None or ws.numel() < need:
            self._workspace.pop(key, None)
            ws = torch.empty(need, dtype=torch.uint8, device=device)
            self._workspace[key] = ws
        return ws

    def _forward_absmax(self, x, dtype):
        device = x.device
        n, _, d, h, w = x.shape
        with torch.cuda.device(device):
            handle = self._ensure_engine(device, dtype)
            stream = torch.cuda.current_stream(device).cuda_stream
            need = _native.lib().exaspim_unet_workspace_bytes(handle, n, d, h, w)
            if need == 0:
                raise RuntimeError("Sizes of tensors must match: " + _native.last_error())
            ws = torch.empty(need, dtype=torch.uint8, device=device)
            out = torch.empty((n, self.output_channels, d, h, w), dtype=torch.float32, device=device)
            absmax = torch.zeros(22, dtype=torch.float32, device=device)
            _native.check(
                _native.lib().exaspim_unet_forward_absmax(
                    handle, x.data_ptr(), out.data_ptr(), n, d, h, w, 1, absmax.data_ptr(),
                    ws.data_ptr(), ws.numel(), stream),
                "exaspim_unet_forward_absmax",
            )
        return out, absmax

    def fp16_report(self, x):
        if x.dim() != 5 or x.shape[1] != 1 or not x.is_cuda:
            raise RuntimeError(f"expected a (B, 1, D, H, W) tensor on a HIP device, got {tuple(x.shape)} on {x.device}")
        x = x.to(torch.float32).contiguous()
        p32, r32 = self._forward_absmax(x, "fp32")
        p16, r16 = self._forward_absmax(x, "fp16")
        diff = float((p16 - p32).abs().max().item())
        r32, r16 = r32.cpu().numpy(), r16.cpu().numpy()
        return {
            "max_abs_diff": diff,
            "fp32_absmax": [float(v) for v in r32],
            "fp16_absmax": [float(v) for v in r16],
            "fp32_peak": float(np.nanmax(r32)) if np.isfinite(r32).any() else float("nan"),
            "saturated": bool((r16 >= self.HALF_MAX).any()),
            "finite": bool(np.isfinite(r32).all() and np.isfinite(r16).all() and np.isfinite(diff)),
            "patches": int(x.shape[0]),
        }

    def needs_resolution(self):
        if self.compute_dtype != "auto":
            return False
        if self._resolved is not None and self._resolved_key != self._state_key(
                next(self.parameters()).device, "auto"):
            self._resolved, self.auto_report = None, None
        return self._resolved is None

    def resolve_compute_dtype(self, x):
        if self.compute_dtype != "auto":
            return self.compute_dtype
        rep = self.fp16_report(x)
        reasons = []
        if not rep["finite"]:
            reasons.append("non-finite activations")
        if rep["saturated"]:
            reasons.append("a half-precision store saturated at 65504")
        if rep["fp32_peak"] * self.AUTO_HEADROOM > self.HALF_MAX:
            reasons.append(f"float32 activations reach {rep['fp32_peak']:.4g} (less than a factor "
                           f"{self.AUTO_HEADROOM:g} below 65504)")
        if not rep["max_abs_diff"] <= self.AUTO_TOLERANCE:
            reasons.append(f"fp16 probabilities deviate by {rep['max_abs_diff']:.3g} > {self.AUTO_TOLERANCE:g}")
        self._resolved = "fp32" if reasons else "fp16"
        self._resolved_key = self._state_key(x.device, "auto")
        rep["chosen"], rep["reasons"] = self._resolved, reasons
        self.auto_report = rep
        if reasons:
            warnings.warn("UNet3D(compute_dtype='auto'): falling back to float32 -- " + "; ".join(reasons),
                          RuntimeWarning, stacklevel=2)
        return self._resolved

    def run(self, x, apply_sigmoid=False, out=None, trim=0):
        if self.training:
            raise RuntimeError(
                "UNet3D (MI355X) implements eval-mode inference only; call .eval()"
            )
        if not x.is_cuda:
            raise RuntimeError(
                "UNet3D (MI355X) has no CPU path: move the input to a HIP device"
            )
        if x.dim() != 5 or x.shape[1] != 1:
            raise RuntimeError(f"expected input of shape (B, 1, D, H, W), got {tuple(x.shape)}")
        x = x.to(torch.float32).contiguous()
        n, _, d, h, w = x.shape
        if d % 16 or h % 16 or w % 16:
            raise RuntimeError(
                "Sizes of tensors must match: patch dimensions must be multiples of 16, "
                f"got {(d, h, w)}"
            )
        device = x.device
        with torch.cuda.device(device):
            self._ensure_engine(device)
            stream = torch.cuda.current_stream(device).cuda_stream
            ws = self._get_workspace(n, d, h, w, device, stream)
            if out is None:
                out = torch.empty(
                    (n, self.output_channels, d, h, w), dtype=torch.float32, device=device
                )
            _native.check(
                _native.lib().exaspim_unet_forward_trimmed(
                    self._engine, x.data_ptr(), out.data_ptr(), n, d, h, w,
                    1 if apply_sigmoid else 0, int(trim), ws.data_ptr(), ws.numel(), stream,
                ),
                "exaspim_unet_forward_trimmed",
            )
        return out

    def input_layout(self, device=None):
        device = next(self.parameters()).device if device is None else device
        with torch.cuda.device(device):
            self._ensure_engine(device)
        code = _native.lib().exaspim_unet_input_layout(self._engine)
        if code < 0:
            raise RuntimeError("exaspim_unet_input_layout failed")
        return int(code)

    def run_prepared(self, prepared, shape, apply_sigmoid=False, out=None, trim=0, row_stride=0, keep_hi=None):
        if self.training:
            raise RuntimeError(
                "UNet3D (MI355X) implements eval-mode inference only; call .eval()"
            )
        n, d, h, w = (int(v) for v in shape)
        if (not prepared.is_cuda or not prepared.is_contiguous() or prepared.element_size() != 4
                or tuple(prepared.shape) != (n, d + 2, h + 2, w + 2)):
            raise RuntimeError(
                f"prepared input must be a contiguous 4-byte device tensor of shape {(n, d + 2, h + 2, w + 2)}"
            )
        if d % 16 or h % 16 or w % 16:
            raise RuntimeError(
                "Sizes of tensors must match: patch dimensions must be multiples of 16, "
                f"got {(d, h, w)}"
            )
        device = prepared.device
        with torch.cuda.device(device):
            self._ensure_engine(device)
            stream = torch.cuda.current_stream(device).cuda_stream
            ws = self._get_workspace(n, d, h, w, device, stream)
            if out is None:
                out = torch.empty(
                    (n, self.output_channels, d, h, w), dtype=torch.float32, device=device
                )
            if keep_hi is not None:
                _native.check(
                    _native.lib().exaspim_unet_forward_prepared_clipped(
                        self._engine, prepared.data_ptr(), out.data_ptr(), n, d, h, w,
                        1 if apply_sigmoid else 0, int(trim), int(row_stride), _native.int3(keep_hi),
                        ws.data_ptr(), ws.numel(), stream,
                    ),
                    "exaspim_unet_forward_prepared_clipped",
                )
            elif row_stride > 0:
                _native.check(
                    _native.lib().exaspim_unet_forward_prepared_row(
                        self._engine, prepared.data_ptr(), out.data_ptr(), n, d, h, w,
                        1 if apply_sigmoid else 0, int(trim), int(row_stride), ws.data_ptr(), ws.numel(),
                        stream,
                    ),
                    "exaspim_unet_forward_prepared_row",
                )
            else:
                _native.check(
                    _native.lib().exaspim_unet_forward_prepared(
                        self._engine, prepared.data_ptr(), out.data_ptr(), n, d, h, w,
                        1 if apply_sigmoid else 0, int(trim), ws.data_ptr(), ws.numel(), stream,
                    ),
                    "exaspim_unet_forward_prepared",
                )
        return out

    def forward(self, x):
        return self.run(x, apply_sigmoid=False)
```

### include/exaspim_affinity.h

```cpp
#ifndef EXASPIM_AFFINITY_H
#define EXASPIM_AFFINITY_H

#include <stddef.h>
#include <stdint.h>

#ifdef __cplusplus
extern "C" {
#endif

#define EXASPIM_ABI_VERSION 5

#define EXASPIM_OK 0
#define EXASPIM_E_INVALID (-1)
#define EXASPIM_E_HIP (-2)
#define EXASPIM_E_WORKSPACE (-3)
#define EXASPIM_E_NODEVICE (-4)

#define EXASPIM_DT_F32 0
#define EXASPIM_DT_BF16 1
#define EXASPIM_DT_F16 2
#define EXASPIM_DT_BF16X3 3
#define EXASPIM_UP_CONVT 0x100

#define EXASPIM_VOX_U8 0
#define EXASPIM_VOX_U16 1
#define EXASPIM_VOX_I16 2
#define EXASPIM_VOX_F32 3
#define EXASPIM_VOX_F64 4

typedef struct exaspim_unet exaspim_unet;

typedef struct exaspim_block {
    int32_t dims[3];
    int32_t origin[3];
    int32_t global[3];
} exaspim_block;

typedef struct exaspim_window {
    int32_t patch[3];
    int32_t overlap[3];
    int32_t trim;
} exaspim_window;

int exaspim_abi_version(void);
const char* exaspim_last_error(void);


size_t exaspim_unet_param_count(const int32_t channels[5], int32_t out_channels,
                                int32_t dtype);

size_t exaspim_unet_packed_bytes(const int32_t channels[5], int32_t out_channels,
                                 int32_t dtype);

int exaspim_unet_pack_weights(const int32_t channels[5], int32_t out_channels,
                              int32_t dtype, const float* params, size_t n_params,
                              void* packed_host, size_t packed_bytes);

int exaspim_unet_create(const int32_t channels[5], int32_t out_channels,
                        int32_t dtype, int32_t device, const void* packed_dev,
                        size_t packed_bytes, exaspim_unet** out);
void exaspim_unet_destroy(exaspim_unet* h);

size_t exaspim_unet_workspace_bytes(const exaspim_unet* h, int32_t n, int32_t d,
                                    int32_t hgt, int32_t w);

int exaspim_unet_forward(exaspim_unet* h, const float* x_dev, float* out_dev,
                         int32_t n, int32_t d, int32_t hgt, int32_t w,
                         int32_t apply_sigmoid, void* workspace_dev,
                         size_t workspace_bytes, void* stream);

int exaspim_unet_forward_trimmed(exaspim_unet* h, const float* x_dev, float* out_dev,
                                 int32_t n, int32_t d, int32_t hgt, int32_t w,
                                 int32_t apply_sigmoid, int32_t trim, void* workspace_dev,
                                 size_t workspace_bytes, void* stream);

int exaspim_unet_input_layout(const exaspim_unet* h);
int exaspim_unet_forward_prepared(exaspim_unet* h, const void* x_prepared_dev, float* out_dev,
                                  int32_t n, int32_t d, int32_t hgt, int32_t w,
                                  int32_t apply_sigmoid, int32_t trim, void* workspace_dev,
                                  size_t workspace_bytes, void* stream);
int exaspim_unet_forward_prepared_row(exaspim_unet* h, const void* x_prepared_dev, float* out_dev,
                                      int32_t n, int32_t d, int32_t hgt, int32_t w,
                                      int32_t apply_sigmoid, int32_t trim, int32_t row_stride,
                                      void* workspace_dev, size_t workspace_bytes, void* stream);
int exaspim_unet_forward_prepared_clipped(exaspim_unet* h, const void* x_prepared_dev, float* out_dev,
                                          int32_t n, int32_t d, int32_t hgt, int32_t w,
                                          int32_t apply_sigmoid, int32_t trim, int32_t row_stride,
                                          const int32_t keep_hi[3], void* workspace_dev,
                                          size_t workspace_bytes, void* stream);

#define EXASPIM_ABSMAX_SLOTS 22
int exaspim_unet_forward_absmax(exaspim_unet* h, const float* x_dev, float* out_dev,
                                int32_t n, int32_t d, int32_t hgt, int32_t w,
                                int32_t apply_sigmoid, float* absmax_dev, void* workspace_dev,
                                size_t workspace_bytes, void* stream);

#define EXASPIM_OPT_SEPARATE_POOL 1u
#define EXASPIM_OPT_SEPARATE_DEEP_POOLS 2u
#define EXASPIM_OPT_PLAIN_UPSAMPLE 4u
#define EXASPIM_OPT_FIRST_PER_GROUP 8u
#define EXASPIM_OPT_UPSAMPLE_PER_THREAD 16u
#define EXASPIM_OPT_PER_PATCH_ENCODER 32u
#define EXASPIM_OPT_SEPARATE_HEAD 64u
#define EXASPIM_OPT_ROW_SEPARATE_BORDERS 256u
int exaspim_unet_set_options(exaspim_unet* h, uint32_t options);

int exaspim_unet_timing_begin(exaspim_unet* h, uint32_t conv_mask);
int exaspim_unet_timing_read(exaspim_unet* h, double ms_sum[17], int32_t count[17]);


int exaspim_histogram(const void* vol_dev, int32_t vox_dtype, size_t n,
                      double clip, int32_t has_clip, int32_t pass,
                      uint32_t prefix, uint64_t* hist_dev, void* stream);

int exaspim_histogram_wide(const void* vol_dev, int32_t vox_dtype, size_t n,
                           double clip, int32_t has_clip, int32_t pass,
                           uint64_t prefix, uint64_t* hist_dev, void* stream);

#define EXASPIM_IN_F32 0
#define EXASPIM_IN_PADDED_F32 1
#define EXASPIM_IN_PADDED_SPLIT_F16 2
#define EXASPIM_IN_PADDED_SPLIT_BF16 3
int exaspim_gather_patches_as(const void* vol_dev, int32_t vox_dtype,
                              const exaspim_block* blk, const int32_t* starts_dev,
                              int32_t n, const int32_t patch[3], double clip,
                              int32_t has_clip, double mn, double denom, int32_t layout,
                              void* out_dev, void* stream);
int exaspim_gather_patches(const void* vol_dev, int32_t vox_dtype,
                           const exaspim_block* blk, const int32_t* starts_dev,
                           int32_t n, const int32_t patch[3], double clip,
                           int32_t has_clip, double mn, double denom,
                           float* out_dev, void* stream);


int exaspim_stitch_accumulate(const float* pred_dev, const int32_t* starts_dev,
                              int32_t n, int32_t channels,
                              const exaspim_window* win, float* accum_dev,
                              const exaspim_block* blk, void* stream);

int exaspim_stitch_finalize(float* accum_dev, int32_t channels,
                            const exaspim_window* win, const exaspim_block* blk,
                            void* stream);

int exaspim_export_f16(const float* src_dev, void* dst_dev, size_t n, void* stream);


#define EXASPIM_AFF_F32 0
#define EXASPIM_AFF_F16 1

size_t exaspim_components_workspace_bytes(const int32_t dims[3]);

int exaspim_components(const void* aff_dev, int32_t aff_dtype, int32_t channels,
                       const int32_t dims[3], float threshold, int64_t min_size,
                       int32_t* labels_dev, int32_t* n_segments_dev, void* workspace_dev,
                       size_t workspace_bytes, void* stream);

typedef struct exaspim_components_stream {
    int32_t dims[3];
    int32_t channels;
    float threshold;
    int32_t capacity;
    int64_t min_size;
    int32_t next_z;
    int32_t reserved;
    int32_t* id_parent_dev;
    int64_t* id_count_dev;
    int32_t* table_dev;
    int32_t* state_dev;
    int32_t* seam_ids_dev;
    uint8_t* seam_bits_dev;
} exaspim_components_stream;

size_t exaspim_components_stream_slab_workspace_bytes(const int32_t slab_dims[3]);

size_t exaspim_components_stream_finish_workspace_bytes(int32_t capacity);

int exaspim_components_stream_slab(exaspim_components_stream* st, const void* aff_dev, int32_t aff_dtype,
                                   const int32_t slab_dims[3], int32_t z0, int32_t* labels_dev,
                                   void* workspace_dev, size_t workspace_bytes, void* stream);

int exaspim_components_stream_finish(const exaspim_components_stream* st, void* workspace_dev,
                                     size_t workspace_bytes, void* stream);

int exaspim_components_stream_apply(const exaspim_components_stream* st, int32_t* labels_dev, size_t n,
                                    void* stream);


size_t exaspim_region_graph_workspace_bytes(const int32_t dims[3], int32_t n_labels, int64_t edge_capacity);

int exaspim_region_graph(const int32_t* labels_dev, const void* aff_dev, int32_t aff_dtype,
                         const int32_t dims[3], int32_t n_labels, int64_t edge_capacity,
                         int32_t* edges_dev, int64_t* count_dev, uint64_t* sum_dev, int64_t* sizes_dev,
                         int32_t* n_edges_dev, void* workspace_dev, size_t workspace_bytes, void* stream);

int exaspim_agglomerate(const int32_t* edges, const int64_t* counts, const uint64_t* sums, int64_t n_edges,
                        const int64_t* sizes, int32_t n_labels, float threshold, int64_t min_size,
                        int32_t* table, int32_t* n_segments);

int exaspim_apply_label_table(int32_t* labels_dev, size_t n, const int32_t* table_dev, int32_t table_len,
                              void* stream);


int exaspim_synth_volume_u16(uint16_t* vol_dev, const exaspim_block* blk,
                             uint64_t seed, void* stream);

int exaspim_synth_volume_neurite_u16(uint16_t* vol_dev, const exaspim_block* blk,
                                     uint64_t seed, void* stream);

#ifdef __cplusplus
}
#endif
#endif
```

Measured before the change: 819.6 million voxels/s.

## Carry first-layer skip and pool planes between z-overlapping batches to skip recompute

Adds a carry mechanism in row mode. The first encoder conv writes the z-planes that overlap the next batch's patches into a side buffer, shifted by the z offset. The next batch then skips the z-tiles already covered by that buffer. This removes redundant first-layer conv work in the overlap region between neighbouring patches, at the cost of extra stores, buffer pools, cross-stream events and a more complex schedule. The later outputs depend on the carried planes matching what would have been recomputed, which holds because the same input voxels are used.

```diff
diff --git a/aind_exaspim_neuron_segmentation_amd/_native.py b/aind_exaspim_neuron_segmentation_amd/_native.py
--- a/aind_exaspim_neuron_segmentation_amd/_native.py
+++ b/aind_exaspim_neuron_segmentation_amd/_native.py
@@ -77,6 +77,20 @@
         ("state_dev", ctypes.c_void_p),
         ("seam_ids_dev", ctypes.c_void_p),
         ("seam_bits_dev", ctypes.c_void_p),
+    ]
+
+
+class UNetCarry(ctypes.Structure):
+
+    _fields_ = [
+        ("own_skip", ctypes.c_void_p),
+        ("own_pool", ctypes.c_void_p),
+        ("in_z", ctypes.c_int32 * 2),
+        ("out_skip", ctypes.c_void_p),
+        ("out_pool", ctypes.c_void_p),
+        ("out_z", ctypes.c_int32 * 2),
+        ("out_shift", ctypes.c_int32),
+        ("reserved", ctypes.c_int32),
     ]
 
 
@@ -108,6 +122,10 @@
         _i32, [_vp, _vp, _vp, _i32, _i32, _i32, _i32, _i32, _i32, _i32, _vp, _sz, _vp]),
     "exaspim_unet_forward_prepared_clipped": (
         _i32, [_vp, _vp, _vp, _i32, _i32, _i32, _i32, _i32, _i32, _i32, _I32x3, _vp, _sz, _vp]),
+    "exaspim_unet_carry_planes": (_i32, [_vp, _i32, _i32, _i32, _i32, _i32, _i32, ctypes.c_int32 * 2]),
+    "exaspim_unet_forward_prepared_carry": (
+        _i32, [_vp, _vp, _vp, _i32, _i32, _i32, _i32, _i32, _i32, _i32, _I32x3, ctypes.POINTER(UNetCarry), _vp,
+               _sz, _vp]),
     "exaspim_unet_forward_absmax": (
         _i32, [_vp, _vp, _vp, _i32, _i32, _i32, _i32, _i32, _vp, _vp, _sz, _vp]),
     "exaspim_unet_set_options": (_i32, [_vp, ctypes.c_uint32]),
diff --git a/aind_exaspim_neuron_segmentation_amd/csrc/common.h b/aind_exaspim_neuron_segmentation_amd/csrc/common.h
--- a/aind_exaspim_neuron_segmentation_amd/csrc/common.h
+++ b/aind_exaspim_neuron_segmentation_amd/csrc/common.h
@@ -163,8 +163,8 @@
     const void* src_b;
     int ca, cb;
     const void* weights;
-    const void* weights_paired = nullptr;
-    const void* weights_k32 = nullptr;
+    void* carry_dst = nullptr;
+    void* carry_pool_dst = nullptr;
     const float* bias;
     void* dst;
     int cout;
@@ -179,9 +179,12 @@
     int ext[3] = {0, 0, 0};
     void* pool_dst = nullptr;
     int row_stride = 0;
+    unsigned short in_z0 = 0, in_z1 = 0;
     float* partial = nullptr;
     size_t partial_patch_bytes = 0;
     int ksplit = 1;
+    unsigned char out_z0 = 0, out_z1 = 0;
+    unsigned short out_shift = 0;
 #ifdef EXASPIM_TRACE
     unsigned long long* trace = nullptr;
 #endif
@@ -191,6 +194,7 @@
     const char* config = "";
     int ksplit = 0;
     bool row = false;
+    bool carry = false;
 };
 ConvLaunchRecord& last_conv_launch();
 const char*& last_layer_kernel();
@@ -208,6 +212,10 @@
 constexpr int kRowStageBorders = 8;
 constexpr int kRowStagesFused = kRowStageMain | kRowStageBorders;
 int launch_conv3x3x3_row(int dtype, const ConvArgs& a, int stages, hipStream_t stream);
+int conv_zcol_tile_depth(int d);
+#ifndef EXASPIM_TRACE
+static_assert(sizeof(ConvArgs) == 184, "ConvArgs: the carry fields fill padding, the argument block keeps its size");
+#endif
 
 int launch_conv_first(int dtype, const float* x, float* xpad, const float* w, const float* bias,
                       void* dst, int n, int d, int h, int wd, int c0p, float slope,
diff --git a/aind_exaspim_neuron_segmentation_amd/csrc/conv3d.hip b/aind_exaspim_neuron_segmentation_amd/csrc/conv3d.hip
--- a/aind_exaspim_neuron_segmentation_amd/csrc/conv3d.hip
+++ b/aind_exaspim_neuron_segmentation_amd/csrc/conv3d.hip
@@ -59,6 +59,10 @@
     return ks;
 }
 
+static bool conv_has_carry(const ConvArgs& a) {
+    return a.carry_dst || a.carry_pool_dst || a.in_z0 || a.in_z1 || a.out_z0 || a.out_z1;
+}
+
 template <typename Tag, int TZ, int TY, int TX, int MINW, int D, int HEAD = 0, bool POOL = false>
 static int launch_zpipe(const ConvArgs& a, hipStream_t stream) {
     const bool row = POOL && HEAD == 0 && Tag::kG == 8 && a.row_stride > 0;
@@ -66,6 +70,11 @@
     if (int rc = row ? tile_grid(a, TZ, TY, TX, a.n * a.row_stride + a.w - a.row_stride, 1, g)
                      : tile_grid(a, TZ, TY, TX, a.ext[2], a.n, g))
         return rc;
+    const bool carry = row && conv_has_carry(a);
+    if (carry) {
+        g.tz -= (a.in_z1 - a.in_z0) / TZ;
+        g.blocks = (long long)g.tz * g.ty * g.tx;
+    }
     const int tz = g.tz, ty = g.ty, tx = g.tx;
     const long long blocks = g.blocks;
     const int slices = a.cout / 32;
@@ -79,6 +88,12 @@
     dim3 grid((unsigned)wgs, slices);
     last_conv_launch() = {__PRETTY_FUNCTION__, 1};
     if constexpr (POOL && HEAD == 0 && Tag::kG == 8) {
+        if (carry) {
+            last_conv_launch().carry = true;
+            conv3x3x3_zpipe_rowz<Tag, TZ, TY, TX, MINW, D><<<grid, TY * TX * 2, 0, stream>>>(a, tz, ty, tx);
+            EXA_CHECK_HIP(hipGetLastError());
+            return EXASPIM_OK;
+        }
         if (row) {
             last_conv_launch().row = true;
             conv3x3x3_zpipe_row<Tag, TZ, TY, TX, MINW, D><<<grid, TY * TX * 2, 0, stream>>>(a, tz, ty, tx);
@@ -177,7 +192,7 @@
                     case 4: return launch_zpipe<Tag, kHeadTZ, 8, 16, 2, 4, 4>(a, stream);
                 }
             }
-            if (a.d % 6 == 0) return launch_zpipe_d<Tag, 6>(a, stream);
+            if (conv_zcol_tile_depth(a.d) == 6) return launch_zpipe_d<Tag, 6>(a, stream);
             return launch_zpipe_d<Tag, 4>(a, stream);
         }
         if (a.pool_dst) return launch_cfg_pool<Tag, 4, 8, 16, 4, 1, 4, 2, 2>(a, stream);
@@ -283,6 +298,8 @@
     return EXASPIM_OK;
 }
 
+int conv_zcol_tile_depth(int d) { return d % 6 == 0 ? 6 : 4; }
+
 int conv_zcol_main_extent(int ext, int axis) {
     const int tile = axis == 1 ? 8 : 16;
     const int rem = ext % tile;
@@ -303,6 +320,17 @@
                   "conv: row mode needs a 16-bit fused-pool z-column layer, whole patches, n >= 2 and "
                   "an overlap that is a multiple of 32 and at most the stride (w %d, stride %d, n %d)",
                   a.w, a.row_stride, a.n);
+    const int tzd = conv_zcol_tile_depth(a.d);
+    EXA_CHECK_ARG(a.in_z0 <= a.in_z1 && a.in_z0 % 2 == 0 && a.in_z1 % 2 == 0 && a.in_z0 % tzd == 0 && a.in_z1 % tzd == 0 &&
+                      (a.in_z0 == a.in_z1 || (a.in_z0 >= 2 && a.in_z1 <= a.d - 2)),
+                  "conv: carry in [%d, %d) must be whole %d-plane tiles with even bounds inside [2, %d)", (int)a.in_z0,
+                  (int)a.in_z1, tzd, a.d - 2);
+    const bool out = a.carry_dst || a.carry_pool_dst || a.out_z0 || a.out_z1;
+    EXA_CHECK_ARG(!out || (a.carry_dst && a.carry_pool_dst && a.out_z0 < a.out_z1 && a.out_z0 % 2 == 0 && a.out_z1 % 2 == 0 &&
+                           a.out_z0 >= 2 && a.out_z1 <= a.d - 2 && a.out_shift > 0 && a.out_shift % 2 == 0 &&
+                           (int)a.out_z0 - a.out_shift >= 2),
+                  "conv: carry out [%d, %d) shifted by %d needs both targets, even bounds and source and target planes "
+                  "inside [2, %d)", (int)a.out_z0, (int)a.out_z1, a.out_shift, a.d - 2);
     return EXASPIM_OK;
 }
 
@@ -330,6 +358,7 @@
                   "float32: a 32-cout-slice layer)");
     EXA_CHECK_ARG(!a.head_out || conv_can_fuse_head(a.cout, a.w, a.head_oc, dtype),
                   "conv: fused head needs cout 32, w %% 16 == 0, 1..4 outputs (and not bf16x3)");
+    EXA_CHECK_ARG(a.row_stride > 0 || !conv_has_carry(a), "conv: carried planes need row mode");
     if (a.row_stride > 0)
         if (int rc = check_row_args(dtype, a)) return rc;
     switch (dtype) {
@@ -378,7 +407,8 @@
 int launch_conv3x3x3_thin(int dtype, const ConvArgs& a_in, hipStream_t stream) {
     ConvArgs a = a_in;
     if (int rc = check_conv_args(dtype, a, kCheckPadded | kCheckEmpty)) return rc;
-    EXA_CHECK_ARG(!a.pool_dst && !a.head_out && a.row_stride == 0, "conv: thin tiles have no fused pool, head or row mode");
+    EXA_CHECK_ARG(!a.pool_dst && !a.head_out && a.row_stride == 0 && !conv_has_carry(a),
+                  "conv: thin tiles have no fused pool, head, row mode or carried planes");
     if (int rc = resolve_region(a)) return rc;
     a.partial = nullptr;
     switch (dtype) {
@@ -426,6 +456,9 @@
     if (stages & kRowStageMain) r = launch_conv3x3x3(dtype, a, stream);
     b.pool_dst = nullptr;
     b.row_stride = 0;
+    b.carry_dst = b.carry_pool_dst = nullptr;
+    b.in_z0 = b.in_z1 = b.out_z0 = b.out_z1 = 0;
+    b.out_shift = 0;
     b.n = a.n - 1;
     b.ext[2] = 2;
     if (r == EXASPIM_OK && (stages & kRowStageThin)) {
@@ -446,6 +479,9 @@
         r = check_conv_args(dtype, a, kCheckPadded);
         ConvArgs c = a;
         for (int i = 0; i < 3; ++i) { c.org[i] = b.org[i]; c.ext[i] = b.ext[i]; }
+        c.carry_dst = c.carry_pool_dst = nullptr;
+        c.in_z0 = c.in_z1 = c.out_z0 = c.out_z1 = 0;
+        c.out_shift = 0;
         c.org[2] = 0;
         if (r == EXASPIM_OK)
             r = dtype == EXASPIM_DT_F16 ? launch_row_borders<F16Tag>(c, stream) : launch_row_borders<BF16Tag>(c, stream);
diff --git a/aind_exaspim_neuron_segmentation_amd/csrc/conv_zcol.h b/aind_exaspim_neuron_segmentation_amd/csrc/conv_zcol.h
--- a/aind_exaspim_neuron_segmentation_amd/csrc/conv_zcol.h
+++ b/aind_exaspim_neuron_segmentation_amd/csrc/conv_zcol.h
@@ -4,7 +4,7 @@
 
 namespace exaspim {
 
-template <typename Tag, int TZ, int TY, int TX, int MINW, int D, int HEAD, bool POOL, bool ROW>
+template <typename Tag, int TZ, int TY, int TX, int MINW, int D, int HEAD, bool POOL, bool ROW, bool CARRY = false>
 __device__ __forceinline__ void zpipe_body(const ConvArgs& a, int tiles_z, int tiles_y, int tiles_x) {
     constexpr int G = Tag::kG;
     constexpr int KC = 2 * G;
@@ -44,6 +44,7 @@
 
     constexpr bool row = ROW;
     static_assert(!ROW || (POOL && ES == 2 && HEAD == 0), "row mode: 16-bit fused-pool epilogue");
+    static_assert(!CARRY || ROW, "carry: row mode only");
     const int total = tiles_z * tiles_y * tiles_x * (row ? 1 : a.n);
     int t_first, t_count, t_step;
     {
@@ -67,7 +68,9 @@
         const int nb = min(max(rx - ho, 0) / s, a.n - 1);
         t.x0 = __builtin_amdgcn_readfirstlane(rx - nb * s);
         t.y0 = __builtin_amdgcn_readfirstlane((id % tiles_y) * TY); id /= tiles_y;
-        t.z0 = __builtin_amdgcn_readfirstlane((id % tiles_z) * TZ);
+        int tz = id % tiles_z;
+        if (CARRY && tz >= a.in_z0 / TZ) tz += (a.in_z1 - a.in_z0) / TZ;
+        t.z0 = __builtin_amdgcn_readfirstlane(tz * TZ);
         t.nb = __builtin_amdgcn_readfirstlane(nb);
         return t;
     };
@@ -101,7 +104,12 @@
         s_slot[k] = q < REM * HZ ? kg * GS + hz * PLANE + (c / HX) * HXP + c % HX : -1;
     }
     auto set_offsets = [&](const Tile& t) {
-        {
+        if constexpr (CARRY) {
+            const int ft = wave * 64 + fresh_lane();
+            const int gy = t.y0 + (ft >> 1) / HX - 1, gx = t.x0 + (ft >> 1) % HX - 1;
+            const bool in = ft < NPAIR && (unsigned)gy < (unsigned)a.h && (unsigned)gx < (unsigned)a.w;
+            p_voff = in ? (unsigned)(gy * a.w + gx) * 32u + (ft & 1) * 16u : kOutOfRange;
+        } else {
             const int gy = t.y0 + p_hy - 1, gx = t.x0 + p_hx - 1;
             const bool in = p_ok && (unsigned)gy < (unsigned)a.h && (unsigned)gx < (unsigned)a.w;
             p_voff = in ? (unsigned)(gy * a.w + gx) * 32u + p_kg * 16u : kOutOfRange;
@@ -367,6 +375,12 @@
             char* const nplane = static_cast<char*>(a.dst) + nbase +
                                  ((size_t)nnb * (a.cout / KC) + ntile0 * 2) * patch_vox * 32;
             const size_t nbytes = (size_t)((long long)2 * patch_vox * 32 - nbase);
+            const bool cout_on = CARRY && a.carry_dst != nullptr;
+            const long long cshift = (long long)a.out_shift * plane_vox * 32;
+            char* const cplane = static_cast<char*>(a.carry_dst) - cshift +
+                                 ((size_t)cur.nb * (a.cout / KC) + ntile0 * 2) * patch_vox * 32;
+            char* const cnplane = static_cast<char*>(a.carry_dst) - cshift + nbase +
+                                  ((size_t)nnb * (a.cout / KC) + ntile0 * 2) * patch_vox * 32;
 #pragma unroll
             for (int zp = 0; zp < TZ / 2; ++zp) {
                 uint2 grp[2][4];
@@ -394,6 +408,14 @@
                         buf_store16(rec, orsrc, ovoff, ((unsigned)ck * (unsigned)patch_vox + (unsigned)gz * (unsigned)plane_vox) * 32u);
                         if (shared)
                             buf_store16(rec, nrsrc, nlane ? ovoff : kOutOfRange, ((unsigned)ck * (unsigned)patch_vox + (unsigned)gz * (unsigned)plane_vox) * 32u);
+                        if (CARRY && cout_on) {
+                            const bool cz = gz >= a.out_z0 && gz < a.out_z1;
+                            buf_store16(rec, make_rsrc(cplane, cz ? (size_t)2 * patch_vox * 32 : (size_t)0), ovoff,
+                                        ((unsigned)ck * (unsigned)patch_vox + (unsigned)gz * (unsigned)plane_vox) * 32u);
+                            if (shared)
+                                buf_store16(rec, make_rsrc(cnplane, cz ? nbytes : (size_t)0), nlane ? ovoff : kOutOfRange,
+                                            ((unsigned)ck * (unsigned)patch_vox + (unsigned)gz * (unsigned)plane_vox) * 32u);
+                        }
                     }
                 }
             }
@@ -409,6 +431,11 @@
                 char* const npplane = static_cast<char*>(a.pool_dst) + nbase / 2 +
                                       ((size_t)nnb * (a.cout / KC) + ntile0 * CPT) * pvox * 32;
                 const __amdgpu_buffer_rsrc_t nprsrc = make_rsrc(npplane, (size_t)((long long)CPT * pvox * 32 - nbase / 2));
+                const long long cpshift = (long long)(a.out_shift >> 1) * ph * pw2 * 32;
+                char* const cpplane = static_cast<char*>(a.carry_pool_dst) - cpshift +
+                                      ((size_t)cur.nb * (a.cout / KC) + ntile0 * CPT) * pvox * 32;
+                char* const cnpplane = static_cast<char*>(a.carry_pool_dst) - cpshift + nbase / 2 +
+                                       ((size_t)nnb * (a.cout / KC) + ntile0 * CPT) * pvox * 32;
 #pragma unroll
                 for (int p0 = 0; p0 < NP; p0 += 64) {
                     const int p = p0 + lane_e;
@@ -430,6 +457,15 @@
                     if (shared) {
                         const int nqx = qx + nshift / 2;
                         buf_store16(m, nprsrc, nqx >= 1 && nqx < pw2 - 1 ? pvoff : kOutOfRange, 0u);
+                    }
+                    if (CARRY && cout_on) {
+                        const unsigned cpvoff = 2 * qz >= a.out_z0 && 2 * qz < a.out_z1 ? pvoff : kOutOfRange;
+                        buf_store16(m, make_rsrc(cpplane, (size_t)CPT * pvox * 32), cpvoff, 0u);
+                        if (shared) {
+                            const int nqx = qx + nshift / 2;
+                            buf_store16(m, make_rsrc(cnpplane, (size_t)((long long)CPT * pvox * 32 - nbase / 2)),
+                                        nqx >= 1 && nqx < pw2 - 1 ? cpvoff : kOutOfRange, 0u);
+                        }
                     }
                 }
             }
@@ -539,4 +575,10 @@
     zpipe_body<Tag, TZ, TY, TX, MINW, D, 0, true, true>(a, tiles_z, tiles_y, tiles_x);
 }
 
+template <typename Tag, int TZ, int TY, int TX, int MINW, int D>
+__global__ __launch_bounds__(TY* TX * 2, MINW) void conv3x3x3_zpipe_rowz(
+    ConvArgs a, int tiles_z, int tiles_y, int tiles_x) {
+    zpipe_body<Tag, TZ, TY, TX, MINW, D, 0, true, true, true>(a, tiles_z, tiles_y, tiles_x);
 }
+
+}
diff --git a/aind_exaspim_neuron_segmentation_amd/csrc/engine.hip b/aind_exaspim_neuron_segmentation_amd/csrc/engine.hip
--- a/aind_exaspim_neuron_segmentation_amd/csrc/engine.hip
+++ b/aind_exaspim_neuron_segmentation_amd/csrc/engine.hip
@@ -45,6 +45,15 @@
     if (i == 0) return 0;
     if (i <= 8) return (i + 1) / 2;
     return 3 - (i - 9) / 2;
+}
+
+static void carry_span(int d, int shift_z, int32_t out[2]) {
+    out[0] = out[1] = 0;
+    if (shift_z <= 0 || shift_z % 2 != 0 || shift_z >= d) return;
+    const int tz = conv_zcol_tile_depth(d);
+    const int step = tz % 2 == 0 ? tz : 2 * tz;
+    const int lo = (2 + step - 1) / step * step, hi = (d - shift_z - 2) / step * step;
+    if (lo < hi && hi + shift_z <= 254) { out[0] = lo; out[1] = hi; }
 }
 
 static Workspace make_workspace(const UNetPlan& p, int n, int d, int h, int w) {
@@ -73,7 +82,7 @@
 static int forward(exaspim_unet* e, const float* x, float* out, int n, int d, int h, int w,
                    int apply_sigmoid, int trim, void* workspace, size_t workspace_bytes,
                    hipStream_t stream, const void* x_prepared = nullptr, float* absmax = nullptr,
-                   int row_stride = 0, const int32_t* keep_hi = nullptr) {
+                   int row_stride = 0, const int32_t* keep_hi = nullptr, const exaspim_unet_carry* carry = nullptr) {
     const UNetPlan& p = e->plan;
     const Workspace ws = make_workspace(p, n, d, h, w);
     if (workspace_bytes < ws.bytes) {
@@ -103,12 +112,36 @@
         fuse_pool[l] = !separate_pool && !(separate_deep && l > 0) && conv_can_fuse_pool(p.dtype, p.conv[2 * l].cout, d >> l, h >> l, w >> l);
     const bool row = !absmax && !(e->options & EXASPIM_OPT_PER_PATCH_ENCODER) &&
                      conv_row_mode_ok(dt, p.conv[0].cout, n, w, row_stride, fuse_pool[0]);
+    if (carry) {
+        int32_t span[2];
+        const int shift = carry->out_skip ? carry->out_shift : 0;
+        const bool in = carry->in_z[0] != 0 || carry->in_z[1] != 0;
+        EXA_CHECK_ARG(row && carry->own_skip && carry->own_pool && carry->reserved == 0,
+                      "forward: carried planes need row mode at this geometry and both own buffers");
+        EXA_CHECK_ARG(!carry->out_skip == !carry->out_pool, "forward: carry out needs both targets or neither");
+        const int tzd = conv_zcol_tile_depth(d);
+        if (in)
+            EXA_CHECK_ARG(carry->in_z[0] >= 2 && carry->in_z[0] < carry->in_z[1] && carry->in_z[1] <= d - 2 &&
+                              carry->in_z[0] % tzd == 0 && carry->in_z[1] % tzd == 0 && carry->in_z[0] % 2 == 0 &&
+                              carry->in_z[1] % 2 == 0,
+                          "forward: carry in [%d, %d) is not whole %d-plane tiles with even bounds inside [2, %d)",
+                          carry->in_z[0], carry->in_z[1], tzd, d - 2);
+        if (shift || carry->out_skip) {
+            carry_span(d, shift, span);
+            EXA_CHECK_ARG(shift > 0 && span[0] < span[1] && carry->out_z[0] == span[0] + shift &&
+                              carry->out_z[1] == span[1] + shift && carry->out_z[1] <= 254,
+                          "forward: carry out [%d, %d) shifted by %d is not the range a forward %d planes down takes over",
+                          carry->out_z[0], carry->out_z[1], shift, shift);
+        }
+    }
+    void* const x1 = carry ? carry->own_skip : skip(0);
+    void* const x1_pool = carry ? carry->own_pool : A(1);
     auto conv = [&](int idx, const void* sa, const void* sb, void* dst, int l) -> int {
         const ConvLayer& L = p.conv[idx];
         ConvArgs a;
         a.partial = reinterpret_cast<float*>(base + ws.xpad);
         a.partial_patch_bytes = (size_t)(d + 2) * (h + 2) * (w + 2) * sizeof(float);
-        if (idx <= 6 && idx % 2 == 0 && fuse_pool[idx / 2]) a.pool_dst = A(idx / 2 + 1);
+        if (idx <= 6 && idx % 2 == 0 && fuse_pool[idx / 2]) a.pool_dst = idx == 0 ? x1_pool : A(idx / 2 + 1);
         const bool last = idx == kNumMfmaConvs - 1, last_but_one = idx == kNumMfmaConvs - 2;
         const int margin = !trimmed ? 0 : last ? trim : last_but_one ? trim - 1 : 0;
         const int full[3] = {d >> l, h >> l, w >> l};
@@ -138,6 +171,17 @@
         a.n = n; a.d = d >> l; a.h = h >> l; a.w = w >> l;
         a.slope = kLeakySlope;
         if (idx == 0 && row) a.row_stride = row_stride;
+        if (idx == 0 && carry) {
+            a.in_z0 = (unsigned short)carry->in_z[0];
+            a.in_z1 = (unsigned short)carry->in_z[1];
+            if (carry->out_skip) {
+                a.carry_dst = carry->out_skip;
+                a.carry_pool_dst = carry->out_pool;
+                a.out_z0 = (unsigned char)carry->out_z[0];
+                a.out_z1 = (unsigned char)carry->out_z[1];
+                a.out_shift = (unsigned short)carry->out_shift;
+            }
+        }
         LayerTimer* t = e->timer;
         const bool timed = t && (t->mask >> idx & 1u) && t->used < LayerTimer::kRing;
         int slot = 0;
@@ -178,14 +222,14 @@
                           reinterpret_cast<const float*>(e->packed + p.first_b_off), A(0), n, d,
                           h, w, p.c0p, kLeakySlope, stream, (e->options & EXASPIM_OPT_FIRST_PER_GROUP) != 0));
     if (absmax) RUN(launch_absmax(dt, A(0), (size_t)n * d * h * w * p.c0p * dtype_size(dt), absmax, stream));
-    RUN(conv(0, A(0), nullptr, skip(0), 0));
+    RUN(conv(0, A(0), nullptr, x1, 0));
     for (int l = 1; l <= 4; ++l) {
         const ConvLayer& L0 = p.conv[2 * l - 1];
-        const void* prev = skip(l - 1);
+        const void* prev = l == 1 ? x1 : skip(l - 1);
         if (!fuse_pool[l - 1])
             RUN(launch_maxpool2(dt, prev, A(l), n, d >> (l - 1), h >> (l - 1), w >> (l - 1), L0.ca,
                                 stream));
-        RUN(conv(2 * l - 1, A(l), nullptr, B(l), l));
+        RUN(conv(2 * l - 1, l == 1 ? x1_pool : A(l), nullptr, B(l), l));
         RUN(conv(2 * l, B(l), nullptr, l < 4 ? skip(l) : A(l), l));
     }
     const void* prev = A(4);
@@ -208,7 +252,7 @@
                                  (e->options & EXASPIM_OPT_PLAIN_UPSAMPLE) != 0,
                                  (e->options & EXASPIM_OPT_UPSAMPLE_PER_THREAD) != 0, ups_trimmed ? ups_hi : nullptr));
         }
-        RUN(conv(i0, skip(l), A(l), B(l), l));
+        RUN(conv(i0, l == 0 ? x1 : skip(l), A(l), B(l), l));
         RUN(conv(i0 + 1, B(l), nullptr, A(l), l));
         prev = A(l);
     }
@@ -417,6 +461,42 @@
                    workspace_bytes, (hipStream_t)stream, x_prepared_dev, nullptr, row_stride, keep_hi);
 }
 
+extern "C" int exaspim_unet_carry_planes(const exaspim_unet* h, int32_t n, int32_t d, int32_t hgt, int32_t w,
+                                         int32_t row_stride, int32_t shift_z, int32_t out[2]) {
+    EXA_CHECK_ARG(h && out, "carry_planes: NULL pointer");
+    out[0] = out[1] = 0;
+    EXA_CHECK_ARG(n > 0 && level_dims_ok(d, hgt, w) && row_stride >= 0 && shift_z > 0,
+                  "carry_planes: bad arguments (n %d, patch %dx%dx%d, row stride %d, shift %d)", n, d, hgt, w,
+                  row_stride, shift_z);
+    const UNetPlan& p = h->plan;
+    const bool fused = !(h->options & EXASPIM_OPT_SEPARATE_POOL) && conv_can_fuse_pool(p.dtype, p.conv[0].cout, d, hgt, w);
+    if ((h->options & EXASPIM_OPT_PER_PATCH_ENCODER) || !conv_row_mode_ok(p.dtype, p.conv[0].cout, n, w, row_stride, fused))
+        return EXASPIM_OK;
+    carry_span(d, shift_z, out);
+    return EXASPIM_OK;
+}
+
+extern "C" int exaspim_unet_forward_prepared_carry(exaspim_unet* h, const void* x_prepared_dev, float* out_dev,
+                                                   int32_t n, int32_t d, int32_t hgt, int32_t w,
+                                                   int32_t apply_sigmoid, int32_t trim, int32_t row_stride,
+                                                   const int32_t keep_hi[3], const exaspim_unet_carry* carry,
+                                                   void* workspace_dev, size_t workspace_bytes, void* stream) {
+    EXA_CHECK_ARG(h && x_prepared_dev && out_dev && workspace_dev && keep_hi && carry, "forward: NULL pointer");
+    EXA_CHECK_ARG(n > 0, "forward: empty batch");
+    EXA_CHECK_ARG(trim >= 0, "forward: negative trim %d", trim);
+    EXA_CHECK_ARG(row_stride >= 0, "forward: negative row stride %d", row_stride);
+    EXA_CHECK_ARG(level_dims_ok(d, hgt, w),
+                  "forward: patch %dx%dx%d: every dimension must be a positive multiple of 16",
+                  d, hgt, w);
+    const int size[3] = {d, hgt, w};
+    for (int i = 0; i < 3; ++i)
+        EXA_CHECK_ARG(keep_hi[i] > trim && keep_hi[i] <= size[i] - trim,
+                      "forward: keep_hi[%d] = %d outside (%d, %d] (trim %d of %d voxels)", i, keep_hi[i], trim,
+                      size[i] - trim, trim, size[i]);
+    return forward(h, nullptr, out_dev, n, d, hgt, w, apply_sigmoid, trim, workspace_dev,
+                   workspace_bytes, (hipStream_t)stream, x_prepared_dev, nullptr, row_stride, keep_hi, carry);
+}
+
 extern "C" int exaspim_unet_forward_trimmed(exaspim_unet* h, const float* x_dev, float* out_dev,
                                             int32_t n, int32_t d, int32_t hgt, int32_t w,
                                             int32_t apply_sigmoid, int32_t trim,
diff --git a/aind_exaspim_neuron_segmentation_amd/csrc/layer_probe.hip b/aind_exaspim_neuron_segmentation_amd/csrc/layer_probe.hip
--- a/aind_exaspim_neuron_segmentation_amd/csrc/layer_probe.hip
+++ b/aind_exaspim_neuron_segmentation_amd/csrc/layer_probe.hip
@@ -104,6 +104,38 @@
     return launch_conv3x3x3_row(dtype, a, stages, stream);
 }
 
+int probe_conv3x3x3_row_carry(int dtype, const void* src, int ca, const void* weights, const float* bias, void* dst,
+                              int cout, int n, int d, int h, int w, float slope, int row_stride, void* pool_dst,
+                              const int32_t* carry, void* carry_dst, void* carry_pool_dst, int stages,
+                              hipStream_t stream) {
+    EXA_CHECK_ARG(carry != nullptr, "probe: NULL carry");
+    for (int i = 0; i < 5; ++i)
+        EXA_CHECK_ARG(carry[i] >= 0 && carry[i] <= (i == 2 || i == 3 ? 254 : 65534), "probe: carry[%d] = %d out of range", i, carry[i]);
+    ConvArgs a{};
+    a.src_a = src;
+    a.ca = ca;
+    a.weights = weights;
+    a.bias = bias;
+    a.dst = dst;
+    a.cout = cout;
+    a.n = n;
+    a.d = d;
+    a.h = h;
+    a.w = w;
+    a.slope = slope;
+    a.row_stride = row_stride;
+    a.pool_dst = pool_dst;
+    a.in_z0 = (unsigned short)carry[0];
+    a.in_z1 = (unsigned short)carry[1];
+    a.out_z0 = (unsigned char)carry[2];
+    a.out_z1 = (unsigned char)carry[3];
+    a.out_shift = (unsigned short)carry[4];
+    a.carry_dst = carry_dst;
+    a.carry_pool_dst = carry_pool_dst;
+    return launch_conv3x3x3_row(dtype, a, stages, stream);
+}
+int probe_last_carry(void) { return last_conv_launch().carry ? 1 : 0; }
+
 int probe_conv_row_mode_ok(int dtype, int cout, int n, int w, int row_stride, int fused_pool_whole_patch) {
     return conv_row_mode_ok(dtype, cout, n, w, row_stride, fused_pool_whole_patch != 0) ? 1 : 0;
 }
diff --git a/aind_exaspim_neuron_segmentation_amd/inference.py b/aind_exaspim_neuron_segmentation_amd/inference.py
--- a/aind_exaspim_neuron_segmentation_amd/inference.py
+++ b/aind_exaspim_neuron_segmentation_amd/inference.py
@@ -1,4 +1,5 @@
 
+import collections
 import ctypes
 import itertools
 import threading
@@ -20,6 +21,8 @@
 DEFAULT_STREAMS = 3
 PLAIN_GATHER = False
 FULL_PATCHES = False
+CARRY_Z = True
+CARRY_POOL_BYTES = 24 << 30
 CLIP_TO_VOLUME = True
 
 _VOX_CODES = {
@@ -655,6 +658,62 @@
     return stride
 
 
+def carry_plan(starts, batch_size, patch_shape, overlap):
+    batch_size = int(batch_size)
+    batches = [starts[i:i + batch_size] for i in range(0, len(starts), batch_size)]
+    chains = {}
+    for bi, b in enumerate(batches):
+        stride = batch_row_stride(b, patch_shape, overlap)
+        if stride > 0:
+            key = (stride, tuple((int(s[1]), int(s[2])) for s in b))
+            chains.setdefault(key, []).append((int(b[0][0]), bi))
+    succ = [None] * len(batches)
+    depth = int(patch_shape[0])
+    for members in chains.values():
+        for z, bi in members:
+            later = [(z2 - z, bj) for z2, bj in members if bj > bi and 0 < z2 - z < depth]
+            if later:
+                succ[bi] = min(later)[1]
+    return succ
+
+
+def _carry_schedule(model, succ, starts, batch_size, patch_shape, overlap, n_streams, device):
+    links = [None] * len(succ)
+    spans = {}
+    for bi, bj in enumerate(succ):
+        if bj is None:
+            continue
+        own = starts[bi * batch_size:(bi + 1) * batch_size]
+        shift = int(starts[bj * batch_size][0]) - int(own[0][0])
+        stride = batch_row_stride(own, patch_shape, overlap)
+        key = (len(own), stride, shift)
+        if key not in spans:
+            spans[key] = model.carry_planes((len(own),) + tuple(patch_shape), stride, shift, device)
+        if spans[key][1] > spans[key][0]:
+            links[bi] = (bj, shift, spans[key])
+    if not any(links):
+        return None, 0
+    has_pair, alive, peak = set(), 0, 0
+    for bi, link in enumerate(links):
+        if bi not in has_pair and link is not None:
+            has_pair.add(bi)
+            alive += 1
+        if link is not None:
+            has_pair.add(link[0])
+            alive += 1
+        peak = max(peak, alive)
+        if bi in has_pair:
+            alive -= 1
+    if n_streams > 1:
+        peak += int(n_streams)
+    skip_elems, pool_elems = model.carry_pair_elems((int(batch_size),) + tuple(patch_shape))
+    need = peak * 2 * (skip_elems + pool_elems)
+    free, _ = torch.cuda.mem_get_info(device)
+    if need > CARRY_POOL_BYTES or need > free // 2:
+        return None, 0
+    return links, peak
+
+
 def batch_keep_hi(starts, patch_shape, trim, global_shape):
     trim = int(trim)
     keep = []
@@ -890,6 +949,24 @@
     prepared_layout = None
     if isinstance(model, UNet3D) and not PLAIN_GATHER:
         prepared_layout = model.input_layout(device)
+    links, free_pairs = None, collections.deque()
+    if CARRY_Z and prepared_layout is not None and not model.needs_resolution():
+        links, peak = _carry_schedule(model, carry_plan(starts, batch_size, plan.patch_shape, plan.overlap), starts,
+                                      batch_size, plan.patch_shape, plan.overlap, n_streams, device)
+        if links is not None:
+            elems = model.carry_pair_elems((batch_size,) + tuple(plan.patch_shape))
+            free_pairs.extend([tuple(torch.empty(e, dtype=torch.int16, device=device) for e in elems), None]
+                              for _ in range(peak))
+            for s in workers:
+                s.wait_stream(main)
+    pending = {}
+
+    def take_pair(worker):
+        pair = free_pairs.popleft()
+        if pair[1] is not None:
+            worker.wait_event(pair[1])
+        return pair
+
     for bi, i in enumerate(range(0, len(starts), batch_size)):
         batch = starts_dev[i:i + batch_size]
         row_stride = batch_row_stride(starts[i:i + batch_size], plan.patch_shape, plan.overlap)
@@ -901,9 +978,29 @@
             if prepared_layout is not None:
                 inputs = _get_batch_inputs(volume, batch, plan.patch_shape, device, clip=clip,
                                            mn=mn, mx=mx, layout=prepared_layout)
+                carry, own = None, None
+                if links is not None and (bi in pending or links[bi] is not None):
+                    own, in_z, before = pending.pop(bi, None) or (take_pair(worker), (0, 0), None)
+                    carry = {"own": own[0], "in_z": in_z}
+                    if before is not None:
+                        worker.wait_event(before)
+                    if links[bi] is not None:
+                        nxt, shift, span = links[bi]
+                        out_pair = take_pair(worker)
+                        carry.update(out=out_pair[0], out_z=(span[0] + shift, span[1] + shift), out_shift=shift)
+                        pending[nxt] = [out_pair, span, None]
                 pred = model.run_prepared(
                     inputs, (int(batch.shape[0]),) + tuple(plan.patch_shape), apply_sigmoid=True,
-                    trim=0 if FULL_PATCHES else plan.trim, row_stride=row_stride, keep_hi=keep_hi)
+                    trim=0 if FULL_PATCHES else plan.trim, row_stride=row_stride, keep_hi=keep_hi, carry=carry)
+                if own is not None:
+                    done = None
+                    if n_streams > 1:
+                        done = torch.cuda.Event()
+                        done.record(worker)
+                    if links[bi] is not None:
+                        pending[links[bi][0]][2] = done
+                    own[1] = done
+                    free_pairs.append(own)
             else:
                 inputs = _get_batch_inputs(volume, batch, plan.patch_shape, device, clip=clip,
                                            mn=mn, mx=mx)
diff --git a/aind_exaspim_neuron_segmentation_amd/machine_learning/unet3d.py b/aind_exaspim_neuron_segmentation_amd/machine_learning/unet3d.py
--- a/aind_exaspim_neuron_segmentation_amd/machine_learning/unet3d.py
+++ b/aind_exaspim_neuron_segmentation_amd/machine_learning/unet3d.py
@@ -315,7 +315,24 @@
             raise RuntimeError("exaspim_unet_input_layout failed")
         return int(code)
 
-    def run_prepared(self, prepared, shape, apply_sigmoid=False, out=None, trim=0, row_stride=0, keep_hi=None):
+    def carry_planes(self, shape, row_stride, shift_z, device=None):
+        device = next(self.parameters()).device if device is None else device
+        n, d, h, w = (int(v) for v in shape)
+        with torch.cuda.device(device):
+            self._ensure_engine(device)
+        span = (ctypes.c_int32 * 2)()
+        _native.check(
+            _native.lib().exaspim_unet_carry_planes(self._engine, n, d, h, w, int(row_stride), int(shift_z), span),
+            "exaspim_unet_carry_planes")
+        return int(span[0]), int(span[1])
+
+    def carry_pair_elems(self, shape):
+        n, d, h, w = (int(v) for v in shape)
+        c0p = -(-int(self.channels[0]) // 32) * 32
+        return n * d * h * w * c0p, n * (d // 2) * (h // 2) * (w // 2) * c0p
+
+    def run_prepared(self, prepared, shape, apply_sigmoid=False, out=None, trim=0, row_stride=0, keep_hi=None,
+                     carry=None):
         if self.training:
             raise RuntimeError(
                 "UNet3D (MI355X) implements eval-mode inference only; call .eval()"
@@ -340,7 +357,31 @@
                 out = torch.empty(
                     (n, self.output_channels, d, h, w), dtype=torch.float32, device=device
                 )
-            if keep_hi is not None:
+            if carry is not None:
+                desc = _native.UNetCarry()
+                need = self.carry_pair_elems(shape)
+                pairs = [carry["own"]] + ([carry["out"]] if carry.get("out") is not None else [])
+                for pair in pairs:
+                    for t, elems in zip(pair, need):
+                        if not t.is_cuda or t.element_size() != 2 or t.numel() < elems or not t.is_contiguous():
+                            raise RuntimeError("carry buffers must be contiguous 16-bit device tensors of "
+                                               f"{need} elements")
+                desc.own_skip, desc.own_pool = carry["own"][0].data_ptr(), carry["own"][1].data_ptr()
+                desc.in_z[:] = [int(v) for v in carry.get("in_z", (0, 0))]
+                if carry.get("out") is not None:
+                    desc.out_skip, desc.out_pool = carry["out"][0].data_ptr(), carry["out"][1].data_ptr()
+                    desc.out_z[:] = [int(v) for v in carry["out_z"]]
+                    desc.out_shift = int(carry["out_shift"])
+                hi = keep_hi if keep_hi is not None else (d - int(trim), h - int(trim), w - int(trim))
+                _native.check(
+                    _native.lib().exaspim_unet_forward_prepared_carry(
+                        self._engine, prepared.data_ptr(), out.data_ptr(), n, d, h, w,
+                        1 if apply_sigmoid else 0, int(trim), int(row_stride), _native.int3(hi),
+                        ctypes.byref(desc), ws.data_ptr(), ws.numel(), stream,
+                    ),
+                    "exaspim_unet_forward_prepared_carry",
+                )
+            elif keep_hi is not None:
                 _native.check(
                     _native.lib().exaspim_unet_forward_prepared_clipped(
                         self._engine, prepared.data_ptr(), out.data_ptr(), n, d, h, w,
diff --git a/include/exaspim_affinity.h b/include/exaspim_affinity.h
--- a/include/exaspim_affinity.h
+++ b/include/exaspim_affinity.h
@@ -88,6 +88,24 @@
                                           int32_t apply_sigmoid, int32_t trim, int32_t row_stride,
                                           const int32_t keep_hi[3], void* workspace_dev,
                                           size_t workspace_bytes, void* stream);
+
+int exaspim_unet_carry_planes(const exaspim_unet* h, int32_t n, int32_t d, int32_t hgt, int32_t w,
+                              int32_t row_stride, int32_t shift_z, int32_t out[2]);
+typedef struct exaspim_unet_carry {
+    void* own_skip;
+    void* own_pool;
+    int32_t in_z[2];
+    void* out_skip;
+    void* out_pool;
+    int32_t out_z[2];
+    int32_t out_shift;
+    int32_t reserved;
+} exaspim_unet_carry;
+int exaspim_unet_forward_prepared_carry(exaspim_unet* h, const void* x_prepared_dev, float* out_dev,
+                                        int32_t n, int32_t d, int32_t hgt, int32_t w,
+                                        int32_t apply_sigmoid, int32_t trim, int32_t row_stride,
+                                        const int32_t keep_hi[3], const exaspim_unet_carry* carry,
+                                        void* workspace_dev, size_t workspace_bytes, void* stream);
 
 #define EXASPIM_ABSMAX_SLOTS 22
 int exaspim_unet_forward_absmax(exaspim_unet* h, const float* x_dev, float* out_dev,
```

Result: faster. 834.4 million voxels/s, median of 6 (+1.8%).
